# assafmu/wav2letter_pytorch

Hardware: AMD Instinct MI355X
Metric: audio-frames/sec/GPU (fwd+bwd+CTC), Wav2Letter 64-mel x 1000-frame bf16 (higher is better)
Workload: dtype bf16

## Files before the change

include/w2l_hip.h:

```cpp
#ifndef W2L_HIP_H
#define W2L_HIP_H
#include <stdint.h>
#ifdef __cplusplus
extern "C" {
#endif

const char* w2l_last_error(void);
int w2l_abi_version(void);


int w2l_pack_weights(const float* w, int64_t s_co, int64_t s_ci, int64_t s_kw, int Cout, int Cin, int Kw,
                     int CoutP, int CinP, void* w_fwd_hi, void* w_fwd_lo, void* w_dgr_hi, void* w_dgr_lo,
                     void* stream);

int w2l_sgd_pack(float* p, float* g, float* m, int first_step, float lr, float momentum, float weight_decay,
                 int nesterov, int zero_grad, int Cout, int Cin, int Kw, void* w_fwd_hi, void* w_fwd_lo, void* w_dgr_hi,
                 void* w_dgr_lo, void* w_fwd_q, void* w_dgr_q, float q_scale, void* stream);

int w2l_nct_to_ntc(const float* x, int N, int C, int T, int CP, int pad_l, int pad_r, int pad_mode,
                   const int32_t* lens, void* out_hi, void* out_lo, void* stream);

int w2l_pad_cast(const float* g, int N, int T, int C, int CP, int halo, void* out_hi, void* out_lo, float* colsum,
                 void* stream);

int w2l_conv_stat_tiles(int N, int Tout);
int w2l_conv1d_igemm(const void* xp, int64_t x_bstride, int64_t x_rows_total, const void* w, void* y, int y_f32,
                     int accumulate, const float* bias, float* stats_partial, int N, int Cin, int Cout, int Tout,
                     int Kw, int stride, int dil, void* stream);

int w2l_conv1d_igemm_tune(const void* xp, int64_t x_bstride, int64_t x_rows_total, const void* w, void* y, int y_f32,
                          const float* bias, float* stats_partial, int N, int Cin, int Cout, int Tout, int Kw, int stride,
                          int dil, int reps, void* stream);

int w2l_conv1d_igemm_ws(const void* xp, int64_t x_bstride, int64_t x_rows_total, const void* w, void* y, int y_f32,
                        int accumulate, const float* bias, float* stats_partial, int N, int Cin, int Cout, int Tout, int Kw,
                        int stride, int dil, void* splitk_ws, int64_t splitk_ws_bytes, void* stream);
int w2l_conv1d_igemm_tune_ws(const void* xp, int64_t x_bstride, int64_t x_rows_total, const void* w, void* y, int y_f32,
                             const float* bias, float* stats_partial, int N, int Cin, int Cout, int Tout, int Kw, int stride,
                             int dil, int reps, void* splitk_ws, int64_t splitk_ws_bytes, void* stream);
int64_t w2l_conv_splitk_workspace_bytes(int N, int Cout, int Tout);
int w2l_conv_streamk_ranges(int idx, int N, int Cin, int Cout, int Tout, int Kw, int stride, int dil, int64_t ws_bytes);
int w2l_conv_streamk_pieces(int tiles, int steps, int G, int* out, int cap);

int w2l_conv1d_igemm_fp8(const void* xq, int64_t x_bstride, int64_t x_rows_total, const void* wq, void* y, int y_f32,
                         float descale, const float* descale_dev, const float* bias, float* stats_partial, int N, int Cin,
                         int Cout, int Tout, int Kw, int dil, void* stream);
int w2l_conv1d_igemm_fp8_tune(const void* xq, int64_t x_bstride, int64_t x_rows_total, const void* wq, void* y, int y_f32,
                              const float* bias, float* stats_partial, int N, int Cin, int Cout, int Tout, int Kw, int dil,
                              int reps, void* stream);

void w2l_conv_force_tile_config(int idx);
void w2l_conv_force_fp8_config(int idx);
int w2l_conv_plan(int N, int Cin, int Cout, int Tout, int Kw, int stride, int dil, int stats_flag, int64_t ws_bytes,
                  int forced_idx, int* out);
int w2l_conv_plan_fp8(int N, int Cin, int Cout, int Tout, int Kw, int dil, int stats_flag, int forced_idx, int* out);

int w2l_wgrad_needs_zero(int N, int Cin, int Cout, int Tout, int Kw);
int w2l_conv1d_wgrad(const void* dy, int64_t dy_bstride, const void* xp, int64_t x_bstride, int64_t x_rows_total,
                     float* dw, int N, int Cin, int Cout, int Tout, int Kw, int stride, int dil, int accumulate,
                     void* stream);

int w2l_conv1d_wgrad_ws(const void* dy, int64_t dy_bstride, const void* xp, int64_t x_bstride, int64_t x_rows_total, float* dw,
                        int N, int Cin, int Cout, int Tout, int Kw, int stride, int dil, int accumulate, void* ws,
                        int64_t ws_bytes, void* stream);
int w2l_conv1d_wgrad_tune_ws(const void* dy, int64_t dy_bstride, const void* xp, int64_t x_bstride, int64_t x_rows_total,
                             float* dw_scratch, int N, int Cin, int Cout, int Tout, int Kw, int stride, int dil, int reps,
                             void* ws, int64_t ws_bytes, void* stream);
int w2l_wgrad_needs_zero_ws(int N, int Cin, int Cout, int Tout, int Kw, int64_t ws_bytes);
int64_t w2l_wgrad_workspace_bytes(int Cin, int Cout, int Kw);

int64_t w2l_wgrad_dealt_workspace_bytes(int Cin, int Cout, int Kw);
int w2l_conv1d_wgrad_tune_x(const void* dy, int64_t dy_bstride, const void* xp, int64_t x_bstride, int64_t x_rows_total,
                            float* dw_scratch, int N, int Cin, int Cout, int Tout, int Kw, int stride, int dil, int reps,
                            void* ws, int64_t ws_bytes, int flags, void* stream);
int w2l_wgrad_needs_zero_x(int N, int Cin, int Cout, int Tout, int Kw, int stride, int dil, int64_t ws_bytes);
int w2l_wgrad_dealt_segments(int tiles, int steps, int ranges, int* out, int max_blocks);
int w2l_wgrad_plan(int N, int Cin, int Cout, int Tout, int Kw);

typedef struct {
    const void* dy;
    int64_t dy_bstride;
    const void* xp;
    int64_t x_bstride;
    int64_t x_rows_total;
    float* dw;
    int Cin, Cout, Kw, pad_;
} w2l_wgrad_item_t;
#define W2L_WGRAD_GROUP_MAX 8
int w2l_conv1d_wgrad_group(const w2l_wgrad_item_t* items, int nitems, int N, int Tout, int dil, int form, void* stream);
int w2l_wgrad_group_tiles(int Cin, int Cout, int Kw, int form);

void w2l_wgrad_force_plan(int splits, int order);
void w2l_wgrad_deterministic(int on);

int w2l_conv1d_wgrad_tune(const void* dy, int64_t dy_bstride, const void* xp, int64_t x_bstride, int64_t x_rows_total,
                          float* dw_scratch, int N, int Cin, int Cout, int Tout, int Kw, int stride, int dil, int reps,
                          void* stream);

int w2l_wgrad_fp8_needs_zero(int N, int Cin, int Cout, int Tout, int Kw);
int w2l_conv1d_wgrad_fp8(const void* dyq, int64_t dy_bstride, const void* xq, int64_t x_bstride, int64_t x_rows_total,
                         float* dw, int N, int Cin, int Cout, int Tout, int Kw, int dil, float descale,
                         const float* descale_dev, int accumulate, void* stream);
int w2l_conv1d_wgrad_fp8_tune(const void* dyq, int64_t dy_bstride, const void* xq, int64_t x_bstride, int64_t x_rows_total,
                              float* dw_scratch, int N, int Cin, int Cout, int Tout, int Kw, int dil, int reps, void* stream);

int w2l_tune_save(const char* path);
int w2l_tune_load(const char* path);

int w2l_dwconv_fwd(const void* x_hi, const void* x_lo, int x_rows, const float* w, void* y_hi, void* y_lo, int N, int Tout,
                   int C, int K, int stride, int dil, const int32_t* lens, void* stream);
int w2l_dwconv_dgrad(const void* dy, int dy_f32, int dy_rows, const float* w, void* dxp, int dxp_f32, int N, int Tp, int Tout,
                     int C, int K, int dil, const int32_t* lens, void* stream);
int w2l_dwconv_wgrad(const void* dy, int dy_f32, int dy_rows, const void* x_hi, const void* x_lo, int x_rows, float* dw, int N,
                     int Tout, int C, int K, int stride, int dil, const int32_t* lens, void* stream);


int w2l_bn_finalize(const float* partial, int ntiles, int C, int64_t count, const float* gamma, const float* beta,
                    float eps, float momentum, float* running_mean, float* running_var, float* mean, float* invstd,
                    float* scale, float* shift, void* stream);

typedef struct {
    int32_t N, T, C;
    const void* y;
    int32_t y_f32;
    const float* scale;
    const float* shift;
    const float* mean;
    const float* invstd;
    const void* y2;
    const float* scale2;
    const float* shift2;
    const float* mean2;
    const float* invstd2;
    int32_t act;
    float drop_p;
    uint64_t seed, offset;
    uint8_t* mask;
    const int32_t* lens;
    const uint64_t* offset_dev;
    uint64_t* q_clipped;
} w2l_bnact_t;

int w2l_bn_act_fwd(const w2l_bnact_t* d, void* out_hi, void* out_lo, int out_rows, int pad_l, int pad_r,
                   int pad_mode, void* stream);
int w2l_bn_act_fwd_q(const w2l_bnact_t* d, void* out_hi, void* out_lo, void* out_q, float q_scale, int out_rows,
                     int pad_l, int pad_r, int pad_mode, void* stream);
typedef struct {
    const float* partial;
    int32_t rows;
    int64_t count;
    const float* gamma;
    const float* beta;
    float eps, momentum;
    float* running_mean;
    float* running_var;
    float* mean;
    float* invstd;
    float* scale;
    float* shift;
} w2l_bnfin_t;
int w2l_bn_act_fwd_fin(const w2l_bnact_t* d, const w2l_bnfin_t* f1, const w2l_bnfin_t* f2, void* out_hi, void* out_q,
                       float q_scale, int out_rows, int pad_l, int pad_r, int pad_mode, void* stream);
void w2l_conv_stats_mode(int slots);

int w2l_quantize_e4m3(const void* src, int src_f32, int64_t n, float scale, void* dst, void* stream);

typedef struct {
    const void* dxp;
    int32_t f32;
    int32_t pad_l, pad_r, pad_mode;
    int32_t rows;
} w2l_gradsrc_t;

int w2l_bn_bwd_blocks(int N, int T, int C);
int w2l_bn_act_bwd_reduce(const w2l_bnact_t* d, const w2l_gradsrc_t* g1, const w2l_gradsrc_t* g2, float* partial,
                          void* stream);
int w2l_bn_bwd_finalize(const float* partial, int nblocks, int C, int ncomp, float* sums, void* stream);
int w2l_bn_act_bwd_apply(const w2l_bnact_t* d, const w2l_gradsrc_t* g1, const w2l_gradsrc_t* g2, const float* sums,
                         void* dy_hi, void* dy_lo, int halo, void* dy2_hi, void* dy2_lo, int halo2, void* stream);
int w2l_bn_act_bwd_apply_fin(const w2l_bnact_t* d, const w2l_gradsrc_t* g1, const w2l_gradsrc_t* g2, const float* partial,
                             int nblocks, float* sums, void* dy_hi, void* dy_lo, int halo, void* dy2_hi, void* dy2_lo,
                             int halo2, float* amax, void* stream);
int w2l_bn_bwd_fast_ok(const w2l_bnact_t* d, const w2l_gradsrc_t* g1, const w2l_gradsrc_t* g2);
int w2l_bn_act_bwd_reduce_slots(const w2l_bnact_t* d, const w2l_gradsrc_t* g1, float* partial, int slots, void* stream);
int w2l_bn_act_bwd_apply_slots(const w2l_bnact_t* d, const w2l_gradsrc_t* g1, const float* partial, int nrows, float* sums,
                               void* dy_hi, int halo, float* amax, void* stream);
#define W2L_AMAX_SLOTS 64
int w2l_bn_act_bwd_apply_amax(const w2l_bnact_t* d, const w2l_gradsrc_t* g1, const w2l_gradsrc_t* g2, const float* sums,
                              void* dy_hi, void* dy_lo, int halo, void* dy2_hi, void* dy2_lo, int halo2, float* amax,
                              void* stream);
int w2l_quantize_e4m3_dyn(const void* src_bf16, int64_t n, const float* amax, void* dst, float* inv_scale, void* stream);

int w2l_conv1d_dgrad_bnreduce_ws(const void* dy, int64_t dy_rows_total, const void* w_dgr, void* dxp, float* partial,
                                 const w2l_bnact_t* d, int pad_l, int pad_r, int pad_mode, int per, int Cconv_out,
                                 int flat_rows, int Kw, int dil, void* splitk_ws, int64_t splitk_ws_bytes, void* stream);
int w2l_conv1d_dgrad_bnreduce_tune_ws(const void* dy, int64_t dy_rows_total, const void* w_dgr, void* dxp, float* partial,
                                      const w2l_bnact_t* d, int pad_l, int pad_r, int pad_mode, int per, int Cconv_out,
                                      int flat_rows, int Kw, int dil, int reps, void* splitk_ws, int64_t splitk_ws_bytes,
                                      void* stream);

typedef struct {
    const float* scale;
    const float* shift;
    const void* res;
    const void* res_lo;
    int32_t act;
    const int32_t* lens;
    void* out_hi;
    void* out_lo;
    int32_t out_rows, pad_l, pad_r, pad_mode;
} w2l_bnact_epi_t;
int w2l_conv1d_igemm_bnact(const void* xp, int64_t x_bstride, int64_t x_rows_total, const void* w, const float* acc_in,
                           const float* bias, const w2l_bnact_epi_t* e, int N, int Cin, int Cout, int Tout, int Kw, int stride,
                           int dil, void* stream);
int w2l_conv1d_igemm_bnact_ws(const void* xp, int64_t x_bstride, int64_t x_rows_total, const void* w, const float* acc_in,
                              const float* bias, const w2l_bnact_epi_t* e, int N, int Cin, int Cout, int Tout, int Kw,
                              int stride, int dil, void* splitk_ws, int64_t splitk_ws_bytes, void* stream);
int w2l_conv1d_igemm_bnact_tune_ws(const void* xp, int64_t x_bstride, int64_t x_rows_total, const void* w, const float* bias,
                                   const w2l_bnact_epi_t* e, int N, int Cin, int Cout, int Tout, int Kw, int stride, int dil,
                                   int reps, void* splitk_ws, int64_t splitk_ws_bytes, void* stream);

int w2l_conv1d_igemm_bnact_fp8(const void* xq, int64_t x_bstride, int64_t x_rows_total, const void* wq, float descale,
                               const float* bias, const w2l_bnact_epi_t* e, void* out_q, float q_scale, int64_t* q_clipped,
                               int N, int Cin, int Cout, int Tout, int Kw, int dil, void* stream);
int w2l_conv1d_igemm_bnact_fp8_tune(const void* xq, int64_t x_bstride, int64_t x_rows_total, const void* wq, const float* bias,
                                    const w2l_bnact_epi_t* e, void* out_q, float q_scale, int N, int Cin, int Cout, int Tout,
                                    int Kw, int dil, int reps, void* stream);

int w2l_log_softmax_fwd(const float* logits, int N, int T, int C, int CP, int mode, float* out, void* stream);
int w2l_log_softmax_bwd(const float* gout, const float* out, int N, int T, int C, int mode, float* glogits,
                        void* stream);
int64_t w2l_ctc_workspace_bytes(int N, int T, int Smax);
int w2l_ctc_loss(const float* log_probs, const int32_t* targets, const int32_t* input_lengths,
                 const int32_t* target_lengths, int N, int T, int C, int Smax, int blank, int zero_infinity,
                 float* nll, float* loss, float* grad, void* workspace, void* stream);

int64_t w2l_ctc_align_workspace_bytes(int N, int T, int Smax);
int w2l_ctc_align(const float* x, const int32_t* input_lengths, const int32_t* targets, int64_t target_stride,
                  const int32_t* target_lengths, int64_t length_stride, int N, int T, int A, int Smax, int blank,
                  int log_probs, void* workspace, int64_t workspace_bytes, float* score, int32_t* status, int32_t* path,
                  int32_t* starts, int32_t* ends, void* stream);

int w2l_argmax(const float* probs, int64_t rows, int C, int32_t* idx, void* stream);
int64_t w2l_ctc_beam_search_workspace_bytes(int N, int T, int k);
int w2l_ctc_beam_search(const float* probs, const int32_t* sizes, int N, int T, int A, const int32_t* label_info_host,
                        int blank, int end_index, int k, double beta, double prune, int log_probs, void* workspace,
                        int64_t workspace_bytes, void* out, void* stream);
typedef struct {
    const float* prob;
    const float* bo;
    const uint64_t* ngram_keys;
    const int32_t* ngram_vals;
    int64_t ngram_cap;
    const uint64_t* trie_keys;
    const int32_t* trie_vals;
    int64_t trie_cap;
    const int32_t* trie_word;
    int32_t n_entries;
    int32_t n_words;
    int32_t n_trie_nodes;
} w2l_ngram_lm_t;
int w2l_ngram_lm_build(const uint64_t* keys, const int32_t* vals, int64_t n, uint64_t* table_keys, int32_t* table_vals,
                       int64_t cap, int32_t* dups, void* stream);
int64_t w2l_ctc_beam_search_lm_workspace_bytes(int N, int T, int k, int order);
int w2l_ctc_beam_search_lm(const float* probs, const int32_t* sizes, int N, int T, int A, const int32_t* label_info_host,
                           int blank, int end_index, int space_index, int k, double alpha, double beta, double prune,
                           int log_probs, const w2l_ngram_lm_t* lm, int order, void* workspace, int64_t workspace_bytes,
                           void* out, void* stream);
int w2l_levenshtein_host(const int32_t* a_host, int na, const int32_t* b_host, int nb);
int w2l_greedy_score_host(const int32_t* idx_host, int N, int T, const int32_t* sizes_host, int blank, const int32_t* lut,
                          int n_labels, const int32_t* ref_cp, const int64_t* ref_off, int64_t* totals, int32_t* hyp_cp,
                          int64_t* hyp_off);

int w2l_novograd_pack(float* p, const float* g, float* exp_avg, float* exp_avg_sq, float* max_exp_avg_sq, float* scratch,
                      int scratch_floats, float lr, float beta1, float beta2, float eps, float weight_decay, int grad_averaging,
                      int Cout, int Cin, int Kw, void* w_fwd_hi, void* w_fwd_lo, void* w_dgr_hi, void* w_dgr_lo, void* stream);

int w2l_logmel(const float* audio, const int32_t* n_samples, const float* noise, float dither, float preemph, int N,
               int64_t audio_stride, const float* window, int win_length, int n_fft, int hop, const float* fbT,
               const int32_t* fb_range, int n_mels, int take_log, float log_guard, float* logmel, int Tmax, void* stream);
int w2l_feature_normalize(const float* logmel, const int32_t* n_samples, int hop, int N, int Tmax, int n_mels, float eps,
                          float* mean_ws, float* std_ws, float* out_nct, void* stream);
int w2l_zero_rects(float* x, int N, int C, int T, const int32_t* rects, int R, void* stream);

#define W2L_RESAMPLE_TILE 512
#define W2L_RESAMPLE_MAX_K 512
#define W2L_RESAMPLE_MAX_SPAN 8192
int w2l_resample(const float* x, int64_t in_stride, float* out, int64_t out_stride, int N, const int32_t* rows_host,
                 const int32_t* rows_dev, const int32_t* banks_host, const int32_t* banks_dev, int n_banks, const float* taps,
                 int64_t n_taps, void* stream);

int w2l_stream_probe(void* stream_a, void* stream_b, void* stamps_dev, int rounds, int spin_us);

// ... 53 lines not shown
```

wav2letter_pytorch_amd/_lib.py:

```python
from __future__ import annotations

import ctypes as C
import os

os.environ.setdefault('GPU_MAX_HW_QUEUES', '8')

import torch

_HERE = os.path.dirname(os.path.abspath(__file__))
LIB_PATH = os.environ.get('W2L_LIB') or os.path.join(_HERE, 'libw2l_hip.so')

c_p = C.c_void_p
c_i = C.c_int
c_i64 = C.c_int64
c_u64 = C.c_uint64
c_f = C.c_float


class BnActDesc(C.Structure):
    _fields_ = [
        ('N', C.c_int32), ('T', C.c_int32), ('C', C.c_int32),
        ('y', c_p), ('y_f32', C.c_int32),
        ('scale', c_p), ('shift', c_p), ('mean', c_p), ('invstd', c_p),
        ('y2', c_p), ('scale2', c_p), ('shift2', c_p), ('mean2', c_p), ('invstd2', c_p),
        ('act', C.c_int32), ('drop_p', c_f), ('seed', c_u64), ('offset', c_u64),
        ('mask', c_p), ('lens', c_p), ('offset_dev', c_p), ('q_clipped', c_p),
    ]


class WgradItem(C.Structure):
    _fields_ = [('dy', c_p), ('dy_bstride', C.c_int64), ('xp', c_p), ('x_bstride', C.c_int64), ('x_rows_total', C.c_int64),
                ('dw', c_p), ('Cin', C.c_int32), ('Cout', C.c_int32), ('Kw', C.c_int32), ('pad_', C.c_int32)]


class BnFin(C.Structure):
    _fields_ = [('partial', c_p), ('rows', C.c_int32), ('count', C.c_int64), ('gamma', c_p), ('beta', c_p), ('eps', c_f),
                ('momentum', c_f), ('running_mean', c_p), ('running_var', c_p), ('mean', c_p), ('invstd', c_p), ('scale', c_p),
                ('shift', c_p)]


class LmTables(C.Structure):
    _fields_ = [('prob', c_p), ('bo', c_p), ('ngram_keys', c_p), ('ngram_vals', c_p), ('ngram_cap', C.c_int64),
                ('trie_keys', c_p), ('trie_vals', c_p), ('trie_cap', C.c_int64), ('trie_word', c_p), ('n_entries', C.c_int32),
                ('n_words', C.c_int32), ('n_trie_nodes', C.c_int32)]


class BnActEpi(C.Structure):
    _fields_ = [('scale', c_p), ('shift', c_p), ('res', c_p), ('res_lo', c_p), ('act', C.c_int32), ('lens', c_p),
                ('out_hi', c_p), ('out_lo', c_p), ('out_rows', C.c_int32), ('pad_l', C.c_int32), ('pad_r', C.c_int32),
                ('pad_mode', C.c_int32)]


class GradSrc(C.Structure):
    _fields_ = [('dxp', c_p), ('f32', C.c_int32), ('pad_l', C.c_int32), ('pad_r', C.c_int32),
                ('pad_mode', C.c_int32), ('rows', C.c_int32)]


_SIGNATURES = {
    'w2l_last_error': (C.c_char_p, []),
    'w2l_abi_version': (c_i, []),
    'w2l_tune_save': (c_i, [C.c_char_p]),
    'w2l_tune_load': (c_i, [C.c_char_p]),
    'w2l_pack_weights': (c_i, [c_p, c_i64, c_i64, c_i64, c_i, c_i, c_i, c_i, c_i, c_p, c_p, c_p, c_p, c_p]),
    'w2l_sgd_pack': (c_i, [c_p, c_p, c_p, c_i, c_f, c_f, c_f, c_i, c_i, c_i, c_i, c_i, c_p, c_p, c_p, c_p, c_p, c_p, c_f, c_p]),
    'w2l_novograd_pack': (c_i, [c_p, c_p, c_p, c_p, c_p, c_p, c_i, c_f, c_f, c_f, c_f, c_f, c_i, c_i, c_i, c_i, c_p, c_p, c_p, c_p,
                                c_p]),
    'w2l_nct_to_ntc': (c_i, [c_p, c_i, c_i, c_i, c_i, c_i, c_i, c_i, c_p, c_p, c_p, c_p]),
    'w2l_pad_cast': (c_i, [c_p, c_i, c_i, c_i, c_i, c_i, c_p, c_p, c_p, c_p]),
    'w2l_conv_stat_tiles': (c_i, [c_i, c_i]),
    'w2l_conv1d_igemm': (c_i, [c_p, c_i64, c_i64, c_p, c_p, c_i, c_i, c_p, c_p, c_i, c_i, c_i, c_i, c_i, c_i, c_i, c_p]),
    'w2l_conv1d_igemm_tune': (c_i, [c_p, c_i64, c_i64, c_p, c_p, c_i, c_p, c_p, c_i, c_i, c_i, c_i, c_i, c_i, c_i, c_i, c_p]),
    'w2l_conv1d_igemm_ws': (c_i, [c_p, c_i64, c_i64, c_p, c_p, c_i, c_i, c_p, c_p, c_i, c_i, c_i, c_i, c_i, c_i, c_i, c_p, c_i64, c_p]),
    'w2l_conv1d_igemm_tune_ws': (c_i, [c_p, c_i64, c_i64, c_p, c_p, c_i, c_p, c_p, c_i, c_i, c_i, c_i, c_i, c_i, c_i, c_i, c_p,
                                       c_i64, c_p]),
    'w2l_conv1d_igemm_bnact': (c_i, [c_p, c_i64, c_i64, c_p, c_p, c_p, C.POINTER(BnActEpi), c_i, c_i, c_i, c_i, c_i, c_i, c_i, c_p]),
    'w2l_conv1d_igemm_bnact_ws': (c_i, [c_p, c_i64, c_i64, c_p, c_p, c_p, C.POINTER(BnActEpi), c_i, c_i, c_i, c_i, c_i, c_i, c_i,
                                        c_p, c_i64, c_p]),
    'w2l_conv1d_igemm_bnact_tune_ws': (c_i, [c_p, c_i64, c_i64, c_p, c_p, C.POINTER(BnActEpi), c_i, c_i, c_i, c_i, c_i, c_i, c_i,
                                             c_i, c_p, c_i64, c_p]),
    'w2l_conv_splitk_workspace_bytes': (c_i64, [c_i, c_i, c_i]),
    'w2l_conv_streamk_ranges': (c_i, [c_i] * 8 + [c_i64]),
    'w2l_conv_streamk_pieces': (c_i, [c_i, c_i, c_i, c_p, c_i]),
    'w2l_conv_force_tile_config': (None, [c_i]),
    'w2l_conv_force_fp8_config': (None, [c_i]),
    'w2l_conv_plan': (c_i, [c_i] * 8 + [c_i64, c_i, c_p]),
    'w2l_conv_plan_fp8': (c_i, [c_i] * 8 + [c_p]),
    'w2l_wgrad_force_plan': (None, [c_i, c_i]),
    'w2l_wgrad_deterministic': (None, [c_i]),
    'w2l_wgrad_needs_zero': (c_i, [c_i, c_i, c_i, c_i, c_i]),
    'w2l_conv1d_wgrad': (c_i, [c_p, c_i64, c_p, c_i64, c_i64, c_p, c_i, c_i, c_i, c_i, c_i, c_i, c_i, c_i, c_p]),
    'w2l_conv1d_wgrad_ws': (c_i, [c_p, c_i64, c_p, c_i64, c_i64, c_p, c_i, c_i, c_i, c_i, c_i, c_i, c_i, c_i, c_p, c_i64, c_p]),
    'w2l_conv1d_wgrad_tune_ws': (c_i, [c_p, c_i64, c_p, c_i64, c_i64, c_p, c_i, c_i, c_i, c_i, c_i, c_i, c_i, c_i, c_p, c_i64, c_p]),
    'w2l_wgrad_needs_zero_ws': (c_i, [c_i, c_i, c_i, c_i, c_i, c_i64]),
    'w2l_wgrad_workspace_bytes': (c_i64, [c_i, c_i, c_i]),
    'w2l_wgrad_dealt_workspace_bytes': (c_i64, [c_i, c_i, c_i]),
    'w2l_conv1d_wgrad_tune_x': (c_i, [c_p, c_i64, c_p, c_i64, c_i64, c_p, c_i, c_i, c_i, c_i, c_i, c_i, c_i, c_i, c_p, c_i64, c_i, c_p]),
    'w2l_wgrad_needs_zero_x': (c_i, [c_i, c_i, c_i, c_i, c_i, c_i, c_i, c_i64]),
    'w2l_wgrad_dealt_segments': (c_i, [c_i, c_i, c_i, c_p, c_i]),
    'w2l_wgrad_plan': (c_i, [c_i, c_i, c_i, c_i, c_i]),
    'w2l_conv1d_wgrad_group': (c_i, [c_p, c_i, c_i, c_i, c_i, c_i, c_p]),
    'w2l_wgrad_group_tiles': (c_i, [c_i, c_i, c_i, c_i]),
    'w2l_conv1d_wgrad_tune': (c_i, [c_p, c_i64, c_p, c_i64, c_i64, c_p, c_i, c_i, c_i, c_i, c_i, c_i, c_i, c_i, c_p]),
    'w2l_dwconv_fwd': (c_i, [c_p, c_p, c_i, c_p, c_p, c_p, c_i, c_i, c_i, c_i, c_i, c_i, c_p, c_p]),
    'w2l_dwconv_dgrad': (c_i, [c_p, c_i, c_i, c_p, c_p, c_i, c_i, c_i, c_i, c_i, c_i, c_i, c_p, c_p]),
    'w2l_dwconv_wgrad': (c_i, [c_p, c_i, c_i, c_p, c_p, c_i, c_p, c_i, c_i, c_i, c_i, c_i, c_i, c_p, c_p]),
    'w2l_bn_finalize': (c_i, [c_p, c_i, c_i, c_i64, c_p, c_p, c_f, c_f, c_p, c_p, c_p, c_p, c_p, c_p, c_p]),
    'w2l_bn_act_fwd': (c_i, [C.POINTER(BnActDesc), c_p, c_p, c_i, c_i, c_i, c_i, c_p]),
    'w2l_bn_act_fwd_q': (c_i, [C.POINTER(BnActDesc), c_p, c_p, c_p, c_f, c_i, c_i, c_i, c_i, c_p]),
    'w2l_bn_bwd_fast_ok': (c_i, [C.POINTER(BnActDesc), C.POINTER(GradSrc), C.POINTER(GradSrc)]),
    'w2l_bn_act_bwd_reduce_slots': (c_i, [C.POINTER(BnActDesc), C.POINTER(GradSrc), c_p, c_i, c_p]),
    'w2l_bn_act_bwd_apply_slots': (c_i, [C.POINTER(BnActDesc), C.POINTER(GradSrc), c_p, c_i, c_p, c_p, c_i, c_p, c_p]),
    'w2l_bn_act_fwd_fin': (c_i, [C.POINTER(BnActDesc), C.POINTER(BnFin), C.POINTER(BnFin), c_p, c_p, c_f, c_i, c_i, c_i, c_i, c_p]),
    'w2l_conv_stats_mode': (None, [c_i]),
    'w2l_quantize_e4m3': (c_i, [c_p, c_i, c_i64, c_f, c_p, c_p]),
    'w2l_quantize_e4m3_dyn': (c_i, [c_p, c_i64, c_p, c_p, c_p, c_p]),
    'w2l_bn_act_bwd_apply_amax': (c_i, [C.POINTER(BnActDesc), C.POINTER(GradSrc), C.POINTER(GradSrc), c_p, c_p, c_p, c_i,
                                        c_p, c_p, c_i, c_p, c_p]),
    'w2l_conv1d_igemm_fp8': (c_i, [c_p, c_i64, c_i64, c_p, c_p, c_i, c_f, c_p, c_p, c_p, c_i, c_i, c_i, c_i, c_i, c_i, c_p]),
    'w2l_conv1d_igemm_bnact_fp8': (c_i, [c_p, c_i64, c_i64, c_p, c_f, c_p, C.POINTER(BnActEpi), c_p, c_f, c_p, c_i, c_i, c_i, c_i,
                                         c_i, c_i, c_p]),
    'w2l_conv1d_igemm_bnact_fp8_tune': (c_i, [c_p, c_i64, c_i64, c_p, c_p, C.POINTER(BnActEpi), c_p, c_f, c_i, c_i, c_i, c_i, c_i,
                                              c_i, c_i, c_p]),
    'w2l_conv1d_igemm_fp8_tune': (c_i, [c_p, c_i64, c_i64, c_p, c_p, c_i, c_p, c_p, c_i, c_i, c_i, c_i, c_i, c_i, c_i, c_p]),
    'w2l_bn_bwd_blocks': (c_i, [c_i, c_i, c_i]),
    'w2l_bn_act_bwd_reduce': (c_i, [C.POINTER(BnActDesc), C.POINTER(GradSrc), C.POINTER(GradSrc), c_p, c_p]),
    'w2l_bn_bwd_finalize': (c_i, [c_p, c_i, c_i, c_i, c_p, c_p]),
    'w2l_bn_act_bwd_apply': (c_i, [C.POINTER(BnActDesc), C.POINTER(GradSrc), C.POINTER(GradSrc), c_p, c_p, c_p, c_i,
                                   c_p, c_p, c_i, c_p]),
    'w2l_conv1d_dgrad_bnreduce_ws': (c_i, [c_p, c_i64, c_p, c_p, c_p, C.POINTER(BnActDesc), c_i, c_i, c_i, c_i, c_i, c_i, c_i, c_i,
                                           c_p, c_i64, c_p]),
    'w2l_conv1d_dgrad_bnreduce_tune_ws': (c_i, [c_p, c_i64, c_p, c_p, c_p, C.POINTER(BnActDesc), c_i, c_i, c_i, c_i, c_i, c_i, c_i,
                                                c_i, c_i, c_p, c_i64, c_p]),
    'w2l_bn_act_bwd_apply_fin': (c_i, [C.POINTER(BnActDesc), C.POINTER(GradSrc), C.POINTER(GradSrc), c_p, c_i, c_p, c_p, c_p, c_i,
                                       c_p, c_p, c_i, c_p, c_p]),
    'w2l_log_softmax_fwd': (c_i, [c_p, c_i, c_i, c_i, c_i, c_i, c_p, c_p]),
    'w2l_log_softmax_bwd': (c_i, [c_p, c_p, c_i, c_i, c_i, c_i, c_p, c_p]),
    'w2l_ctc_workspace_bytes': (c_i64, [c_i, c_i, c_i]),
    'w2l_ctc_loss': (c_i, [c_p, c_p, c_p, c_p, c_i, c_i, c_i, c_i, c_i, c_i, c_p, c_p, c_p, c_p, c_p]),
    'w2l_argmax': (c_i, [c_p, c_i64, c_i, c_p, c_p]),
    'w2l_ctc_align_workspace_bytes': (c_i64, [c_i, c_i, c_i]),
    'w2l_ctc_align': (c_i, [c_p, c_p, c_p, c_i64, c_p, c_i64, c_i, c_i, c_i, c_i, c_i, c_i, c_p, c_i64, c_p, c_p, c_p, c_p, c_p,
                            c_p]),
    'w2l_ctc_beam_search_workspace_bytes': (c_i64, [c_i, c_i, c_i]),
    'w2l_ctc_beam_search': (c_i, [c_p, c_p, c_i, c_i, c_i, c_p, c_i, c_i, c_i, C.c_double, C.c_double, c_i, c_p, c_i64, c_p,
                                  c_p]),
    'w2l_ngram_lm_build': (c_i, [c_p, c_p, c_i64, c_p, c_p, c_i64, c_p, c_p]),
    'w2l_ctc_beam_search_lm_workspace_bytes': (c_i64, [c_i, c_i, c_i, c_i]),
    'w2l_ctc_beam_search_lm': (c_i, [c_p, c_p, c_i, c_i, c_i, c_p, c_i, c_i, c_i, c_i, C.c_double, C.c_double, C.c_double, c_i,
                                     C.POINTER(LmTables), c_i, c_p, c_i64, c_p, c_p]),
    'w2l_logmel': (c_i, [c_p, c_p, c_p, c_f, c_f, c_i, c_i64, c_p, c_i, c_i, c_i, c_p, c_p, c_i, c_i, c_f, c_p, c_i, c_p]),
    'w2l_feature_normalize': (c_i, [c_p, c_p, c_i, c_i, c_i, c_i, c_f, c_p, c_p, c_p, c_p]),
    'w2l_zero_rects': (c_i, [c_p, c_i, c_i, c_i, c_p, c_i, c_p]),
    'w2l_resample': (c_i, [c_p, c_i64, c_p, c_i64, c_i, c_p, c_p, c_p, c_p, c_i, c_p, c_i64, c_p]),
    'w2l_levenshtein_host': (c_i, [c_p, c_i, c_p, c_i]),
    'w2l_greedy_score_host': (c_i, [c_p, c_i, c_i, c_p, c_i, c_p, c_i, c_p, c_p, c_p, c_p, c_p]),
    'w2l_wgrad_fp8_needs_zero': (c_i, [c_i, c_i, c_i, c_i, c_i]),
    'w2l_conv1d_wgrad_fp8': (c_i, [c_p, c_i64, c_p, c_i64, c_i64, c_p, c_i, c_i, c_i, c_i, c_i, c_i, c_f, c_p, c_i, c_p]),
    'w2l_conv1d_wgrad_fp8_tune': (c_i, [c_p, c_i64, c_p, c_i64, c_i64, c_p, c_i, c_i, c_i, c_i, c_i, c_i, c_i, c_p]),
    'w2l_stream_probe': (c_i, [c_p, c_p, c_p, c_i, c_i]),
    'w2l_rccl_available': (c_i, []),
    'w2l_rccl_library': (C.c_char_p, []),
    'w2l_rccl_unique_id': (c_i, [c_p]),
    'w2l_rccl_init': (c_i, [c_p, c_i, c_i, c_p]),
    'w2l_rccl_world': (c_i, [c_p, c_p]),
    'w2l_rccl_all_reduce': (c_i, [c_p, c_p, c_i64, c_i, c_i, c_p]),
    'w2l_rccl_broadcast': (c_i, [c_p, c_p, c_i64, c_i, c_p]),
    'w2l_rccl_destroy': (c_i, [c_p]),
    'w2l_replay_op': (c_i, [C.c_char_p]),
    'w2l_replay_arity': (c_i, [c_i]),
    'w2l_replay': (c_i, [c_p, c_i, c_p]),
    'w2l_event_create': (c_i, [c_p]),
    'w2l_event_destroy': (c_i, [c_p]),
    'w2l_event_record': (c_i, [c_p, c_p]),
    'w2l_stream_wait_event': (c_i, [c_p, c_p]),
    'w2l_event_query': (c_i, [c_p]),
    'w2l_event_synchronize': (c_i, [c_p]),
    'w2l_stream_wait_stream': (c_i, [c_p, c_p]),
    'w2l_fill_zero': (c_i, [c_p, c_i64, c_p]),
    'w2l_pad_vec_f32': (c_i, [c_p, c_i, c_p, c_i, c_f, c_p]),
# ... 378 lines not shown
```

wav2letter_pytorch_amd/csrc/bn_act.hip:

```cpp
#include "common.h"
#include "../../include/w2l_hip.h"

namespace {

#ifndef W2L_PHILOX_ROUNDS
#define W2L_PHILOX_ROUNDS 10
#endif
__device__ __forceinline__ void philox4x32_10(uint32_t c0, uint32_t c1, uint32_t c2, uint32_t c3, uint32_t k0,
                                              uint32_t k1, uint32_t out[4]) {
#pragma unroll
    for (int i = 0; i < W2L_PHILOX_ROUNDS; ++i) {
        const uint64_t p0 = (uint64_t)0xD2511F53u * c0, p1 = (uint64_t)0xCD9E8D57u * c2;
        const uint32_t hi0 = (uint32_t)(p0 >> 32), lo0 = (uint32_t)p0;
        const uint32_t hi1 = (uint32_t)(p1 >> 32), lo1 = (uint32_t)p1;
        const uint32_t n0 = hi1 ^ c1 ^ k0, n1 = lo1, n2 = hi0 ^ c3 ^ k1, n3 = lo0;
        c0 = n0; c1 = n1; c2 = n2; c3 = n3;
        k0 += 0x9E3779B9u; k1 += 0xBB67AE85u;
    }
    out[0] = c0; out[1] = c1; out[2] = c2; out[3] = c3;
}

__device__ __forceinline__ uint32_t dropout_bits(uint64_t seed, uint64_t offset, uint64_t gidx, uint32_t thresh) {
    uint32_t r[4];
    philox4x32_10((uint32_t)gidx, (uint32_t)(gidx >> 32), (uint32_t)offset, (uint32_t)(offset >> 32), (uint32_t)seed,
                  (uint32_t)(seed >> 32), r);
    uint32_t bits = 0;
#pragma unroll
    for (int j = 0; j < 4; ++j) {
        bits |= ((r[j] & 0xFFFFu) >= thresh ? 1u : 0u) << (2 * j);
        bits |= ((r[j] >> 16) >= thresh ? 1u : 0u) << (2 * j + 1);
    }
    return bits;
}

template <bool F32>
__device__ __forceinline__ void load8(const void* base, int64_t off, float v[8]) {
    if (F32) {
        const f32x4* p = reinterpret_cast<const f32x4*>(reinterpret_cast<const float*>(base) + off);
        const f32x4 a = p[0], b = p[1];
#pragma unroll
        for (int j = 0; j < 4; ++j) { v[j] = a[j]; v[4 + j] = b[j]; }
    } else {
        const u16x8 a = *reinterpret_cast<const u16x8*>(reinterpret_cast<const bf16_raw*>(base) + off);
#pragma unroll
        for (int j = 0; j < 8; ++j) v[j] = bf16_bits_to_f32(a[j]);
    }
}
__device__ __forceinline__ void loadp8(const float* p, int c, float v[8]) {
    const f32x4 a = *reinterpret_cast<const f32x4*>(p + c), b = *reinterpret_cast<const f32x4*>(p + c + 4);
#pragma unroll
    for (int j = 0; j < 4; ++j) { v[j] = a[j]; v[4 + j] = b[j]; }
}
__device__ __forceinline__ void store8_split(bf16_raw* hi, bf16_raw* lo, int64_t off, const float v[8]) {
    u16x8 h, l;
#pragma unroll
    for (int j = 0; j < 8; ++j) {
        bf16_raw a, b;
        f32_split_bf16(v[j], a, b);
        h[j] = a; l[j] = b;
    }
    *reinterpret_cast<u16x8*>(hi + off) = h;
    if (lo) *reinterpret_cast<u16x8*>(lo + off) = l;
}

__device__ __forceinline__ int pad_src_row(int r, int T, int pad_l, int pad_r, int pad_mode) {
    int t = r - pad_l;
    if (t >= 0 && t < T) return t;
    if (pad_mode != 1 || t < -pad_l || t >= T + pad_r) return -1;
    t = t < 0 ? -t : 2 * (T - 1) - t;
    return (t >= 0 && t < T) ? t : -1;
}

struct Chan {
    float sc[8], sh[8], m[8], is[8];
};
__device__ __forceinline__ void load_chan(Chan& ch, const float* scale, const float* shift, const float* mean,
                                          const float* invstd, int c) {
#pragma unroll
    for (int j = 0; j < 8; ++j) { ch.sc[j] = 1.f; ch.sh[j] = 0.f; ch.m[j] = 0.f; ch.is[j] = 0.f; }
    if (scale) { loadp8(scale, c, ch.sc); loadp8(shift, c, ch.sh); }
    if (mean) { loadp8(mean, c, ch.m); loadp8(invstd, c, ch.is); }
}

template <bool F32, bool HAS2>
__device__ __forceinline__ uint32_t preact8(const w2l_bnact_t& d, const Chan& c1, const Chan& c2, int64_t row ,
                                            int cg, int G, float z[8], float y1[8], float y2v[8], uint32_t thresh,
                                            float inv_keep, bool gen_mask, bool write_mask) {
    const int64_t off = row * d.C + cg * 8;
    load8<F32>(d.y, off, y1);
#pragma unroll
    for (int j = 0; j < 8; ++j) z[j] = y1[j] * c1.sc[j] + c1.sh[j];
    if (HAS2) {
        load8<F32>(d.y2, off, y2v);
#pragma unroll
        for (int j = 0; j < 8; ++j) z[j] += y2v[j] * c2.sc[j] + c2.sh[j];
    }
    uint32_t bits = 0xFFu;
    if (d.drop_p > 0.f) {
        const int64_t gidx = row * G + cg;
        if (gen_mask) {
            bits = dropout_bits(d.seed, d.offset + (d.offset_dev ? *d.offset_dev : 0ull), (uint64_t)gidx, thresh);
            if (write_mask) d.mask[gidx] = (uint8_t)bits;
        } else {
            bits = d.mask[gidx];
        }
#pragma unroll
        for (int j = 0; j < 8; ++j) z[j] = (bits >> j) & 1u ? z[j] * inv_keep : 0.f;
    }
    return bits;
}

__device__ __forceinline__ float activate(float z, int act) {
    if (act == 1) return fminf(fmaxf(z, 0.f), 20.f);
    if (act == 2) return fmaxf(z, 0.f);
    return z;
}
template <int ACT>
__device__ __forceinline__ float activate_t(float z) {
    if (ACT == 1) return fminf(fmaxf(z, 0.f), 20.f);
    if (ACT == 2) return fmaxf(z, 0.f);
    return z;
}
__device__ __forceinline__ bool act_pass(float z, int act) {
    if (act == 1) return z >= 0.f && z <= 20.f;
    if (act == 2) return z > 0.f;
    return true;
}

constexpr int AMAX_SLOTS = W2L_AMAX_SLOTS;
__device__ __forceinline__ void amax_publish(float* amax, int slot, float mx) {
    unsigned* p = reinterpret_cast<unsigned*>(amax) + slot;
    const unsigned v = __float_as_uint(mx);
    if (v > __hip_atomic_load(p, __ATOMIC_RELAXED, __HIP_MEMORY_SCOPE_AGENT)) atomicMax(p, v);
}
constexpr int BWD_SLAB = 64;

__device__ __forceinline__ uint2 quant8_e4m3(const float v[8], float scale) {
    float q[8];
#pragma unroll
    for (int j = 0; j < 8; ++j) q[j] = fminf(fmaxf(v[j] * scale, -448.f), 448.f);
    int lo = __builtin_amdgcn_cvt_pk_fp8_f32(q[0], q[1], 0, false);
    lo = __builtin_amdgcn_cvt_pk_fp8_f32(q[2], q[3], lo, true);
    int hi = __builtin_amdgcn_cvt_pk_fp8_f32(q[4], q[5], 0, false);
    hi = __builtin_amdgcn_cvt_pk_fp8_f32(q[6], q[7], hi, true);
    return make_uint2((unsigned)lo, (unsigned)hi);
}

template <bool F32, bool HAS2, int ACT>
__global__ __launch_bounds__(256) void bn_act_fwd_kernel(w2l_bnact_t d, bf16_raw* out_hi, bf16_raw* out_lo, int R,
                                                          int pad_l, int pad_r, int pad_mode, uint32_t thresh,
                                                          float inv_keep, uint8_t* out_q, float q_scale, float inv_g) {
    const int G = d.C >> 3;
    const int n = blockIdx.y;
    unsigned clipped = 0;
    const float q_limit = 448.f / q_scale;
    const int idx = blockIdx.x * 256 + threadIdx.x;
    if (idx < R * G) {
        int r = (int)((float)idx * inv_g);
        r -= (r * G > idx) ? 1 : 0;
        r += ((r + 1) * G <= idx) ? 1 : 0;
        const int cg = idx - r * G;
        const unsigned orow = (unsigned)n * R + r;
        const int t = pad_src_row(r, d.T, pad_l, pad_r, pad_mode);
        float a[8];
#pragma unroll
        for (int j = 0; j < 8; ++j) a[j] = 0.f;
        if (t >= 0 && (!d.lens || t < d.lens[n])) {
            float z[8], y1[8], y2v[8];
            Chan c1, c2;
            load_chan(c1, d.scale, d.shift, nullptr, nullptr, cg * 8);
            if (HAS2) load_chan(c2, d.scale2, d.shift2, nullptr, nullptr, cg * 8);
            preact8<F32, HAS2>(d, c1, c2, (int64_t)n * d.T + t, cg, G, z, y1, y2v, thresh, inv_keep, true,
                         r - pad_l == t);
#pragma unroll
            for (int j = 0; j < 8; ++j) a[j] = activate_t<ACT>(z[j]);
        }
        store8_split(out_hi, out_lo, (int64_t)orow * d.C + cg * 8, a);
        if (out_q) {
            *reinterpret_cast<uint2*>(out_q + (int64_t)orow * d.C + cg * 8) = quant8_e4m3(a, q_scale);
            if (d.q_clipped && r - pad_l == t) {
#pragma unroll
                for (int j = 0; j < 8; ++j) clipped += fabsf(a[j]) > q_limit ? 1u : 0u;
            }
        }
    }
    if (out_q && d.q_clipped && __any(clipped != 0)) {
#pragma unroll
        for (int m = 1; m < 64; m <<= 1) clipped += __shfl_xor(clipped, m, 64);
        if ((threadIdx.x & 63) == 0) atomicAdd(reinterpret_cast<unsigned long long*>(d.q_clipped), (unsigned long long)clipped);
    }
}

struct FinBranch {
    const float* partial;
    int rows;
    double count;
    const float* gamma;
    const float* beta;
    float eps, momentum;
    float* running_mean;
    float* running_var;
    float* mean;
    float* invstd;
    float* scale;
    float* shift;
};

#ifndef W2L_FWD_FIN_U
#define W2L_FWD_FIN_U 1
#endif
constexpr int FWD_FIN_U = W2L_FWD_FIN_U;
#ifndef W2L_FWD_FIN_BLOCKS
#define W2L_FWD_FIN_BLOCKS 2560
#endif
__host__ __device__ inline int fwd_rows_per_block(int64_t rows, int C) {
    const int batch = 4 * FWD_FIN_U * 8;
    int64_t nb = (rows * (C / BWD_SLAB) + (int64_t)batch * W2L_FWD_FIN_BLOCKS - 1) / ((int64_t)batch * W2L_FWD_FIN_BLOCKS);
    nb = nb < 1 ? 1 : (nb > 16 ? 16 : nb);
    return (int)nb * batch;
}

template <bool HAS2, int ACT>
__global__ __launch_bounds__(256) void bn_act_fwd_fin_kernel(w2l_bnact_t d, FinBranch f1, FinBranch f2, bf16_raw* out_hi, int R,
                                                              int pad_l, int pad_r, int pad_mode, uint32_t thresh, float inv_keep,
                                                              uint8_t* out_q, float q_scale, int rpb) {
    __shared__ double red[2][2][BWD_SLAB];
    __shared__ float s_sc[2][BWD_SLAB], s_sh[2][BWD_SLAB];
    const int tid = threadIdx.x, lane = tid & 63, wave = tid >> 6;
    const int G = d.C >> 3;
    const int nslabs = d.C / BWD_SLAB;
    const int slab = blockIdx.x % nslabs, chunk = blockIdx.x / nslabs;
    const int cgl = lane & 7, rr = lane >> 3;
    const int cg = slab * (BWD_SLAB / 8) + cgl, c = cg * 8;
    const int T = d.T;
    const int64_t rows = (int64_t)d.N * R;
    constexpr int U = FWD_FIN_U;
    const int nbatch = rpb / (4 * U * 8);
    int64_t q0 = (int64_t)chunk * rpb + (int64_t)wave * (U * 8) + rr;
    u16x8 ya[U], yb[U];
    int nn[U], tt[U], rw[U];
    bool ok[U];
    auto load_batch = [&]() {
#pragma unroll
        for (int u = 0; u < U; ++u) {
            const int64_t q = q0 + 8 * u;
            ok[u] = false;
            nn[u] = 0; tt[u] = 0; rw[u] = 0;
            if (q < rows) {
                const int n = (int)(q / R), r = (int)(q - (int64_t)n * R);
                const int t = pad_src_row(r, T, pad_l, pad_r, pad_mode);
                nn[u] = n; tt[u] = t; rw[u] = r;
                ok[u] = t >= 0 && (!d.lens || t < d.lens[n]);
                if (ok[u]) {
                    const int64_t src = ((int64_t)n * T + t) * d.C + c;
                    ya[u] = *reinterpret_cast<const u16x8*>(reinterpret_cast<const bf16_raw*>(d.y) + src);
                    if (HAS2) yb[u] = *reinterpret_cast<const u16x8*>(reinterpret_cast<const bf16_raw*>(d.y2) + src);
                }
            }
        }
    };
    load_batch();
    {
        const int cc = tid & 63, ch = slab * BWD_SLAB + cc;
        const int br = tid >> 7, k = (tid >> 6) & 1;
        const FinBranch& f = br ? f2 : f1;
        if ((br == 0 || HAS2) && f.partial) {
            double a = 0.0;
            int j = 0;
            for (; j + 8 <= f.rows; j += 8) {
                float v[8];
#pragma unroll
                for (int u = 0; u < 8; ++u) v[u] = f.partial[((int64_t)(j + u) * 2 + k) * d.C + ch];
#pragma unroll
                for (int u = 0; u < 8; ++u) a += v[u];
            }
            for (; j < f.rows; ++j) a += f.partial[((int64_t)j * 2 + k) * d.C + ch];
            red[br][k][cc] = a;
        }
        __syncthreads();
        if (tid < 128 && (tid < 64 || HAS2)) {
            const int b = tid >> 6;
            const FinBranch& g = b ? f2 : f1;
            float sc = 1.f, sh = 0.f;
            if (g.partial) {
                const double mu = red[b][0][cc] / g.count;
                double var = red[b][1][cc] / g.count - mu * mu;
                if (var < 0.0) var = 0.0;
                const float m = (float)mu, istd = (float)(1.0 / sqrt(var + (double)g.eps));
                const float ga = g.gamma ? g.gamma[ch] : 1.f, be = g.beta ? g.beta[ch] : 0.f;
                sc = ga * istd;
                sh = be - m * ga * istd;
                if (chunk == 0) {
                    if (g.running_mean) {
                        const double unbiased = g.count > 1.0 ? var * g.count / (g.count - 1.0) : var;
                        g.running_mean[ch] = (1.f - g.momentum) * g.running_mean[ch] + g.momentum * m;
                        g.running_var[ch] = (1.f - g.momentum) * g.running_var[ch] + g.momentum * (float)unbiased;
                    }
                    if (g.mean) { g.mean[ch] = m; g.invstd[ch] = istd; }
                    g.scale[ch] = sc;
                    g.shift[ch] = sh;
                }
            } else {
                const float* scp = b ? d.scale2 : d.scale;
                const float* shp = b ? d.shift2 : d.shift;
                if (scp) { sc = scp[ch]; sh = shp[ch]; }
            }
            s_sc[b][cc] = sc;
            s_sh[b][cc] = sh;
        }
        __syncthreads();
    }
    float sc1[8], sh1[8], sc2[8], sh2[8];
#pragma unroll
    for (int j = 0; j < 8; ++j) {
        sc1[j] = s_sc[0][cgl * 8 + j]; sh1[j] = s_sh[0][cgl * 8 + j];
        sc2[j] = HAS2 ? s_sc[1][cgl * 8 + j] : 0.f; sh2[j] = HAS2 ? s_sh[1][cgl * 8 + j] : 0.f;
    }
    unsigned clipped = 0;
    const float q_limit = 448.f / q_scale;
    const bool drop = d.drop_p > 0.f;
    const uint64_t off = drop ? d.offset + (d.offset_dev ? *d.offset_dev : 0ull) : 0ull;
    for (int bt = 0; bt < nbatch; ++bt) {
    if (bt) load_batch();
#pragma unroll
    for (int u = 0; u < U; ++u) {
        const int64_t q = q0 + 8 * u;
        if (q >= rows) break;
        float a[8];
#pragma unroll
        for (int j = 0; j < 8; ++j) a[j] = 0.f;
        if (ok[u]) {
            float z[8];
#pragma unroll
            for (int j = 0; j < 8; ++j) {
                z[j] = bf16_bits_to_f32(ya[u][j]) * sc1[j] + sh1[j];
                if (HAS2) z[j] += bf16_bits_to_f32(yb[u][j]) * sc2[j] + sh2[j];
            }
            if (drop) {
                const int64_t gidx = ((int64_t)nn[u] * T + tt[u]) * G + cg;
                const uint32_t bits = dropout_bits(d.seed, off, (uint64_t)gidx, thresh);
                if (rw[u] - pad_l == tt[u]) d.mask[gidx] = (uint8_t)bits;
#pragma unroll
                for (int j = 0; j < 8; ++j) z[j] = (bits >> j) & 1u ? z[j] * inv_keep : 0.f;
            }
#pragma unroll
            for (int j = 0; j < 8; ++j) a[j] = activate_t<ACT>(z[j]);
        }
        store8_split(out_hi, nullptr, q * d.C + c, a);
        if (out_q) {
            *reinterpret_cast<uint2*>(out_q + q * d.C + c) = quant8_e4m3(a, q_scale);
            if (d.q_clipped && rw[u] - pad_l == tt[u]) {
#pragma unroll
                for (int j = 0; j < 8; ++j) clipped += fabsf(a[j]) > q_limit ? 1u : 0u;
            }
        }
    }
    q0 += 4 * U * 8;
    }
    if (out_q && d.q_clipped && __any(clipped != 0)) {
#pragma unroll
        for (int m = 1; m < 64; m <<= 1) clipped += __shfl_xor(clipped, m, 64);
        if (lane == 0) atomicAdd(reinterpret_cast<unsigned long long*>(d.q_clipped), (unsigned long long)clipped);
    }
}

__global__ __launch_bounds__(256) void quantize_e4m3_kernel(const void* src, int src_f32, int64_t ngroups, float scale,
                                                             uint8_t* dst) {
    for (int64_t i = (int64_t)blockIdx.x * 256 + threadIdx.x; i < ngroups; i += (int64_t)gridDim.x * 256) {
        float v[8];
        if (src_f32) load8<true>(src, i * 8, v);
        else load8<false>(src, i * 8, v);
        *reinterpret_cast<uint2*>(dst + i * 8) = quant8_e4m3(v, scale);
    }
}

template <bool GF32>
__device__ __forceinline__ void add_grad8(const w2l_gradsrc_t& s, int n, int t, int T, int C, int cg, float g[8]) {
    const int64_t base = (int64_t)n * s.rows;
    float v[8];
    load8<GF32>(s.dxp, (base + t + s.pad_l) * C + cg * 8, v);
#pragma unroll
    for (int j = 0; j < 8; ++j) g[j] += v[j];
    if (s.pad_mode == 1) {
        if (t >= 1 && t <= s.pad_l) {
            load8<GF32>(s.dxp, (base + s.pad_l - t) * C + cg * 8, v);
#pragma unroll
            for (int j = 0; j < 8; ++j) g[j] += v[j];
        }
        if (t <= T - 2 && t >= T - 1 - s.pad_r) {
            load8<GF32>(s.dxp, (base + s.pad_l + 2 * (T - 1) - t) * C + cg * 8, v);
#pragma unroll
            for (int j = 0; j < 8; ++j) g[j] += v[j];
        }
    }
}

struct BwdRow {
    float g[8];
    float xh1[8];
    float xh2[8];
};

template <bool F32, bool GF32, bool HAS2>
__device__ __forceinline__ void bwd_row(const w2l_bnact_t& d, const Chan& c1, const Chan& c2, const w2l_gradsrc_t& g1,
                                        const w2l_gradsrc_t& g2, int has_g2, int n, int t, int cg, int G, float inv_keep,
                                        BwdRow& o) {
    float z[8], y1[8], y2v[8];
#pragma unroll
    for (int j = 0; j < 8; ++j) { o.g[j] = 0.f; o.xh1[j] = 0.f; o.xh2[j] = 0.f; y2v[j] = 0.f; }
    const uint32_t bits = preact8<F32, HAS2>(d, c1, c2, (int64_t)n * d.T + t, cg, G, z, y1, y2v, 0, inv_keep, false, false);
    const bool masked = d.lens && t >= d.lens[n];
    float g[8];
#pragma unroll
    for (int j = 0; j < 8; ++j) g[j] = 0.f;
    if (!masked) {
        add_grad8<GF32>(g1, n, t, d.T, d.C, cg, g);
        if (has_g2) add_grad8<GF32>(g2, n, t, d.T, d.C, cg, g);
    }
    const float gk = d.drop_p > 0.f ? inv_keep : 1.f;
#pragma unroll
    for (int j = 0; j < 8; ++j) {
        const bool keep = (bits >> j) & 1u;
        o.g[j] = (!masked && keep && act_pass(z[j], d.act)) ? g[j] * gk : 0.f;
        o.xh1[j] = (y1[j] - c1.m[j]) * c1.is[j];
        if (HAS2) o.xh2[j] = (y2v[j] - c2.m[j]) * c2.is[j];
    }
}

__host__ __device__ inline int bwd_rows_per_wave(int64_t rows, int C) {
    int64_t rw = (rows * (C / BWD_SLAB) + 4095) / 4096;
    rw = (rw + 7) / 8 * 8;
    return (int)(rw < 16 ? 16 : (rw > 64 ? 64 : rw));
}

template <bool F32, bool GF32, bool HAS2>
__global__ __launch_bounds__(256) void bn_act_bwd_reduce_kernel(w2l_bnact_t d, w2l_gradsrc_t g1, w2l_gradsrc_t g2,
                                                                 int has_g2, float* partial, float inv_keep, int rw,
                                                                 int nchunks) {
    const int G = d.C >> 3;
    const int nslabs = d.C / BWD_SLAB;
    const int lane = threadIdx.x & 63;
    const int task = blockIdx.x * 4 + (threadIdx.x >> 6);
    if (task >= nslabs * nchunks) return;
    const int chunk = task / nslabs, slab = task - chunk * nslabs;
    const int cg = slab * (BWD_SLAB / 8) + (lane & 7);
    const int rr = lane >> 3;
    constexpr int ncomp = HAS2 ? 4 : 2;
    const int64_t rows = (int64_t)d.N * d.T;
    const int64_t row0 = (int64_t)chunk * rw;
    int64_t rend = row0 + rw;
    if (rend > rows) rend = rows;
    float s0[8], s1[8], s2[8];
#pragma unroll
    for (int j = 0; j < 8; ++j) { s0[j] = 0.f; s1[j] = 0.f; s2[j] = 0.f; }
    Chan c1, c2;
    load_chan(c1, d.scale, d.shift, d.mean, d.invstd, cg * 8);
    if (HAS2) load_chan(c2, d.scale2, d.shift2, d.mean2, d.invstd2, cg * 8);
    int n = (int)((row0 + rr) / d.T), t = (int)((row0 + rr) - (int64_t)n * d.T);
#pragma unroll 2
    for (int64_t row = row0 + rr; row < rend; row += 8, t += 8) {
        while (t >= d.T) { t -= d.T; ++n; }
        BwdRow o;
        bwd_row<F32, GF32, HAS2>(d, c1, c2, g1, g2, has_g2, n, t, cg, G, inv_keep, o);
#pragma unroll
        for (int j = 0; j < 8; ++j) {
            s0[j] += o.g[j];
            s1[j] += o.g[j] * o.xh1[j];
            if (HAS2) s2[j] += o.g[j] * o.xh2[j];
        }
    }
#pragma unroll
    for (int m = 8; m < 64; m <<= 1)
#pragma unroll
        for (int j = 0; j < 8; ++j) {
            s0[j] += __shfl_xor(s0[j], m, 64);
            s1[j] += __shfl_xor(s1[j], m, 64);
            if (HAS2) s2[j] += __shfl_xor(s2[j], m, 64);
        }
    if (rr == 0) {
        float* dst = partial + (int64_t)chunk * ncomp * d.C + cg * 8;
        auto put = [&](float* q, const float* v) {
            *reinterpret_cast<f32x4*>(q) = f32x4{v[0], v[1], v[2], v[3]};
            *reinterpret_cast<f32x4*>(q + 4) = f32x4{v[4], v[5], v[6], v[7]};
        };
        put(dst, s0);
        put(dst + d.C, s1);
        if (ncomp == 4) { put(dst + 2 * d.C, s0); put(dst + 3 * d.C, s2); }
    }
}

__global__ __launch_bounds__(256) void bn_bwd_finalize_kernel(const float* partial, int nblocks, int ncols, float* sums) {
    __shared__ float red[8][33];
    const int cx = threadIdx.x & 31, ly = threadIdx.x >> 5;
    const int col = blockIdx.x * 32 + cx;
    float s = 0.f;
    if (col < ncols) {
        int b = ly;
        float a[8];
        for (; b + 56 < nblocks; b += 64) {
#pragma unroll
// ... 100 lines not shown
        }
    }
}

__host__ __device__ inline int apply_rows_per_block(int64_t rows, int C) {
    int64_t r = rows * (C / BWD_SLAB) / 1536;
    r = (r + 31) / 32 * 32;
    return (int)(r < 64 ? 64 : (r > 1024 ? 1024 : r));
}

template <bool F32, bool GF32, bool HAS2>
__global__ __launch_bounds__(256) void bn_act_bwd_apply_fin_kernel(w2l_bnact_t d, w2l_gradsrc_t g1, w2l_gradsrc_t g2,
                                                                    int has_g2, const float* partial, int nb, float* sums_out,
                                                                    bf16_raw* dy_hi, bf16_raw* dy_lo, int h1, bf16_raw* dy2_hi,
                                                                    bf16_raw* dy2_lo, int h2, float inv_keep, float* amax,
                                                                    int rpb) {
    constexpr int ncomp = HAS2 ? 4 : 2;
    __shared__ float red[4][ncomp][BWD_SLAB];
    __shared__ float ssum[ncomp][BWD_SLAB];
    const int tid = threadIdx.x, lane = tid & 63, wave = tid >> 6;
    const int G = d.C >> 3;
    const int nslabs = d.C / BWD_SLAB;
    const int slab = blockIdx.x % nslabs, chunk = blockIdx.x / nslabs;
    const int T = d.T, N = d.N;
    {
        const int c = slab * BWD_SLAB + (tid & 63);
        float a[ncomp];
#pragma unroll
        for (int k = 0; k < ncomp; ++k) a[k] = 0.f;
        int j = wave;
        for (; j + 12 < nb; j += 16) {
            float v[4][ncomp];
#pragma unroll
            for (int u = 0; u < 4; ++u)
#pragma unroll
                for (int k = 0; k < ncomp; ++k) v[u][k] = partial[((int64_t)(j + 4 * u) * ncomp + k) * d.C + c];
#pragma unroll
            for (int u = 0; u < 4; ++u)
#pragma unroll
                for (int k = 0; k < ncomp; ++k) a[k] += v[u][k];
        }
        for (; j < nb; j += 4)
#pragma unroll
            for (int k = 0; k < ncomp; ++k) a[k] += partial[((int64_t)j * ncomp + k) * d.C + c];
#pragma unroll
        for (int k = 0; k < ncomp; ++k) red[wave][k][tid & 63] = a[k];
        __syncthreads();
        if (tid < ncomp * BWD_SLAB) {
            const int k = tid >> 6, cc = tid & 63;
            const float t4 = (red[0][k][cc] + red[1][k][cc]) + (red[2][k][cc] + red[3][k][cc]);
            ssum[k][cc] = t4;
            if (chunk == 0) sums_out[(int64_t)k * d.C + slab * BWD_SLAB + cc] = t4;
        }
        __syncthreads();
    }
    const int cgl = lane & 7, rr = lane >> 3;
    const int cg = slab * (BWD_SLAB / 8) + cgl, c = cg * 8;
    Chan c1, c2;
    load_chan(c1, d.scale, d.shift, d.mean, d.invstd, c);
    if (HAS2) load_chan(c2, d.scale2, d.shift2, d.mean2, d.invstd2, c);
    float sg[8], sgx[8], sg2[8], sgx2[8];
#pragma unroll
    for (int j = 0; j < 8; ++j) {
        sg[j] = ssum[0][cgl * 8 + j];
        sgx[j] = ssum[1][cgl * 8 + j];
        sg2[j] = HAS2 ? ssum[2][cgl * 8 + j] : 0.f;
        sgx2[j] = HAS2 ? ssum[3][cgl * 8 + j] : 0.f;
    }
    const float invM = 1.f / ((float)N * (float)T);
    const int64_t rows = (int64_t)N * T;
    const int rpw = rpb >> 2;
    const int64_t row0 = (int64_t)chunk * rpb + (int64_t)wave * rpw;
    int64_t rend = row0 + rpw;
    if (rend > rows) rend = rows;
    float mx1 = 0.f, mx2 = 0.f;
    if (row0 + rr < rend) {
        int n = (int)((row0 + rr) / T), t = (int)((row0 + rr) - (int64_t)n * T);
#pragma unroll 2
        for (int64_t row = row0 + rr; row < rend; row += 8, t += 8) {
            while (t >= T) { t -= T; ++n; }
            BwdRow o;
            bwd_row<F32, GF32, HAS2>(d, c1, c2, g1, g2, has_g2, n, t, cg, G, inv_keep, o);
            float o1[8], o2[8];
            if (d.mean) {
#pragma unroll
                for (int j = 0; j < 8; ++j) o1[j] = c1.sc[j] * (o.g[j] - sg[j] * invM - o.xh1[j] * sgx[j] * invM);
            } else {
#pragma unroll
                for (int j = 0; j < 8; ++j) o1[j] = o.g[j] * c1.sc[j];
            }
            store8_split(dy_hi, dy_lo, ((int64_t)h1 + (int64_t)n * (T + h1) + t) * d.C + c, o1);
            if (amax) {
#pragma unroll
                for (int j = 0; j < 8; ++j) mx1 = fmaxf(mx1, fabsf(o1[j]));
            }
            if (HAS2 && dy2_hi) {
                if (d.mean2) {
#pragma unroll
                    for (int j = 0; j < 8; ++j) o2[j] = c2.sc[j] * (o.g[j] - sg2[j] * invM - o.xh2[j] * sgx2[j] * invM);
                } else {
#pragma unroll
                    for (int j = 0; j < 8; ++j) o2[j] = o.g[j] * c2.sc[j];
                }
                store8_split(dy2_hi, dy2_lo, ((int64_t)h2 + (int64_t)n * (T + h2) + t) * d.C + c, o2);
                if (amax) {
#pragma unroll
                    for (int j = 0; j < 8; ++j) mx2 = fmaxf(mx2, fabsf(o2[j]));
                }
            }
        }
    }
    {
        const int nchunks = gridDim.x / nslabs;
        float z[8];
#pragma unroll
        for (int j = 0; j < 8; ++j) z[j] = 0.f;
        for (int pass = 0; pass < 2; ++pass) {
            bf16_raw* hi = pass ? dy2_hi : dy_hi;
            bf16_raw* lo = pass ? dy2_lo : dy_lo;
            const int h = pass ? h2 : h1;
            if (hi == nullptr || h == 0) continue;
            const int total = h * (N + 1);
            const int per = (total + nchunks - 1) / nchunks;
            int e = (chunk + 1) * per;
            if (e > total) e = total;
            for (int hr = chunk * per + wave * 8 + rr; hr < e; hr += 32) {
                const int gap = hr / h, r = hr - gap * h;
                store8_split(hi, lo, ((int64_t)gap * (T + h) + r) * d.C + c, z);
            }
        }
    }
    if (amax) {
#pragma unroll
        for (int m = 1; m < 64; m <<= 1) {
            mx1 = fmaxf(mx1, __shfl_xor(mx1, m, 64));
            mx2 = fmaxf(mx2, __shfl_xor(mx2, m, 64));
        }
        if (lane == 0) {
            const int slot = blockIdx.x & (AMAX_SLOTS - 1);
            amax_publish(amax, slot, mx1);
            if (HAS2 && dy2_hi) amax_publish(amax, AMAX_SLOTS + slot, mx2);
        }
    }
}


struct FastRow {
    u16x8 y, g, ga, gb;
    unsigned bits;
    bool live, fa, fb, masked;
    int n, t;
};

__device__ __forceinline__ void fast_row_load(const w2l_bnact_t& d, const w2l_gradsrc_t& s, int64_t row, int64_t rows, int c,
                                              int cg, int G, FastRow& o) {
    o.live = row < rows;
    o.fa = o.fb = o.masked = false;
    o.bits = 0xFFu;
    o.n = 0; o.t = 0;
    if (!o.live) return;
    const int T = d.T;
    const int n = (int)(row / T), t = (int)(row - (int64_t)n * T);
    o.n = n; o.t = t;
    o.y = *reinterpret_cast<const u16x8*>(reinterpret_cast<const bf16_raw*>(d.y) + row * d.C + c);
    if (d.drop_p > 0.f) o.bits = d.mask[row * G + cg];
    o.masked = d.lens && t >= d.lens[n];
    const bf16_raw* gp = reinterpret_cast<const bf16_raw*>(s.dxp);
    const int64_t base = (int64_t)n * s.rows;
    o.g = *reinterpret_cast<const u16x8*>(gp + (base + t + s.pad_l) * d.C + c);
    if (s.pad_mode == 1) {
        o.fa = t >= 1 && t <= s.pad_l;
        o.fb = t <= T - 2 && t >= T - 1 - s.pad_r;
        if (o.fa) o.ga = *reinterpret_cast<const u16x8*>(gp + (base + s.pad_l - t) * d.C + c);
        if (o.fb) o.gb = *reinterpret_cast<const u16x8*>(gp + (base + s.pad_l + 2 * (T - 1) - t) * d.C + c);
    }
}

template <int ACT, bool DROP>
__device__ __forceinline__ void fast_row_eval(const FastRow& r, const Chan& ch, float inv_keep, float g[8], float xh[8]) {
    float gv[8];
#pragma unroll
    for (int j = 0; j < 8; ++j) gv[j] = bf16_bits_to_f32(r.g[j]);
    if (r.fa) {
#pragma unroll
        for (int j = 0; j < 8; ++j) gv[j] += bf16_bits_to_f32(r.ga[j]);
    }
    if (r.fb) {
#pragma unroll
        for (int j = 0; j < 8; ++j) gv[j] += bf16_bits_to_f32(r.gb[j]);
    }
    const float gk = DROP ? inv_keep : 1.f;
    const bool row_ok = !r.masked;
#pragma unroll
    for (int j = 0; j < 8; ++j) {
        const float y = bf16_bits_to_f32(r.y[j]);
        float z = y * ch.sc[j] + ch.sh[j];
        bool pass = row_ok;
        if (DROP) {
            pass = pass && ((r.bits >> j) & 1u);
            z *= inv_keep;
        }
        if (ACT == 1) pass = pass && z >= 0.f && z <= 20.f;
        else if (ACT == 2) pass = pass && z > 0.f;
        g[j] = pass ? gv[j] * gk : 0.f;
        xh[j] = (y - ch.m[j]) * ch.is[j];
    }
}

template <int U, int ACT, bool DROP>
__global__ __launch_bounds__(256) void bn_bwd_reduce_fast_kernel(w2l_bnact_t d, w2l_gradsrc_t g1, float* partial, float inv_keep,
                                                                  int slots) {
    __shared__ float red[4][2][BWD_SLAB];
    const int tid = threadIdx.x, lane = tid & 63, wave = tid >> 6;
    const int G = d.C >> 3, nslabs = d.C / BWD_SLAB;
    const int slab = blockIdx.x % nslabs, chunk = blockIdx.x / nslabs;
    const int cgl = lane & 7, rr = lane >> 3;
    const int cg = slab * (BWD_SLAB / 8) + cgl, c = cg * 8;
    const int64_t rows = (int64_t)d.N * d.T;
    const int64_t q0 = ((int64_t)chunk * 4 + wave) * (U * 8) + rr;
    FastRow r[U];
#pragma unroll
    for (int u = 0; u < U; ++u) fast_row_load(d, g1, q0 + 8 * u, rows, c, cg, G, r[u]);
    Chan ch;
    load_chan(ch, d.scale, d.shift, d.mean, d.invstd, c);
    float s0[8], s1[8];
#pragma unroll
    for (int j = 0; j < 8; ++j) { s0[j] = 0.f; s1[j] = 0.f; }
#pragma unroll
    for (int u = 0; u < U; ++u) {
        if (!r[u].live) continue;
        float g[8], xh[8];
        fast_row_eval<ACT, DROP>(r[u], ch, inv_keep, g, xh);
#pragma unroll
        for (int j = 0; j < 8; ++j) { s0[j] += g[j]; s1[j] += g[j] * xh[j]; }
    }
#pragma unroll
    for (int m = 8; m < 64; m <<= 1)
#pragma unroll
        for (int j = 0; j < 8; ++j) {
            s0[j] += __shfl_xor(s0[j], m, 64);
            s1[j] += __shfl_xor(s1[j], m, 64);
        }
    if (rr == 0) {
#pragma unroll
        for (int j = 0; j < 8; ++j) { red[wave][0][cgl * 8 + j] = s0[j]; red[wave][1][cgl * 8 + j] = s1[j]; }
    }
    __syncthreads();
    if (tid < 2 * BWD_SLAB) {
        const int k = tid >> 6, cc = tid & 63;
        const float t4 = (red[0][k][cc] + red[1][k][cc]) + (red[2][k][cc] + red[3][k][cc]);
        atomicAdd(partial + ((int64_t)(chunk % slots) * 2 + k) * d.C + slab * BWD_SLAB + cc, t4);
    }
}

template <int U, int ACT, bool DROP>
__global__ __launch_bounds__(256) void bn_bwd_apply_fast_kernel(w2l_bnact_t d, w2l_gradsrc_t g1, const float* partial, int nb,
                                                                 float* sums_out, bf16_raw* dy_hi, int h1, float inv_keep,
                                                                 float* amax) {
    __shared__ float ssum[2][BWD_SLAB];
    __shared__ float smax[4];
    const int tid = threadIdx.x, lane = tid & 63, wave = tid >> 6;
    const int G = d.C >> 3, nslabs = d.C / BWD_SLAB;
    const int slab = blockIdx.x % nslabs, chunk = blockIdx.x / nslabs;
    const int cgl = lane & 7, rr = lane >> 3;
    const int cg = slab * (BWD_SLAB / 8) + cgl, c = cg * 8;
    const int T = d.T, N = d.N;
    const int64_t rows = (int64_t)N * T;
    const int64_t q0 = ((int64_t)chunk * 4 + wave) * (U * 8) + rr;
    FastRow r[U];
#pragma unroll
    for (int u = 0; u < U; ++u) fast_row_load(d, g1, q0 + 8 * u, rows, c, cg, G, r[u]);
    if (tid < 2 * BWD_SLAB) {
        const int k = tid >> 6, cc = tid & 63;
        float a = 0.f;
        int j = 0;
        for (; j + 8 <= nb; j += 8) {
            float v[8];
#pragma unroll
            for (int u = 0; u < 8; ++u) v[u] = partial[((int64_t)(j + u) * 2 + k) * d.C + slab * BWD_SLAB + cc];
#pragma unroll
            for (int u = 0; u < 8; ++u) a += v[u];
        }
        for (; j < nb; ++j) a += partial[((int64_t)j * 2 + k) * d.C + slab * BWD_SLAB + cc];
        ssum[k][cc] = a;
        if (chunk == 0) sums_out[(int64_t)k * d.C + slab * BWD_SLAB + cc] = a;
    }
    __syncthreads();
    Chan ch;
    load_chan(ch, d.scale, d.shift, d.mean, d.invstd, c);
    float sg[8], sgx[8];
#pragma unroll
    for (int j = 0; j < 8; ++j) { sg[j] = ssum[0][cgl * 8 + j]; sgx[j] = ssum[1][cgl * 8 + j]; }
    const float invM = 1.f / ((float)N * (float)T);
    float mx = 0.f;
#pragma unroll
    for (int u = 0; u < U; ++u) {
        if (!r[u].live) continue;
        float g[8], xh[8], o[8];
        fast_row_eval<ACT, DROP>(r[u], ch, inv_keep, g, xh);
        if (d.mean) {
#pragma unroll
            for (int j = 0; j < 8; ++j) o[j] = ch.sc[j] * (g[j] - sg[j] * invM - xh[j] * sgx[j] * invM);
        } else {
#pragma unroll
            for (int j = 0; j < 8; ++j) o[j] = g[j] * ch.sc[j];
        }
        store8_split(dy_hi, nullptr, ((int64_t)h1 + (int64_t)r[u].n * (T + h1) + r[u].t) * d.C + c, o);
        if (amax) {
#pragma unroll
            for (int j = 0; j < 8; ++j) mx = fmaxf(mx, fabsf(o[j]));
        }
    }
    if (h1 > 0) {
        const int nchunks = gridDim.x / nslabs;
        float z[8];
#pragma unroll
        for (int j = 0; j < 8; ++j) z[j] = 0.f;
        const int total = h1 * (N + 1);
        const int per = (total + nchunks - 1) / nchunks;
        int e = (chunk + 1) * per;
        if (e > total) e = total;
        for (int hr = chunk * per + wave * 8 + rr; hr < e; hr += 32) {
            const int gap = hr / h1, rw = hr - gap * h1;
            store8_split(dy_hi, nullptr, ((int64_t)gap * (T + h1) + rw) * d.C + c, z);
        }
    }
    if (amax) {
#pragma unroll
        for (int m = 1; m < 64; m <<= 1) mx = fmaxf(mx, __shfl_xor(mx, m, 64));
        if (lane == 0) smax[wave] = mx;
        __syncthreads();
        if (tid == 0) amax_publish(amax, blockIdx.x & (AMAX_SLOTS - 1), fmaxf(fmaxf(smax[0], smax[1]), fmaxf(smax[2], smax[3])));
    }
}

struct RowCur {
    int64_t row;
    int n, t;
    const bf16_raw* py;
    const bf16_raw* pg;
    const uint8_t* pm;
};
__device__ __forceinline__ void rowcur_init(RowCur& q, const w2l_bnact_t& d, const w2l_gradsrc_t& s, int64_t row, int c, int cg, int G) {
    q.row = row;
    q.n = (int)(row / d.T);
    q.t = (int)(row - (int64_t)q.n * d.T);
    q.py = reinterpret_cast<const bf16_raw*>(d.y) + row * d.C + c;
    q.pg = reinterpret_cast<const bf16_raw*>(s.dxp) + ((int64_t)q.n * s.rows + q.t + s.pad_l) * d.C + c;
    q.pm = d.mask ? d.mask + row * G + cg : nullptr;
}
__device__ __forceinline__ void rowcur_step(RowCur& q, const w2l_bnact_t& d, const w2l_gradsrc_t& s, int G) {
    q.row += 8;
    q.t += 8;
    q.py += 8 * (int64_t)d.C;
    q.pg += 8 * (int64_t)d.C;
    if (q.pm) q.pm += 8 * G;
    if (q.t >= d.T) {
        q.t -= d.T;
        ++q.n;
        q.pg += (int64_t)(s.rows - d.T) * d.C;
    }
}
__device__ __forceinline__ void fast_row_load_cur(const w2l_bnact_t& d, const w2l_gradsrc_t& s, const RowCur& q, bool live, FastRow& o) {
    o.live = live;
    o.fa = o.fb = o.masked = false;
    o.bits = 0xFFu;
    o.n = q.n; o.t = q.t;
    if (!live) return;
    const int T = d.T, t = q.t;
    o.y = *reinterpret_cast<const u16x8*>(q.py);
    if (d.drop_p > 0.f) o.bits = *q.pm;
    o.masked = d.lens && t >= d.lens[q.n];
    o.g = *reinterpret_cast<const u16x8*>(q.pg);
    if (s.pad_mode == 1) {
        o.fa = t >= 1 && t <= s.pad_l;
        o.fb = t <= T - 2 && t >= T - 1 - s.pad_r;
        if (o.fa) o.ga = *reinterpret_cast<const u16x8*>(q.pg - 2 * (int64_t)t * d.C);
        if (o.fb) o.gb = *reinterpret_cast<const u16x8*>(q.pg + 2 * (int64_t)(T - 1 - t) * d.C);
    }
}

template <int ACT, bool DROP>
__global__ __launch_bounds__(256) void bn_bwd_reduce_loop_kernel(w2l_bnact_t d, w2l_gradsrc_t g1, float* partial, float inv_keep,
                                                                  int slots, int iters) {
    __shared__ float red[4][2][BWD_SLAB];
    const int tid = threadIdx.x, lane = tid & 63, wave = tid >> 6;
    const int G = d.C >> 3, nslabs = d.C / BWD_SLAB;
    const int slab = blockIdx.x % nslabs, chunk = blockIdx.x / nslabs;
    const int cgl = lane & 7, rr = lane >> 3;
    const int cg = slab * (BWD_SLAB / 8) + cgl, c = cg * 8;
    const int64_t rows = (int64_t)d.N * d.T;
    RowCur q;
    rowcur_init(q, d, g1, ((int64_t)chunk * 4 + wave) * ((int64_t)iters * 8) + rr, c, cg, G);
    FastRow cur, nxt;
    fast_row_load_cur(d, g1, q, q.row < rows, cur);
    Chan ch;
    load_chan(ch, d.scale, d.shift, d.mean, d.invstd, c);
    float s0[8], s1[8];
#pragma unroll
    for (int j = 0; j < 8; ++j) { s0[j] = 0.f; s1[j] = 0.f; }
    for (int it = 0; it < iters; ++it) {
        rowcur_step(q, d, g1, G);
        fast_row_load_cur(d, g1, q, it + 1 < iters && q.row < rows, nxt);
        if (cur.live) {
            float g[8], xh[8];
            fast_row_eval<ACT, DROP>(cur, ch, inv_keep, g, xh);
#pragma unroll
            for (int j = 0; j < 8; ++j) { s0[j] += g[j]; s1[j] += g[j] * xh[j]; }
        }
        cur = nxt;
    }
#pragma unroll
    for (int m = 8; m < 64; m <<= 1)
#pragma unroll
        for (int j = 0; j < 8; ++j) {
            s0[j] += __shfl_xor(s0[j], m, 64);
            s1[j] += __shfl_xor(s1[j], m, 64);
        }
    if (rr == 0) {
#pragma unroll
        for (int j = 0; j < 8; ++j) { red[wave][0][cgl * 8 + j] = s0[j]; red[wave][1][cgl * 8 + j] = s1[j]; }
    }
    __syncthreads();
    if (tid < 2 * BWD_SLAB) {
        const int k = tid >> 6, cc = tid & 63;
        const float t4 = (red[0][k][cc] + red[1][k][cc]) + (red[2][k][cc] + red[3][k][cc]);
        atomicAdd(partial + ((int64_t)(chunk % slots) * 2 + k) * d.C + slab * BWD_SLAB + cc, t4);
    }
}

template <int ACT, bool DROP>
__global__ __launch_bounds__(256) void bn_bwd_apply_loop_kernel(w2l_bnact_t d, w2l_gradsrc_t g1, const float* partial, int nb,
                                                                 float* sums_out, bf16_raw* dy_hi, int h1, float inv_keep,
                                                                 float* amax, int iters) {
    __shared__ float ssum[2][BWD_SLAB];
    __shared__ float smax[4];
    const int tid = threadIdx.x, lane = tid & 63, wave = tid >> 6;
    const int G = d.C >> 3, nslabs = d.C / BWD_SLAB;
    const int slab = blockIdx.x % nslabs, chunk = blockIdx.x / nslabs;
    const int cgl = lane & 7, rr = lane >> 3;
    const int cg = slab * (BWD_SLAB / 8) + cgl, c = cg * 8;
    const int T = d.T, N = d.N;
    const int64_t rows = (int64_t)N * T;
    RowCur q;
    rowcur_init(q, d, g1, ((int64_t)chunk * 4 + wave) * ((int64_t)iters * 8) + rr, c, cg, G);
    bf16_raw* pdy = dy_hi + ((int64_t)h1 + (int64_t)q.n * (T + h1) + q.t) * d.C + c;
    FastRow cur, nxt;
    fast_row_load_cur(d, g1, q, q.row < rows, cur);
    if (tid < 2 * BWD_SLAB) {
        const int k = tid >> 6, cc = tid & 63;
        float a = 0.f;
        int j = 0;
        for (; j + 8 <= nb; j += 8) {
            float v[8];
#pragma unroll
            for (int u = 0; u < 8; ++u) v[u] = partial[((int64_t)(j + u) * 2 + k) * d.C + slab * BWD_SLAB + cc];
#pragma unroll
            for (int u = 0; u < 8; ++u) a += v[u];
        }
        for (; j < nb; ++j) a += partial[((int64_t)j * 2 + k) * d.C + slab * BWD_SLAB + cc];
        ssum[k][cc] = a;
        if (chunk == 0) sums_out[(int64_t)k * d.C + slab * BWD_SLAB + cc] = a;
    }
    __syncthreads();
    Chan ch;
    load_chan(ch, d.scale, d.shift, d.mean, d.invstd, c);
    const float invM = 1.f / ((float)N * (float)T);
    float sg[8], sgx[8];
#pragma unroll
    for (int j = 0; j < 8; ++j) { sg[j] = ssum[0][cgl * 8 + j] * invM; sgx[j] = ssum[1][cgl * 8 + j] * invM; }
    float mx = 0.f;
    for (int it = 0; it < iters; ++it) {
        bf16_raw* const pdy_cur = pdy;
        pdy += (int64_t)(q.t + 8 >= T ? 8 + h1 : 8) * d.C;
        rowcur_step(q, d, g1, G);
        fast_row_load_cur(d, g1, q, it + 1 < iters && q.row < rows, nxt);
        if (cur.live) {
            float g[8], xh[8], o[8];
            fast_row_eval<ACT, DROP>(cur, ch, inv_keep, g, xh);
            if (d.mean) {
#pragma unroll
                for (int j = 0; j < 8; ++j) o[j] = ch.sc[j] * (g[j] - sg[j] - xh[j] * sgx[j]);
            } else {
#pragma unroll
                for (int j = 0; j < 8; ++j) o[j] = g[j] * ch.sc[j];
            }
            store8_split(pdy_cur, nullptr, 0, o);
            if (amax) {
#pragma unroll
                for (int j = 0; j < 8; ++j) mx = fmaxf(mx, fabsf(o[j]));
            }
        }
        cur = nxt;
    }
    if (h1 > 0) {
        const int nchunks = gridDim.x / nslabs;
        float z[8];
#pragma unroll
        for (int j = 0; j < 8; ++j) z[j] = 0.f;
        const int total = h1 * (N + 1);
        const int per = (total + nchunks - 1) / nchunks;
        int e = (chunk + 1) * per;
        if (e > total) e = total;
        for (int hr = chunk * per + wave * 8 + rr; hr < e; hr += 32) {
            const int gap = hr / h1, rw = hr - gap * h1;
            store8_split(dy_hi, nullptr, ((int64_t)gap * (T + h1) + rw) * d.C + c, z);
        }
    }
    if (amax) {
#pragma unroll
        for (int m = 1; m < 64; m <<= 1) mx = fmaxf(mx, __shfl_xor(mx, m, 64));
        if (lane == 0) smax[wave] = mx;
        __syncthreads();
        if (tid == 0) amax_publish(amax, blockIdx.x & (AMAX_SLOTS - 1), fmaxf(fmaxf(smax[0], smax[1]), fmaxf(smax[2], smax[3])));
    }
}

__global__ __launch_bounds__(256) void quantize_e4m3_dyn_kernel(const bf16_raw* src, int64_t ngroups, const float* amax,
                                                                 uint8_t* dst, float* inv_scale) {
    float a = amax[threadIdx.x & (AMAX_SLOTS - 1)];
#pragma unroll
    for (int m = 1; m < 64; m <<= 1) a = fmaxf(a, __shfl_xor(a, m, 64));
    const float scale = a > 0.f ? exp2f(floorf(log2f(224.f / a))) : 1.f;
    if (blockIdx.x == 0 && threadIdx.x == 0) inv_scale[0] = 1.f / scale;
    for (int64_t i = (int64_t)blockIdx.x * 256 + threadIdx.x; i < ngroups; i += (int64_t)gridDim.x * 256) {
        float v[8];
        load8<false>(src, i * 8, v);
        *reinterpret_cast<uint2*>(dst + i * 8) = quant8_e4m3(v, scale);
    }
}

__global__ __launch_bounds__(256) void bn_finalize_kernel(const float* partial, int ntiles, int C, double count,
                                                          const float* gamma, const float* beta, float eps, float momentum,
                                                          float* running_mean, float* running_var, float* mean,
                                                          float* invstd, float* scale, float* shift) {
    __shared__ double red1[8][33], red2[8][33];
    const int cx = threadIdx.x & 31, ly = threadIdx.x >> 5;
    const int c = blockIdx.x * 32 + cx;
    double s1 = 0.0, s2 = 0.0;
    if (partial && c < C) {
        int t = ly;
        for (; t + 56 < ntiles; t += 64) {
            float a[8], b[8];
#pragma unroll
            for (int u = 0; u < 8; ++u) {
                a[u] = partial[(int64_t)(t + 8 * u) * 2 * C + c];
                b[u] = partial[(int64_t)(t + 8 * u) * 2 * C + C + c];
            }
#pragma unroll
            for (int u = 0; u < 8; ++u) { s1 += a[u]; s2 += b[u]; }
        }
        for (; t < ntiles; t += 8) {
            s1 += partial[(int64_t)t * 2 * C + c];
            s2 += partial[(int64_t)t * 2 * C + C + c];
        }
    }
    red1[ly][cx] = s1;
    red2[ly][cx] = s2;
    __syncthreads();
    if (ly != 0 || c >= C) return;
    float m, istd;
    if (partial) {
        s1 = 0.0; s2 = 0.0;
#pragma unroll
        for (int k = 0; k < 8; ++k) { s1 += red1[k][cx]; s2 += red2[k][cx]; }
        const double mu = s1 / count;
        double var = s2 / count - mu * mu;
        if (var < 0.0) var = 0.0;
        m = (float)mu;
        istd = (float)(1.0 / sqrt(var + (double)eps));
        if (running_mean) {
            const double unbiased = count > 1.0 ? var * count / (count - 1.0) : var;
            running_mean[c] = (1.f - momentum) * running_mean[c] + momentum * m;
            running_var[c] = (1.f - momentum) * running_var[c] + momentum * (float)unbiased;
        }
    } else {
        m = running_mean[c];
        istd = 1.f / sqrtf(running_var[c] + eps);
    }
    const float g = gamma ? gamma[c] : 1.f, b = beta ? beta[c] : 0.f;
    if (mean) { mean[c] = m; invstd[c] = istd; }
    scale[c] = g * istd;
    shift[c] = b - m * g * istd;
}

int elementwise_blocks(int64_t items) {
    int64_t b = (items + 255) / 256;
    return (int)(b < 1 ? 1 : (b > 4096 ? 4096 : b));
}

int check_desc(const w2l_bnact_t* d, const char* who) {
    W2L_CHECK_ARG(d && d->y, "%s: null descriptor / y", who);
    W2L_CHECK_ARG(d->N > 0 && d->T > 0 && d->C > 0 && d->C % 8 == 0 && d->C <= 2048, "%s: bad N/T/C (%d,%d,%d)", who,
                  d->N, d->T, d->C);
    W2L_CHECK_ARG(d->drop_p >= 0.f && d->drop_p < 1.f, "%s: dropout p must be in [0,1)", who);
    W2L_CHECK_ARG(d->drop_p == 0.f || d->mask, "%s: dropout needs a mask buffer", who);
    W2L_CHECK_ARG((d->scale == nullptr) == (d->shift == nullptr), "%s: scale/shift must come together", who);
    return 0;
}

}

extern "C" int w2l_bn_finalize(const float* partial, int ntiles, int C, int64_t count, const float* gamma,
                               const float* beta, float eps, float momentum, float* running_mean, float* running_var,
                               float* mean, float* invstd, float* scale, float* shift, void* stream) {
    W2L_CHECK_ARG(scale && shift && C > 0, "bn_finalize: null output");
    W2L_CHECK_ARG(partial || (running_mean && running_var), "bn_finalize: eval mode needs running stats");
    W2L_CHECK_ARG(!partial || (ntiles > 0 && count > 0), "bn_finalize: bad tile count");
    hipLaunchKernelGGL(bn_finalize_kernel, dim3((C + 31) / 32), dim3(256), 0, (hipStream_t)stream, partial, ntiles, C,
                       (double)count, gamma, beta, eps, momentum, running_mean, running_var, mean, invstd, scale, shift);
    W2L_CHECK_LAUNCH();
    return 0;
}

extern "C" int w2l_bn_act_fwd(const w2l_bnact_t* d, void* out_hi, void* out_lo, int out_rows, int pad_l, int pad_r,
                              int pad_mode, void* stream) {
    return w2l_bn_act_fwd_q(d, out_hi, out_lo, nullptr, 1.f, out_rows, pad_l, pad_r, pad_mode, stream);
}

extern "C" int w2l_quantize_e4m3(const void* src, int src_f32, int64_t n, float scale, void* dst, void* stream) {
    W2L_CHECK_ARG(src && dst && n > 0 && n % 8 == 0 && scale > 0.f, "quantize_e4m3: bad arguments (n must be a multiple of 8)");
    hipLaunchKernelGGL(quantize_e4m3_kernel, dim3(elementwise_blocks(n / 8)), dim3(256), 0, (hipStream_t)stream, src, src_f32,
                       n / 8, scale, (uint8_t*)dst);
    W2L_CHECK_LAUNCH();
    return 0;
}

extern "C" int w2l_bn_act_fwd_q(const w2l_bnact_t* d, void* out_hi, void* out_lo, void* out_q, float q_scale, int out_rows,
                                int pad_l, int pad_r, int pad_mode, void* stream) {
    if (int e = check_desc(d, "bn_act_fwd")) return e;
    W2L_CHECK_ARG(!out_q || q_scale > 0.f, "bn_act_fwd: the e4m3 copy needs a positive scale");
    W2L_CHECK_ARG(out_hi && out_rows >= pad_l + d->T + pad_r && pad_l >= 0 && pad_r >= 0, "bn_act_fwd: bad output geometry");
    W2L_CHECK_ARG(pad_mode != 1 || (pad_l < d->T && pad_r < d->T), "bn_act_fwd: reflect pad (%d,%d) needs pad < T=%d",
                  pad_l, pad_r, d->T);
    const uint32_t thresh = (uint32_t)(d->drop_p * 65536.f);
    const float inv_keep = 1.f / (1.f - d->drop_p);
    W2L_CHECK_ARG((int64_t)d->N * out_rows * (d->C / 8) < (1LL << 31), "bn_act_fwd: tensor too large for 32-bit indexing");
    const int64_t per_utt = (int64_t)out_rows * (d->C / 8);
    W2L_CHECK_ARG(per_utt < (1 << 24) && d->N <= 65535, "bn_act_fwd: more than 2^24 channel groups per utterance or N > 65535");
    const dim3 grid((unsigned)((per_utt + 255) / 256), (unsigned)d->N);
    const float inv_g = 1.f / (float)(d->C / 8);
#define W2L_FWD_A(F, H, A)                                                                                   \
    hipLaunchKernelGGL((bn_act_fwd_kernel<F, H, A>), grid, dim3(256), 0, (hipStream_t)stream, *d,               \
                       (bf16_raw*)out_hi, (bf16_raw*)out_lo, out_rows, pad_l, pad_r, pad_mode, thresh, inv_keep,    \
                       (uint8_t*)out_q, q_scale, inv_g)
#define W2L_FWD(F, H) do { if (d->act == 1) W2L_FWD_A(F, H, 1); else if (d->act == 2) W2L_FWD_A(F, H, 2); else W2L_FWD_A(F, H, 0); } while (0)
    if (d->y_f32) { if (d->y2) W2L_FWD(true, true); else W2L_FWD(true, false); }
    else { if (d->y2) W2L_FWD(false, true); else W2L_FWD(false, false); }
#undef W2L_FWD
#undef W2L_FWD_A
    W2L_CHECK_LAUNCH();
    return 0;
}

extern "C" int w2l_bn_act_fwd_fin(const w2l_bnact_t* d, const w2l_bnfin_t* f1, const w2l_bnfin_t* f2, void* out_hi, void* out_q,
                                  float q_scale, int out_rows, int pad_l, int pad_r, int pad_mode, void* stream) {
    if (int e = check_desc(d, "bn_act_fwd_fin")) return e;
    W2L_CHECK_ARG(!d->y_f32, "bn_act_fwd_fin: bf16 y only (the fp32 mode takes w2l_bn_finalize + w2l_bn_act_fwd)");
    W2L_CHECK_ARG(d->C % BWD_SLAB == 0, "bn_act_fwd_fin: C=%d must be a multiple of %d", d->C, BWD_SLAB);
    W2L_CHECK_ARG(f1 && (f2 != nullptr) == (d->y2 != nullptr), "bn_act_fwd_fin: one finalize record per branch");
    W2L_CHECK_ARG(!out_q || q_scale > 0.f, "bn_act_fwd_fin: the e4m3 copy needs a positive scale");
    W2L_CHECK_ARG(out_hi && out_rows >= pad_l + d->T + pad_r && pad_l >= 0 && pad_r >= 0, "bn_act_fwd_fin: bad output geometry");
    W2L_CHECK_ARG(pad_mode != 1 || (pad_l < d->T && pad_r < d->T), "bn_act_fwd_fin: reflect pad (%d,%d) needs pad < T=%d", pad_l,
                  pad_r, d->T);
    FinBranch b[2];
    const w2l_bnfin_t* fs[2] = {f1, f2};
    for (int i = 0; i < 2; ++i) {
        FinBranch& o = b[i];
        const w2l_bnfin_t* f = fs[i];
        o = FinBranch{nullptr, 0, 1.0, nullptr, nullptr, 0.f, 0.f, nullptr, nullptr, nullptr, nullptr, nullptr, nullptr};
        if (!f) continue;
        W2L_CHECK_ARG(!f->partial || (f->rows > 0 && f->count > 0 && f->scale && f->shift), "bn_act_fwd_fin: bad finalize record");
        o = FinBranch{f->partial, f->rows, (double)f->count, f->gamma, f->beta, f->eps, f->momentum, f->running_mean, f->running_var,
                      f->mean, f->invstd, f->scale, f->shift};
    }
    const uint32_t thresh = (uint32_t)(d->drop_p * 65536.f);
    const float inv_keep = 1.f / (1.f - d->drop_p);
    const int64_t rows = (int64_t)d->N * out_rows;
    W2L_CHECK_ARG(rows * (d->C / 8) < (1LL << 31), "bn_act_fwd_fin: tensor too large for 32-bit indexing");
    const int rpb = fwd_rows_per_block(rows, d->C);
    const int nchunks = (int)((rows + rpb - 1) / rpb);
    const dim3 grid((unsigned)(nchunks * (d->C / BWD_SLAB)));
#define W2L_FIN_A(H, A)                                                                                                      \
    hipLaunchKernelGGL((bn_act_fwd_fin_kernel<H, A>), grid, dim3(256), 0, (hipStream_t)stream, *d, b[0], b[1], (bf16_raw*)out_hi, \
                       out_rows, pad_l, pad_r, pad_mode, thresh, inv_keep, (uint8_t*)out_q, q_scale, rpb)
#define W2L_FIN(H) do { if (d->act == 1) W2L_FIN_A(H, 1); else if (d->act == 2) W2L_FIN_A(H, 2); else W2L_FIN_A(H, 0); } while (0)
    if (d->y2) W2L_FIN(true); else W2L_FIN(false);
#undef W2L_FIN
#undef W2L_FIN_A
    W2L_CHECK_LAUNCH();
    return 0;
}

extern "C" int w2l_bn_bwd_blocks(int N, int T, int C) {
    if (N <= 0 || T <= 0 || C < BWD_SLAB) return 0;
    const int64_t rows = (int64_t)N * T;
    const int rw = bwd_rows_per_wave(rows, C);
    return (int)((rows + rw - 1) / rw);
}

#define W2L_DISPATCH_BWD2(KERNEL, H2, ...)                                                                 \
    do {                                                                                                   \
        if (d->y_f32 && g1->f32) hipLaunchKernelGGL((KERNEL<true, true, H2>), __VA_ARGS__);                \
        else if (d->y_f32) hipLaunchKernelGGL((KERNEL<true, false, H2>), __VA_ARGS__);                     \
        else if (g1->f32) hipLaunchKernelGGL((KERNEL<false, true, H2>), __VA_ARGS__);                      \
        else hipLaunchKernelGGL((KERNEL<false, false, H2>), __VA_ARGS__);                                  \
    } while (0)
#define W2L_DISPATCH_BWD(KERNEL, ...)                                                                      \
    do {                                                                                                   \
        if (d->y2) W2L_DISPATCH_BWD2(KERNEL, true, __VA_ARGS__);                                           \
        else W2L_DISPATCH_BWD2(KERNEL, false, __VA_ARGS__);                                                \
    } while (0)

extern "C" int w2l_bn_act_bwd_reduce(const w2l_bnact_t* d, const w2l_gradsrc_t* g1, const w2l_gradsrc_t* g2,
                                     float* partial, void* stream) {
    if (int e = check_desc(d, "bn_act_bwd_reduce")) return e;
    W2L_CHECK_ARG(g1 && g1->dxp && partial, "bn_act_bwd_reduce: null pointer");
    W2L_CHECK_ARG(!g2 || g2->f32 == g1->f32, "bn_act_bwd_reduce: gradient sources must share a dtype");
    W2L_CHECK_ARG(g1->rows >= g1->pad_l + d->T + g1->pad_r && (!g2 || g2->rows >= g2->pad_l + d->T + g2->pad_r),
                  "bn_act_bwd_reduce: gradient source has too few rows per utterance");
    W2L_CHECK_ARG(d->C % BWD_SLAB == 0, "bn_act_bwd_reduce: C=%d must be a multiple of %d", d->C, BWD_SLAB);
    const int64_t rows = (int64_t)d->N * d->T;
    const int rw = bwd_rows_per_wave(rows, d->C);
    const int nchunks = w2l_bn_bwd_blocks(d->N, d->T, d->C);
    const int tasks = nchunks * (d->C / BWD_SLAB);
    const float inv_keep = 1.f / (1.f - d->drop_p);
    w2l_gradsrc_t g2v = g2 ? *g2 : *g1;
    W2L_DISPATCH_BWD(bn_act_bwd_reduce_kernel, dim3((tasks + 3) / 4), dim3(256), 0, (hipStream_t)stream, *d, *g1, g2v,
                     g2 ? 1 : 0, partial, inv_keep, rw, nchunks);
    W2L_CHECK_LAUNCH();
    return 0;
}

static bool bwd_fast_ok(const w2l_bnact_t* d, const w2l_gradsrc_t* g1, const w2l_gradsrc_t* g2) {
    return !d->y_f32 && !d->y2 && g1 && !g1->f32 && g2 == nullptr && d->C % BWD_SLAB == 0 && d->scale != nullptr;
}

static int bn_loop_iters(int64_t rows, int T, int C) {
    static const int forced = getenv("W2L_BN_LOOP_ITERS") ? atoi(getenv("W2L_BN_LOOP_ITERS")) : -1;
    int it = forced >= 0 ? forced : ((rows >= 12000 && rows * C >= 8000000) ? 4 : 0);
    if (T < 8) it = 0;
    while (it > 1 && rows < 4LL * it * 8 * 4) it >>= 1;
    return it;
}

extern "C" int w2l_bn_bwd_fast_ok(const w2l_bnact_t* d, const w2l_gradsrc_t* g1, const w2l_gradsrc_t* g2) {
    return d && bwd_fast_ok(d, g1, g2) ? 1 : 0;
}

extern "C" int w2l_bn_act_bwd_reduce_slots(const w2l_bnact_t* d, const w2l_gradsrc_t* g1, float* partial, int slots, void* stream) {
    if (int e = check_desc(d, "bn_act_bwd_reduce_slots")) return e;
    W2L_CHECK_ARG(g1 && g1->dxp && partial && slots >= 1 && slots <= 64, "bn_act_bwd_reduce_slots: null pointer / slots not in 1..64");
    W2L_CHECK_ARG(bwd_fast_ok(d, g1, nullptr), "bn_act_bwd_reduce_slots: bf16 y and gradient, one branch, one source, C %% 64 == 0 only");
    W2L_CHECK_ARG(g1->rows >= g1->pad_l + d->T + g1->pad_r, "bn_act_bwd_reduce_slots: gradient source has too few rows per utterance");
    const int64_t rows = (int64_t)d->N * d->T;
    const float inv_keep = 1.f / (1.f - d->drop_p);
    const bool drop = d->drop_p > 0.f;
    const int iters = bn_loop_iters(rows, d->T, d->C);
    if (iters > 0) {
        const int nch = (int)((rows + 4LL * iters * 8 - 1) / (4LL * iters * 8));
        const dim3 lgrid((unsigned)(nch * (d->C / BWD_SLAB)));
#define W2L_REDL(A, D) hipLaunchKernelGGL((bn_bwd_reduce_loop_kernel<A, D>), lgrid, dim3(256), 0, (hipStream_t)stream, *d, *g1, partial, inv_keep, slots, iters)
        switch (d->act) {
            case 1: if (drop) W2L_REDL(1, true); else W2L_REDL(1, false); break;
            case 2: if (drop) W2L_REDL(2, true); else W2L_REDL(2, false); break;
            default: if (drop) W2L_REDL(0, true); else W2L_REDL(0, false); break;
        }
#undef W2L_REDL
        W2L_CHECK_LAUNCH();
        return 0;
    }
    constexpr int U = 2;
    const int nchunks = (int)((rows + 4 * U * 8 - 1) / (4 * U * 8));
    const dim3 grid((unsigned)(nchunks * (d->C / BWD_SLAB)));
#define W2L_RED(A, D) hipLaunchKernelGGL((bn_bwd_reduce_fast_kernel<U, A, D>), grid, dim3(256), 0, (hipStream_t)stream, *d, *g1, partial, inv_keep, slots)
    switch (d->act) {
        case 1: if (drop) W2L_RED(1, true); else W2L_RED(1, false); break;
        case 2: if (drop) W2L_RED(2, true); else W2L_RED(2, false); break;
        default: if (drop) W2L_RED(0, true); else W2L_RED(0, false); break;
    }
#undef W2L_RED
    W2L_CHECK_LAUNCH();
    return 0;
}

extern "C" int w2l_bn_act_bwd_apply_slots(const w2l_bnact_t* d, const w2l_gradsrc_t* g1, const float* partial, int nrows, float* sums,
                                          void* dy_hi, int halo, float* amax, void* stream) {
    if (int e = check_desc(d, "bn_act_bwd_apply_slots")) return e;
    W2L_CHECK_ARG(g1 && g1->dxp && dy_hi && partial && sums && nrows > 0 && halo >= 0, "bn_act_bwd_apply_slots: null pointer / no partial rows");
    W2L_CHECK_ARG(bwd_fast_ok(d, g1, nullptr), "bn_act_bwd_apply_slots: bf16 y and gradient, one branch, one source, C %% 64 == 0 only");
    W2L_CHECK_ARG(g1->rows >= g1->pad_l + d->T + g1->pad_r, "bn_act_bwd_apply_slots: gradient source has too few rows per utterance");
    const int64_t rows = (int64_t)d->N * d->T;
    W2L_CHECK_ARG((rows + (int64_t)halo * (d->N + 1)) * (d->C / 8) < (1LL << 31), "bn_act_bwd_apply_slots: tensor too large for 32-bit indexing");
    const float inv_keep = 1.f / (1.f - d->drop_p);
    const int iters = bn_loop_iters(rows, d->T, d->C);
    if (iters > 0) {
        const int nch = (int)((rows + 4LL * iters * 8 - 1) / (4LL * iters * 8));
        const dim3 lgrid((unsigned)(nch * (d->C / BWD_SLAB)));
        const bool dropl = d->drop_p > 0.f;
#define W2L_APPL(A, D) hipLaunchKernelGGL((bn_bwd_apply_loop_kernel<A, D>), lgrid, dim3(256), 0, (hipStream_t)stream, *d, *g1, partial, nrows, sums, (bf16_raw*)dy_hi, halo, inv_keep, amax, iters)
        switch (d->act) {
            case 1: if (dropl) W2L_APPL(1, true); else W2L_APPL(1, false); break;
            case 2: if (dropl) W2L_APPL(2, true); else W2L_APPL(2, false); break;
            default: if (dropl) W2L_APPL(0, true); else W2L_APPL(0, false); break;
        }
#undef W2L_APPL
        W2L_CHECK_LAUNCH();
        return 0;
    }
    const int U = amax ? 4 : (d->C <= 384 ? 2 : 1);
    const int nchunks = (int)((rows + 4 * U * 8 - 1) / (4 * U * 8));
    const dim3 grid((unsigned)(nchunks * (d->C / BWD_SLAB)));
#define W2L_APP(UU, A, D) hipLaunchKernelGGL((bn_bwd_apply_fast_kernel<UU, A, D>), grid, dim3(256), 0, (hipStream_t)stream, *d, *g1, partial, nrows, sums, (bf16_raw*)dy_hi, halo, inv_keep, amax)
#define W2L_APP_U(A, D) do { if (U == 4) W2L_APP(4, A, D); else if (U == 2) W2L_APP(2, A, D); else W2L_APP(1, A, D); } while (0)
    const bool drop = d->drop_p > 0.f;
    switch (d->act) {
        case 1: if (drop) W2L_APP_U(1, true); else W2L_APP_U(1, false); break;
        case 2: if (drop) W2L_APP_U(2, true); else W2L_APP_U(2, false); break;
        default: if (drop) W2L_APP_U(0, true); else W2L_APP_U(0, false); break;
    }
#undef W2L_APP_U
#undef W2L_APP
    W2L_CHECK_LAUNCH();
    return 0;
}

extern "C" int w2l_bn_bwd_finalize(const float* partial, int nblocks, int C, int ncomp, float* sums, void* stream) {
    W2L_CHECK_ARG(partial && sums && nblocks > 0 && C > 0 && (ncomp == 2 || ncomp == 4), "bn_bwd_finalize: bad arguments");
    hipLaunchKernelGGL(bn_bwd_finalize_kernel, dim3((ncomp * C + 31) / 32), dim3(256), 0, (hipStream_t)stream, partial,
                       nblocks, ncomp * C, sums);
    W2L_CHECK_LAUNCH();
    return 0;
}

extern "C" int w2l_bn_act_bwd_apply(const w2l_bnact_t* d, const w2l_gradsrc_t* g1, const w2l_gradsrc_t* g2,
                                    const float* sums, void* dy_hi, void* dy_lo, int halo, void* dy2_hi, void* dy2_lo,
                                    int halo2, void* stream) {
    return w2l_bn_act_bwd_apply_amax(d, g1, g2, sums, dy_hi, dy_lo, halo, dy2_hi, dy2_lo, halo2, nullptr, stream);
}

extern "C" int w2l_bn_act_bwd_apply_fin(const w2l_bnact_t* d, const w2l_gradsrc_t* g1, const w2l_gradsrc_t* g2,
                                        const float* partial, int nblocks, float* sums, void* dy_hi, void* dy_lo, int halo,
                                        void* dy2_hi, void* dy2_lo, int halo2, float* amax, void* stream) {
    if (int e = check_desc(d, "bn_act_bwd_apply_fin")) return e;
    W2L_CHECK_ARG(g1 && g1->dxp && dy_hi && partial && sums && nblocks > 0, "bn_act_bwd_apply_fin: null pointer / no partial rows");
    W2L_CHECK_ARG(d->C % BWD_SLAB == 0, "bn_act_bwd_apply_fin: C=%d must be a multiple of %d", d->C, BWD_SLAB);
    W2L_CHECK_ARG(!g2 || g2->f32 == g1->f32, "bn_act_bwd_apply_fin: gradient sources must share a dtype");
    W2L_CHECK_ARG(halo >= 0 && halo2 >= 0, "bn_act_bwd_apply_fin: negative halo");
    W2L_CHECK_ARG(g1->rows >= g1->pad_l + d->T + g1->pad_r && (!g2 || g2->rows >= g2->pad_l + d->T + g2->pad_r),
                  "bn_act_bwd_apply_fin: gradient source has too few rows per utterance");
    const int64_t rows = (int64_t)d->N * d->T;
    W2L_CHECK_ARG((rows + (int64_t)(halo + halo2) * (d->N + 1)) * (d->C / 8) < (1LL << 31),
                  "bn_act_bwd_apply_fin: tensor too large for 32-bit indexing");
    const int rpb = apply_rows_per_block(rows, d->C);
    const int nchunks = (int)((rows + rpb - 1) / rpb);
    const int blocks = nchunks * (d->C / BWD_SLAB);
    const float inv_keep = 1.f / (1.f - d->drop_p);
    w2l_gradsrc_t g2v = g2 ? *g2 : *g1;
    W2L_DISPATCH_BWD(bn_act_bwd_apply_fin_kernel, dim3(blocks), dim3(256), 0, (hipStream_t)stream, *d, *g1, g2v, g2 ? 1 : 0,
                     partial, nblocks, sums, (bf16_raw*)dy_hi, (bf16_raw*)dy_lo, halo, (bf16_raw*)dy2_hi, (bf16_raw*)dy2_lo,
                     halo2, inv_keep, amax, rpb);
    W2L_CHECK_LAUNCH();
    return 0;
}

extern "C" int w2l_quantize_e4m3_dyn(const void* src_bf16, int64_t n, const float* amax, void* dst, float* inv_scale,
                                     void* stream) {
    W2L_CHECK_ARG(src_bf16 && dst && amax && inv_scale && n > 0 && n % 8 == 0, "quantize_e4m3_dyn: bad arguments");
    hipLaunchKernelGGL(quantize_e4m3_dyn_kernel, dim3(elementwise_blocks(n / 8)), dim3(256), 0, (hipStream_t)stream,
                       (const bf16_raw*)src_bf16, n / 8, amax, (uint8_t*)dst, inv_scale);
    W2L_CHECK_LAUNCH();
    return 0;
}

extern "C" int w2l_bn_act_bwd_apply_amax(const w2l_bnact_t* d, const w2l_gradsrc_t* g1, const w2l_gradsrc_t* g2,
                                         const float* sums, void* dy_hi, void* dy_lo, int halo, void* dy2_hi, void* dy2_lo,
                                         int halo2, float* amax, void* stream) {
    if (int e = check_desc(d, "bn_act_bwd_apply")) return e;
    W2L_CHECK_ARG(g1 && g1->dxp && dy_hi, "bn_act_bwd_apply: null pointer");
    W2L_CHECK_ARG(!d->mean || sums, "bn_act_bwd_apply: BatchNorm backward needs the reduced sums");
    W2L_CHECK_ARG(!g2 || g2->f32 == g1->f32, "bn_act_bwd_apply: gradient sources must share a dtype");
    W2L_CHECK_ARG(halo >= 0 && halo2 >= 0, "bn_act_bwd_apply: negative halo");
    W2L_CHECK_ARG(g1->rows >= g1->pad_l + d->T + g1->pad_r && (!g2 || g2->rows >= g2->pad_l + d->T + g2->pad_r),
                  "bn_act_bwd_apply: gradient source has too few rows per utterance");
    const int G = d->C / 8;
    const int64_t items = (int64_t)d->N * d->T * G + (int64_t)halo * (d->N + 1) * G +
                          (dy2_hi ? (int64_t)halo2 * (d->N + 1) * G : 0);
    W2L_CHECK_ARG(items < (1LL << 31), "bn_act_bwd_apply: tensor too large for 32-bit indexing");
    const int blocks = elementwise_blocks(items);
    const float inv_keep = 1.f / (1.f - d->drop_p);
    w2l_gradsrc_t g2v = g2 ? *g2 : *g1;
    W2L_DISPATCH_BWD(bn_act_bwd_apply_kernel, dim3(blocks), dim3(256), 0, (hipStream_t)stream, *d, *g1, g2v, g2 ? 1 : 0,
                     sums, (bf16_raw*)dy_hi, (bf16_raw*)dy_lo, halo, (bf16_raw*)dy2_hi, (bf16_raw*)dy2_lo, halo2,
                     inv_keep, amax);
    W2L_CHECK_LAUNCH();
    return 0;
}
```

wav2letter_pytorch_amd/engine.py:

```python
from __future__ import annotations

import atexit
import ctypes as C
import math
import os
from dataclasses import dataclass, field
from typing import Callable, List, NamedTuple, Optional, Sequence, Tuple

import torch

from . import _lib
from . import wgrad_groups as WG
from ._lib import BnActDesc, BnActEpi, GradSrc, check, lib, ptr, stream_ptr

ACT_NONE, ACT_CLAMP20, ACT_RELU = 0, 1, 2
PAD_ZERO, PAD_REFLECT = 0, 1


def _none():
    return None


class _Volatile(dict):

    def __reduce__(self):
        return (_none, ())

    def __deepcopy__(self, memo):
        return None


class _nullctx:
    def __enter__(self):
        return None

    def __exit__(self, *a):
        return False


def roundup(x: int, m: int) -> int:
    return (x + m - 1) // m * m


def zeros(shape, dtype, device) -> torch.Tensor:
    t = torch.empty(shape, dtype=dtype, device=device)
    if t.is_cuda:
        check(lib.w2l_fill_zero(ptr(t), t.numel() * t.element_size(), stream_ptr()), 'w2l_fill_zero')
    else:
        t.zero_()
    return t


def zero_(t: torch.Tensor) -> torch.Tensor:
    if t.is_cuda and t.is_contiguous():
        check(lib.w2l_fill_zero(ptr(t), t.numel() * t.element_size(), stream_ptr()), 'w2l_fill_zero')
    else:
        t.zero_()
    return t


def _py(fn, *args):
    rec = _lib.recording()
    if rec is None:
        return fn(*args)
    rec.python(fn, *args, stream=torch.cuda.current_stream())


def padded_channels(c: int) -> int:
    return roundup(c, 64)


@dataclass
class ConvSpec:
    weight: torch.Tensor
    bias: Optional[torch.Tensor]
    kernel: int
    stride: int
    dilation: int
    pad_l: int
    pad_r: int
    pad_mode: int
    bn_weight: Optional[torch.Tensor] = None
    bn_bias: Optional[torch.Tensor] = None
    running_mean: Optional[torch.Tensor] = None
    running_var: Optional[torch.Tensor] = None
    num_batches_tracked: Optional[torch.Tensor] = None
    eps: float = 1e-3
    momentum: float = 0.1
    name: str = ''

    @property
    def has_bn(self) -> bool:
        return self.bn_weight is not None

    def out_len(self, T: int) -> int:
        return (T + self.pad_l + self.pad_r - (self.kernel - 1) * self.dilation - 1) // self.stride + 1

    @property
    def cout(self) -> int:
        return self.weight.shape[0]

    @property
    def cin(self) -> int:
        return self.weight.shape[1]

    def params(self) -> List[torch.Tensor]:
        out = [self.weight]
        if self.bias is not None:
            out.append(self.bias)
        if self.has_bn:
            out += [self.bn_weight, self.bn_bias]
        return out


@dataclass
class UnitSpec:
    main: ConvSpec
    src: int
    act: int = ACT_NONE
    drop_p: float = 0.0
    dw: Optional[ConvSpec] = None
    res: Optional[ConvSpec] = None
    res_src: Optional[int] = None
    update_lens: bool = False
    mask_out: bool = False


@dataclass
class Act:
    hi: torch.Tensor
    lo: Optional[torch.Tensor]
    N: int
    T: int
    C: int
    CP: int
    pad_l: int
    pad_r: int
    pad_mode: int
    lens: Optional[torch.Tensor] = None
    q: Optional[torch.Tensor] = None
    q_scale: float = 1.0

    @property
    def rows(self) -> int:
        return self.pad_l + self.T + self.pad_r


@dataclass
class _PackedW:
    version: int
    fwd_hi: torch.Tensor
    fwd_lo: Optional[torch.Tensor]
    dgr_hi: torch.Tensor
    dgr_lo: Optional[torch.Tensor]
    cinp: int
    coutp: int
    src_ptr: int = 0
    ready: Optional['_lib.Event'] = None


@dataclass
class _UnitCtx:
    unit: UnitSpec
    y: torch.Tensor = None
    y2: Optional[torch.Tensor] = None
    Tout: int = 0
    scale: Optional[torch.Tensor] = None
    shift: Optional[torch.Tensor] = None
    mean: Optional[torch.Tensor] = None
    invstd: Optional[torch.Tensor] = None
    scale2: Optional[torch.Tensor] = None
    shift2: Optional[torch.Tensor] = None
    mean2: Optional[torch.Tensor] = None
    invstd2: Optional[torch.Tensor] = None
    mask: Optional[torch.Tensor] = None
    seed: int = 0
    offset: int = 0
    out_index: int = 0
    lens_out: Optional[torch.Tensor] = None
    mid: Optional['Act'] = None
    keep: list = field(default_factory=list)


class _GradSource(NamedTuple):
    buf: torch.Tensor
    pad_l: int
    pad_r: int
    pad_mode: int
    per: int
    partial: Optional[torch.Tensor] = None


def _row_ptr(t: torch.Tensor, rows: int, width: int, esize: int) -> C.c_void_p:
    return C.c_void_p(t.data_ptr() + rows * width * esize)


@dataclass(eq=False, slots=True)
class _WgradJob:
    conv: ConvSpec
    pk: _PackedW
    dy_hi: torch.Tensor
    dy_lo: Optional[torch.Tensor]
    halo: int
    Tout: int
    src: Act
    f8: Optional[tuple] = None
    token: Optional[int] = None
    order: int = 0
    at: Optional[int] = None

    @property
    def N(self) -> int:
        return self.src.N

    @property
    def row_off(self) -> int:
        return self.src.pad_l - self.conv.pad_l

    @property
    def x_bstride(self) -> int:
        return self.src.rows * self.src.CP

    @property
    def x_rows_total(self) -> int:
        return self.src.N * self.src.rows - self.row_off

    @property
    def dy_bstride(self) -> int:
        return (self.Tout + self.halo) * self.pk.coutp

    @property
    def dw_shape(self) -> Tuple[int, int, int]:
        return (self.conv.kernel, self.pk.coutp, self.pk.cinp)

    @property
    def flops(self) -> float:
        return 2.0 * self.src.N * self.Tout * self.conv.cout * self.conv.cin * self.conv.kernel

    def dy_ptr(self, t: torch.Tensor, esize: int) -> C.c_void_p:
        return _row_ptr(t, self.halo, self.pk.coutp, esize)

    def x_ptr(self, t: torch.Tensor, esize: int) -> C.c_void_p:
        return _row_ptr(t, self.row_off, self.src.CP, esize)

    def held(self) -> tuple:
        ts = (self.dy_hi, self.dy_lo, self.src.hi, self.src.lo) + ((self.src.q,) + self.f8 if self.f8 else ())
        return tuple(t for t in ts if t is not None)


_dropout_calls = 0
AUTOTUNE = os.environ.get('W2L_AUTOTUNE', '1') != '0'
_tuned_shapes = set()
TUNE_REPS = int(os.environ.get('W2L_TUNE_REPS', '2'))
TUNE_CACHE = os.environ.get('W2L_TUNE_CACHE') or None
_tune_state = {'dirty': False}


def _tune_once(key, why=None) -> bool:
    if key in _tuned_shapes:
        return False
    _tuned_shapes.add(key)
    _tune_state['dirty'] = True
    if why is not None:
        _lib.poison(why)
    return True
_wgroup_plans = {}
_wgroup_forms = {}


def load_tune_cache(path: str) -> int:
    n = lib.w2l_tune_load(path.encode())
    if n < 0:
        check(1, 'w2l_tune_load')
    with open(path) as f:
        for line in f:
            t = line.split()
            if len(t) == 6 and t[0] == 'wgroup':
                try:
                    layers = tuple(tuple(int(v) for v in l.split(',')) for l in t[5].split(';'))
                    _wgroup_forms[(layers, int(t[1]), int(t[2]), int(t[3]))] = int(t[4])
                    n += 1
                except ValueError:
                    pass
    return n


def save_tune_cache(path: str):
    tmp = '%s.tmp.%d' % (path, os.getpid())
    check(lib.w2l_tune_save(tmp.encode()), 'w2l_tune_save')
    with open(tmp, 'a') as f:
        for (layers, n, tout, dil), form in sorted(_wgroup_forms.items()):
            f.write('wgroup %d %d %d %d %s\n' % (n, tout, dil, form, ';'.join(','.join(str(v) for v in l) for l in layers)))
    os.replace(tmp, path)


def _flush_tune_cache():
    if _tune_state['dirty'] and TUNE_CACHE:
        save_tune_cache(TUNE_CACHE)
    _tune_state['dirty'] = False


if TUNE_CACHE and os.path.exists(TUNE_CACHE):
    load_tune_cache(TUNE_CACHE)
atexit.register(_flush_tune_cache)

AFTER_FORWARD: list = []

KERNEL_TIMER: Optional[list] = None


class _timed:
    def __init__(self, name, flops):
        self.name, self.flops = name, flops

    def __enter__(self):
        if KERNEL_TIMER is not None:
            self.s = torch.cuda.Event(enable_timing=True)
            self.e = torch.cuda.Event(enable_timing=True)
            self.s.record()

    def __exit__(self, *a):
        if KERNEL_TIMER is not None:
            self.e.record()
            KERNEL_TIMER.append((self.name, self.flops, self.s, self.e))


def _phys_strides(w: torch.Tensor):
    return w.stride(0), w.stride(1), w.stride(2)
# ... 19 lines not shown
                return hit
        cout, cin, kw = w.shape
        s_co, s_ci, s_kw = _phys_strides(w)
        check(lib.w2l_pack_weights(ptr(w), s_co, s_ci, s_kw, cout, cin, kw, hit.coutp, hit.cinp, ptr(hit.fwd_hi), ptr(hit.fwd_lo),
                                   ptr(hit.dgr_hi), ptr(hit.dgr_lo), stream_ptr()), 'w2l_pack_weights')
        hit.version, hit.ready = w._version, None
        return hit
    cout, cin, kw = w.shape
    coutp, cinp = padded_channels(cout), padded_channels(cin)
    dev = w.device
    if recording:
        _lib.poison('operand pack buffers created')
    fwd_hi = torch.empty(kw, coutp, cinp, dtype=torch.bfloat16, device=dev)
    dgr_hi = torch.empty(kw, cinp, coutp, dtype=torch.bfloat16, device=dev)
    fwd_lo = torch.empty_like(fwd_hi) if precise else None
    dgr_lo = torch.empty_like(dgr_hi) if precise else None
    s_co, s_ci, s_kw = _phys_strides(w)
    check(lib.w2l_pack_weights(ptr(w), s_co, s_ci, s_kw, cout, cin, kw, coutp, cinp, ptr(fwd_hi), ptr(fwd_lo),
                               ptr(dgr_hi), ptr(dgr_lo), stream_ptr()), 'w2l_pack_weights')
    pk = _PackedW(w._version, fwd_hi, fwd_lo, dgr_hi, dgr_lo, cinp, coutp, w.data_ptr())
    cache[precise] = pk
    return pk


def weight_event(w) -> '_lib.Event':
    ev = w.__dict__.get('_w2l_ready_ev')
    if ev is None:
        ev = w.__dict__['_w2l_ready_ev'] = _lib.Event()
        _wev_epoch[0] += 1
    return ev


_wev_epoch = [0]
_in_forward = [False]


FUSED_INFER = os.environ.get('W2L_FUSED_INFER', '1') != '0'
_infer_epoch = [0]


def infer_copies(units: Sequence['UnitSpec'], has_head: bool, fp8: bool, cp0: int) -> List[Tuple[bool, bool]]:
    out = []
    for ai in range(len(units) + 1):
        cp = cp0 if ai == 0 else padded_channels(units[ai - 1].main.cout)
        dense1 = [u.dw is None and u.main.stride == 1 for u in units if u.src == ai]
        dense1 += [u.res.stride == 1 for u in units if u.res is not None and u.res_src == ai]
        q = bool(fp8 and ai > 0 and cp % 128 == 0 and any(dense1))
        hi = (has_head and ai == len(units)) or any(not (q and d) for d in dense1)
        out.append((bool(hi or not q), q))
    return out


def bnact_rows(t: int, T: int, pad_l: int, pad_r: int, reflect: bool) -> List[int]:
    rows = [pad_l + t]
    if reflect:
        if 1 <= t <= pad_l:
            rows.append(pad_l - t)
        j = T - 1 - t
        if 1 <= j <= pad_r:
            rows.append(pad_l + T - 1 + j)
    return rows


def bnact_zero_rows(T: int, pad_l: int, pad_r: int) -> List[int]:
    return list(range(pad_l)) + [pad_l + T + j for j in range(pad_r)]


def fold_bn(gamma, beta, running_mean, running_var, eps: float):
    istd = 1.0 / torch.sqrt(running_var.float() + eps)
    scale = gamma.float() * istd
    return scale, beta.float() - running_mean.float() * gamma.float() * istd


def drop_infer_state():
    _infer_epoch[0] += 1


def invalidate_packed(params) -> int:
    if isinstance(params, torch.nn.Module):
        params = params.parameters()
    drop_infer_state()
    n = 0
    for p in params:
        cache = getattr(p, '_w2l_pack', None)
        if cache:
            for pk in cache.values():
                pk.version = -1
            n += 1
    return n


def _padded_vec(v: Optional[torch.Tensor], cp: int, fill: float) -> Optional[torch.Tensor]:
    if v is None:
        return None
    v = v.detach()
    if v.dtype != torch.float32:
        _lib.poison('a per-channel vector that is not fp32')
        v = v.float()
    if v.numel() == cp and v.is_contiguous():
        return v
    if v.is_cuda and v.is_contiguous():
        out = torch.empty(cp, dtype=torch.float32, device=v.device)
        check(lib.w2l_pad_vec_f32(ptr(v), v.numel(), ptr(out), cp, float(fill), stream_ptr()), 'w2l_pad_vec_f32')
        return out
    out = torch.full((cp,), fill, dtype=torch.float32, device=v.device)
    out[: v.numel()] = v
    return out


SPLITK_WS_CAP = 1 << 30
_splitk_ws = {}


def _splitk_workspace(dev, n, cout, tout):
    need = min(int(lib.w2l_conv_splitk_workspace_bytes(n, cout, tout)), SPLITK_WS_CAP)
    ws = _splitk_ws.get(dev.index)
    if ws is None or ws.numel() < need:
        if ws is not None:
            _retired_ws.append(ws)
        _lib.poison('split-K workspace grown')
        ws = torch.zeros(need, dtype=torch.uint8, device=dev)
        _splitk_ws[dev.index] = ws
    return ws


_side_streams = {}


def _side_stream(dev, main=None) -> 'torch.cuda.Stream':
    st = _side_streams.get(dev.index)
    if st is None:
        from .streams import concurrent_stream
        _lib.poison('side stream created')
        st = concurrent_stream(dev, 'wgrad', main=main)
        _side_streams[dev.index] = st
    return st


WGROUP_MAX = int(os.environ.get('W2L_WGRAD_GROUP_MAX', '3'))
_wgrad_ws = {}
_retired_ws = []
DETERMINISTIC_WGRAD = os.environ.get('W2L_DETERMINISTIC', '0') == '1'
lib.w2l_wgrad_deterministic(int(DETERMINISTIC_WGRAD))
DEALT_WGRAD = os.environ.get('W2L_DEALT_WGRAD', '1') == '1'
DEFER_SPREAD = os.environ.get('W2L_DEFER_SPREAD', 'start')
WGRAD_AFTER_DGRAD = os.environ.get('W2L_WGRAD_AFTER_DGRAD', '0') == '1'
FUSED_BN_REDUCE = os.environ.get('W2L_FUSED_BN_REDUCE', '0')
FUSED_BN_REDUCE_MAX_ROWS = 12288
FOLD_BN_FINALIZE = os.environ.get('W2L_FOLD_BN_FINALIZE', '0') == '1'
FOLD_BN_FWD = os.environ.get('W2L_FOLD_BN_FWD', 'auto')
FOLD_BN_FWD_MAX_ROWS = 12288
FAST_BN_BWD = os.environ.get('W2L_FAST_BN_BWD', '1') == '1'
STAT_SLOTS = int(os.environ.get('W2L_STAT_SLOTS', '8'))


def _wgrad_workspace(dev, cin, cout, kw):
    if DETERMINISTIC_WGRAD:
        need = min(int(lib.w2l_wgrad_workspace_bytes(cin, cout, kw)), SPLITK_WS_CAP)
    else:
        need = min(int(lib.w2l_wgrad_dealt_workspace_bytes(cin, cout, kw)), SPLITK_WS_CAP)
        if need == 0:
            return None
    ws = _wgrad_ws.get(dev.index)
    if ws is None or ws.numel() < need:
        if ws is not None:
            _retired_ws.append(ws)
        _lib.poison('weight-gradient workspace grown')
        ws = torch.zeros(need, dtype=torch.uint8, device=dev)
        _wgrad_ws[dev.index] = ws
    return ws


def _igemm(x: Act, row_off: int, w_hi, w_lo, y, bias, stats, Cin, Cout, Tout, Kw, stride, dil, precise, alg_flops=0.0):
    n = x.N
    bstride = x.rows * x.CP
    rows_total = n * x.rows - row_off
    esz = 2

    def xptr(t):
        return C.c_void_p(t.data_ptr() + row_off * x.CP * esz)

    st = stream_ptr()
    if not precise:
        ws = _splitk_workspace(x.hi.device, n, Cout, Tout)
        if AUTOTUNE:
            key = (n, Cin, Cout, Tout, Kw, stride, dil, stats is not None, x.hi.device.index)
            if _tune_once(key, 'measuring launches'):
                check(lib.w2l_conv1d_igemm_tune_ws(xptr(x.hi), bstride, rows_total, ptr(w_hi), ptr(y),
                                                   int(y.dtype == torch.float32), ptr(bias), ptr(stats), n, Cin, Cout, Tout,
                                                   Kw, stride, dil, TUNE_REPS, ptr(ws), ws.numel(), st), 'w2l_conv1d_igemm_tune_ws')
                if stats is not None and stats.shape[0] <= 64:
                    stats.zero_()
        with _timed('conv_igemm_kernel', alg_flops):
            check(lib.w2l_conv1d_igemm_ws(xptr(x.hi), bstride, rows_total, ptr(w_hi), ptr(y), int(y.dtype == torch.float32),
                                          0, ptr(bias), ptr(stats), n, Cin, Cout, Tout, Kw, stride, dil, ptr(ws), ws.numel(),
                                          st), 'w2l_conv1d_igemm_ws')
        return
    assert y.dtype == torch.float32
    check(lib.w2l_conv1d_igemm(xptr(x.hi), bstride, rows_total, ptr(w_hi), ptr(y), 1, 0, ptr(bias), None, n, Cin, Cout,
                               Tout, Kw, stride, dil, st), 'w2l_conv1d_igemm')
    check(lib.w2l_conv1d_igemm(xptr(x.hi), bstride, rows_total, ptr(w_lo), ptr(y), 1, 1, None, None, n, Cin, Cout, Tout,
                               Kw, stride, dil, st), 'w2l_conv1d_igemm')
    check(lib.w2l_conv1d_igemm(xptr(x.lo), bstride, rows_total, ptr(w_hi), ptr(y), 1, 1, None, ptr(stats), n, Cin, Cout,
                               Tout, Kw, stride, dil, st), 'w2l_conv1d_igemm')


FP8_ACT_SCALE = {ACT_CLAMP20: 16.0, ACT_RELU: 8.0, ACT_NONE: 8.0}
FP8_WEIGHT_RESCALE = 256
FP8_RESCALE_LAG = 8
AMAX_SLOTS = 64
FP8_DGRAD = os.environ.get('W2L_FP8_DGRAD', 'auto')
FP8_DGRAD_MIN_ROWS = 3072
FP8_WGRAD = os.environ.get('W2L_FP8_WGRAD', 'auto')
JOIN_EVENTS = None


_fp8_epoch = [0]


def _pow2_scale(amax: float) -> float:
    return 2.0 ** math.floor(math.log2(448.0 / max(float(amax), 1e-30)))


def _fp8_weights(conv: ConvSpec, pk: '_PackedW', dgrad: bool = False):
    w = conv.weight
    st = w.__dict__.get('_w2l_fp8')
    if st is None or st['q'].shape != pk.fwd_hi.shape or st['q'].device != pk.fwd_hi.device:
        _lib.poison('fp8 weight scale: first use')
        mn, mx = torch.aminmax(pk.fwd_hi)
        scale = _pow2_scale(max(-float(mn), float(mx)))
        dev = pk.fwd_hi.device
        st = _Volatile({'q': torch.empty(pk.fwd_hi.shape, dtype=torch.uint8, device=dev),
                        'qd': torch.empty(pk.dgr_hi.shape, dtype=torch.uint8, device=dev), 'scale': scale, 'age': 0,
                        'version': None, 'version_d': None, 'req': None})
        w.__dict__['_w2l_fp8'] = st
    elif not dgrad and not torch.cuda.is_current_stream_capturing():
        req = st.get('req')
        if req is not None and st['age'] >= FP8_RESCALE_LAG:
            ev, host = req
            ev.synchronize()
            _lib.poison('fp8 weight scale: adoption point')
            st['req'] = None
            scale = _pow2_scale(max(-float(host[0]), float(host[1])))
            if scale != st['scale']:
                st['scale'] = scale
                _fp8_epoch[0] += 1
                st['version'] = st['version_d'] = None
        elif req is None and st['age'] >= FP8_WEIGHT_RESCALE:
            _lib.poison('fp8 weight scale: amax request')
            host = torch.empty(2, dtype=torch.float32, pin_memory=True)
            host.copy_(torch.stack(torch.aminmax(pk.fwd_hi)).float(), non_blocking=True)
            ev = torch.cuda.Event()
            ev.record()
            st['req'] = (ev, host)
            st['age'] = 0
    key, vkey, src = ('qd', 'version_d', pk.dgr_hi) if dgrad else ('q', 'version', pk.fwd_hi)
    if st[vkey] != pk.version:
        check(lib.w2l_quantize_e4m3(ptr(src), 0, src.numel(), st['scale'], ptr(st[key]), stream_ptr()), 'w2l_quantize_e4m3')
        st[vkey] = pk.version
        if not dgrad:
            st['age'] += 1
    return st[key], st['scale']


class StackEngine:

    def __init__(self, units: Sequence[UnitSpec], head: Optional[ConvSpec], n_labels: int, precise: bool = False,
                 fp8: bool = False):
        if fp8 and precise:
            raise ValueError('fp8 operands and the fp32 parity mode exclude each other')
        self.fp8 = fp8
        """``head`` = the classifier conv followed by (log_)softmax; ``None`` runs an OPEN stack whose result is the last
        unit's activation as fp32 [N, C, T'] (stand-alone Conv1dBlock / MaskedConv1d / JasperBlock modules)."""
        self.units = list(units)
        self.head = head
        self.n_labels = n_labels
        self.precise = precise
        self.grad_ready: Optional[Callable] = None
        self.flat_ready: Optional[Callable] = None
        self.backward_done: Optional[Callable[[], None]] = None
        self.overlap_wgrad = True
        self._side = None
        self._main_stream = None
        self._side_used = False
        self._held: list = []
        self._dyq: dict = {}
        self._nbt_pending: list = []
        self._zero_pool = None
        self.dropout_counter: Optional[torch.Tensor] = None
        self._q_clipped: Optional[torch.Tensor] = None
        self.defer_wgrad = 0
        self.deferred = None
        self.grad_reduce_start: Optional[Callable] = None
        self._deferred: list = []
        self._wg_of: dict = {}
        self._wg_pending: dict = {}

    def parameters(self) -> List[torch.Tensor]:
        out = []
        for u in self.units:
            if u.dw is not None:
                out += u.dw.params()
            out += u.main.params()
            if u.res is not None:
                out += u.res.params()
        if self.head is not None:
            out += self.head.params()
        return out

    def _in_pad_for(self, act_index: int):
        pl = pr = 0
        mode = PAD_ZERO
        convs = []
        for u in self.units:
            if u.src == act_index:
                convs.append(u.dw if u.dw is not None else u.main)
            if u.res is not None and u.res_src == act_index:
                convs.append(u.res)
        if act_index == len(self.units) and self.head is not None:
            convs.append(self.head)
        for c in convs:
            if c.pad_l > pl or c.pad_r > pr:
                pl, pr = max(pl, c.pad_l), max(pr, c.pad_r)
            if c.pad_l or c.pad_r:
                mode = c.pad_mode
        return pl, pr, mode

    def forward(self, x: torch.Tensor, lens: Optional[torch.Tensor], training: bool, softmax_mode: int = 0,
                want_input_grad: bool = False):
        _in_forward[0] = True
        try:
            return self._forward(x, lens, training, softmax_mode, want_input_grad)
        finally:
            _in_forward[0] = False
            lib.w2l_conv_stats_mode(0)
            self._stat_pool = None

    def _forward(self, x, lens, training, softmax_mode, want_input_grad):
        _lib.require_device(x)
        global _dropout_calls
        if training:
            _infer_epoch[0] += 1
        if self._deferred:
            self.flush_deferred(pos=0)
        precise = self.precise
        N, C0, T0 = x.shape
        fold = training and not precise and x.is_cuda and not DETERMINISTIC_WGRAD and (
            FOLD_BN_FWD in ('1', True) or (FOLD_BN_FWD == 'auto' and self.units and
                                           N * T0 // max(1, self.units[0].main.stride) < FOLD_BN_FWD_MAX_ROWS))
        self._stat_pool = None
        self._after_apply = []
        if fold:
            need = 0
            for u in self.units:
                for c in (u.main, u.res):
                    if c is not None and c.has_bn:
                        need += STAT_SLOTS * 2 * padded_channels(c.cout)
            fold = need > 0
            if fold:
                self._stat_pool = [zeros(need, torch.float32, x.device), 0]
        lib.w2l_conv_stats_mode(STAT_SLOTS if fold else 0)
        x = x.contiguous().float()
        dev = x.device
        st = stream_ptr
        ctx = {'units': [], 'acts': [], 'training': training, 'x_shape': (N, C0, T0), 'want_dx': bool(want_input_grad)}
        lens_dev, mid_lens, out_lens, lens_final = self._plan_lens(lens, dev)
        pl, pr, mode = self._in_pad_for(0)
        cp0 = padded_channels(C0)
        a_hi = torch.empty(N, pl + T0 + pr, cp0, dtype=torch.bfloat16, device=dev)
        a_lo = torch.empty_like(a_hi) if precise else None
        if lens_dev is not None and not any((u.src == 0 and u.update_lens) for u in self.units):
            in_mask = None
        else:
            in_mask = lens_dev
        check(lib.w2l_nct_to_ntc(ptr(x), N, C0, T0, cp0, pl, pr, mode, ptr(in_mask), ptr(a_hi), ptr(a_lo), st()),
              'w2l_nct_to_ntc')
        acts: List[Act] = [Act(a_hi, a_lo, N, T0, C0, cp0, pl, pr, mode, in_mask)]
        if self.fp8 and self.head is None and self.units and cp0 % 128 == 0 and self._fp8_consumers(0):
            a0 = acts[0]
            a0.q = torch.empty(a_hi.shape, dtype=torch.uint8, device=dev)
            a0.q_scale = FP8_ACT_SCALE[self.units[0].act]
            check(lib.w2l_quantize_e4m3(ptr(a_hi), 0, a_hi.numel(), a0.q_scale, ptr(a0.q), st()), 'w2l_quantize_e4m3')

        for ui, u in enumerate(self.units):
            if ui and self._deferred:
                self.flush_deferred(pos=ui)
            uc = _UnitCtx(unit=u)
            src = acts[u.src]
            conv = u.main
            if u.dw is not None:
                dwc = u.dw
                src = self._dw_forward(dwc, src, mid_lens[ui])
                uc.mid = src
            y, stats, Tout = self._conv_forward(conv, src, need_stats=conv.has_bn and training)
            uc.y, uc.Tout = y, Tout
            coutp = y.shape[2]
            fins = [None, None]
            if conv.has_bn:
                if fold:
                    fins[0], (uc.scale, uc.shift, uc.mean, uc.invstd) = self._bn_fin_record(conv, stats, N * Tout, coutp)
                else:
                    uc.scale, uc.shift, uc.mean, uc.invstd = self._bn_finalize(conv, stats, N * Tout, coutp, training)
            if u.res is not None:
                rsrc = acts[u.res_src]
                y2, stats2, Tout2 = self._conv_forward(u.res, rsrc, need_stats=u.res.has_bn and training)
                if Tout2 != Tout or y2.shape != y.shape:
                    raise ValueError('residual branch shape mismatch')
                uc.y2 = y2
                if u.res.has_bn:
                    if fold:
                        fins[1], (uc.scale2, uc.shift2, uc.mean2, uc.invstd2) = self._bn_fin_record(u.res, stats2, N * Tout, coutp)
                    else:
                        uc.scale2, uc.shift2, uc.mean2, uc.invstd2 = self._bn_finalize(u.res, stats2, N * Tout, coutp, training)
            uc.lens_out = out_lens[ui]
            opl, opr, omode = self._in_pad_for(ui + 1)
            out_hi = torch.empty(N, opl + Tout + opr, coutp, dtype=torch.bfloat16, device=dev)
            out_lo = torch.empty_like(out_hi) if precise else None
            p = u.drop_p if training else 0.0
            if p > 0.0:
                uc.mask = torch.empty(N * Tout * (coutp // 8), dtype=torch.uint8, device=dev)
                uc.seed = torch.initial_seed() & 0xFFFFFFFFFFFFFFFF
                if self.dropout_counter is not None:
                    uc.offset = ui + 1
                else:
                    _dropout_calls += 1
                    uc.offset = _dropout_calls
            d = self._desc(uc, N, Tout, coutp, p, uc.lens_out)
            out_q, q_scale = None, 1.0
            if self.fp8 and coutp % 128 == 0 and self._fp8_consumers(ui + 1):
                out_q = torch.empty(N, opl + Tout + opr, coutp, dtype=torch.uint8, device=dev)
                q_scale = FP8_ACT_SCALE[u.act]
                if self._q_clipped is None or self._q_clipped.device != dev:
                    _lib.poison('fp8 saturation counter created')
                    self._q_clipped = torch.zeros(1, dtype=torch.int64, device=dev)
                d.q_clipped = self._q_clipped.data_ptr()
            if fins[0] is not None or fins[1] is not None:
                f1 = fins[0] if fins[0] is not None else _lib.BnFin()
                f2 = (fins[1] if fins[1] is not None else _lib.BnFin()) if u.res is not None else None
                check(lib.w2l_bn_act_fwd_fin(C.byref(d), C.byref(f1), C.byref(f2) if f2 is not None else None, ptr(out_hi),
                                             ptr(out_q), q_scale, opl + Tout + opr, opl, opr, omode, st()), 'w2l_bn_act_fwd_fin')
                for rm, rv, rm_p, rv_p in self._after_apply:
                    _lib.poison('running statistics of a padded channel count')
                    rm.copy_(rm_p[: rm.numel()])
                    rv.copy_(rv_p[: rv.numel()])
                self._after_apply = []
            else:
                check(lib.w2l_bn_act_fwd_q(C.byref(d), ptr(out_hi), ptr(out_lo), ptr(out_q), q_scale, opl + Tout + opr, opl, opr,
                                           omode, st()), 'w2l_bn_act_fwd_q')
            uc.out_index = ui + 1
            acts.append(Act(out_hi, out_lo, N, Tout, conv.cout, coutp, opl, opr, omode, uc.lens_out, out_q, q_scale))
            ctx['units'].append(uc)

        if self._nbt_pending:
            self._bump_counters(self._nbt_pending)
            self._nbt_pending = []
        if fold:
            lib.w2l_conv_stats_mode(0)
            self._stat_pool = None
        ctx['acts'] = acts
        ctx['softmax_mode'] = softmax_mode
        ctx['lens_out'] = lens_final
        last = acts[-1]
        if self.head is None:
            _lib.poison('open stack')
            a = last.hi[:, last.pad_l:last.pad_l + last.T, :last.C].float()
            if last.lo is not None:
                a = a + last.lo[:, last.pad_l:last.pad_l + last.T, :last.C].float()
            ctx['out'] = a.transpose(1, 2).contiguous()
            return ctx['out'], ctx
        logits, _, Th = self._conv_forward(self.head, last, need_stats=False, force_f32=True)
        out = torch.empty(N, Th, self.n_labels, dtype=torch.float32, device=dev)
        check(lib.w2l_log_softmax_fwd(ptr(logits), N, Th, self.n_labels, logits.shape[2], softmax_mode, ptr(out), st()),
              'w2l_log_softmax_fwd')
        ctx['out'] = out
        for hook in list(AFTER_FORWARD):
            _py(hook)
        return out, ctx

    def infer(self, x: torch.Tensor, lens: Optional[torch.Tensor], softmax_mode: int = 0):
        if self.head is None:
            raise ValueError('infer() needs a stack with a classifier')
        if not FUSED_INFER:
            with torch.no_grad():
                out, ctx = self.forward(x, lens, False, softmax_mode)
            return out, ctx['lens_out']
        _in_forward[0] = True
        try:
            with torch.no_grad():
                return self._infer(x, lens, softmax_mode)
        finally:
            _in_forward[0] = False

    def _infer_affine(self, conv: ConvSpec, cp: int):
        srcs = (conv.bias, conv.bn_weight, conv.bn_bias, conv.running_mean, conv.running_var)
        key = (_infer_epoch[0], cp) + tuple((t.data_ptr(), t._version) if t is not None else None for t in srcs)
        cache = self.__dict__.setdefault('_infer_fold', {})
        hit = cache.get(id(conv))
        if hit is not None and hit[0] == key:
            return hit[1]
        bias = _padded_vec(conv.bias, cp, 0.0)
        scale = shift = None
        if conv.has_bn:
            scale, shift, _, _ = self._bn_finalize(conv, None, 1, cp, False)
        self.infer_folds = getattr(self, 'infer_folds', 0) + 1
        cache[id(conv)] = (key, (bias, scale, shift))
        return bias, scale, shift

    def _infer_conv(self, conv: ConvSpec, src: Act, epi: BnActEpi, Tout: int, out_q=None, q_scale: float = 1.0):
        pk = pack_weights(conv, self.precise, need_dgrad=False)
        if pk.cinp != src.CP:
            raise ValueError(f'channel mismatch: conv expects {pk.cinp} padded channels, activation has {src.CP}')
        bias, scale, shift = self._infer_affine(conv, pk.coutp)
        epi.scale, epi.shift = ptr(scale), ptr(shift)
        n, cin, cout, kw, stride, dil = src.N, pk.cinp, pk.coutp, conv.kernel, conv.stride, conv.dilation
        row_off = src.pad_l - conv.pad_l
        bstride, rows_total = src.rows * src.CP, n * src.rows - row_off
        st = stream_ptr()
        if self.fp8 and src.q is not None and stride == 1 and cin % 128 == 0:
            wq, w_scale = _fp8_weights(conv, pk)
            xq = C.c_void_p(src.q.data_ptr() + row_off * src.CP)
            dev = src.q.device
            if out_q is not None and (self._q_clipped is None or self._q_clipped.device != dev):
                self._q_clipped = torch.zeros(1, dtype=torch.int64, device=dev)
            if AUTOTUNE:
                key = ('bnact_fp8', n, cin, cout, Tout, kw, dil, dev.index)
                if _tune_once(key):
                    check(lib.w2l_conv1d_igemm_bnact_fp8_tune(xq, bstride, rows_total, ptr(wq), ptr(bias), C.byref(epi), ptr(out_q),
                                                              q_scale, n, cin, cout, Tout, kw, dil, TUNE_REPS, st),
                          'w2l_conv1d_igemm_bnact_fp8_tune')
            with _timed('conv_igemm_fp8_kernel', 2.0 * n * Tout * conv.cout * conv.cin * kw):
                check(lib.w2l_conv1d_igemm_bnact_fp8(xq, bstride, rows_total, ptr(wq), 1.0 / (src.q_scale * w_scale), ptr(bias),
                                                     C.byref(epi), ptr(out_q), q_scale,
                                                     ptr(self._q_clipped) if out_q is not None else None, n, cin, cout, Tout, kw,
                                                     dil, st), 'w2l_conv1d_igemm_bnact_fp8')
            return
        if src.hi is None or not epi.out_hi:
            raise RuntimeError('infer(): a bf16-operand launch without its bf16 buffers (buffer plan out of step)')
        self._infer_conv_bf16(conv, src, epi, Tout, pk, bias, row_off, bstride, rows_total, st)
        if out_q is not None:
            check(lib.w2l_quantize_e4m3(C.c_void_p(epi.out_hi), 0, n * epi.out_rows * cout, q_scale, ptr(out_q), st),
                  'w2l_quantize_e4m3')

    def _infer_conv_bf16(self, conv, src, epi, Tout, pk, bias, row_off, bstride, rows_total, st):
        n, cin, cout, kw, stride, dil = src.N, pk.cinp, pk.coutp, conv.kernel, conv.stride, conv.dilation

        def xptr(t):
            return C.c_void_p(t.data_ptr() + row_off * src.CP * 2)

        flops = 2.0 * n * Tout * conv.cout * conv.cin * kw
        if self.precise:
            scratch = self.__dict__.setdefault('_infer_acc', {})
            acc = scratch.get((n, Tout, cout, src.hi.device))
            if acc is None:
                acc = scratch[(n, Tout, cout, src.hi.device)] = torch.empty(n, Tout, cout, dtype=torch.float32,
                                                                            device=src.hi.device)
                self.infer_buffers = getattr(self, 'infer_buffers', 0) + 1
            check(lib.w2l_conv1d_igemm(xptr(src.hi), bstride, rows_total, ptr(pk.fwd_hi), ptr(acc), 1, 0, ptr(bias), None, n, cin,
                                       cout, Tout, kw, stride, dil, st), 'w2l_conv1d_igemm')
            check(lib.w2l_conv1d_igemm(xptr(src.hi), bstride, rows_total, ptr(pk.fwd_lo), ptr(acc), 1, 1, None, None, n, cin,
                                       cout, Tout, kw, stride, dil, st), 'w2l_conv1d_igemm')
            check(lib.w2l_conv1d_igemm_bnact(xptr(src.lo), bstride, rows_total, ptr(pk.fwd_hi), ptr(acc), None, C.byref(epi), n,
                                             cin, cout, Tout, kw, stride, dil, st), 'w2l_conv1d_igemm_bnact')
            return
        ws = _splitk_workspace(src.hi.device, n, cout, Tout)
        if AUTOTUNE:
            key = ('bnact', n, cin, cout, Tout, kw, stride, dil, src.hi.device.index)
            if _tune_once(key):
                check(lib.w2l_conv1d_igemm_bnact_tune_ws(xptr(src.hi), bstride, rows_total, ptr(pk.fwd_hi), ptr(bias),
                                                         C.byref(epi), n, cin, cout, Tout, kw, stride, dil, TUNE_REPS, ptr(ws),
                                                         ws.numel(), st), 'w2l_conv1d_igemm_bnact_tune_ws')
        with _timed('conv_igemm_kernel', flops):
            check(lib.w2l_conv1d_igemm_bnact_ws(xptr(src.hi), bstride, rows_total, ptr(pk.fwd_hi), None, ptr(bias), C.byref(epi),
                                                n, cin, cout, Tout, kw, stride, dil, ptr(ws), ws.numel(), st),
                  'w2l_conv1d_igemm_bnact_ws')

    def _infer(self, x, lens, softmax_mode):
        _lib.require_device(x)
        if self._deferred:
            self.flush_deferred()
# ... 209 lines not shown

    def _igemm_fp8(self, conv: ConvSpec, pk: _PackedW, src: Act, y, bias, stats, Tout, flops):
        wq, w_scale = _fp8_weights(conv, pk)
        N, cin, cout = src.N, pk.cinp, pk.coutp
        row_off = src.pad_l - conv.pad_l
        xq = C.c_void_p(src.q.data_ptr() + row_off * src.CP)
        bstride, rows_total = src.rows * src.CP, N * src.rows - row_off
        y_f32 = int(y.dtype == torch.float32)
        st = stream_ptr()
        if AUTOTUNE:
            key = ('fp8', N, cin, cout, Tout, conv.kernel, conv.dilation, stats is not None, src.q.device.index)
            if _tune_once(key):
                check(lib.w2l_conv1d_igemm_fp8_tune(xq, bstride, rows_total, ptr(wq), ptr(y), y_f32, ptr(bias), ptr(stats), N,
                                                    cin, cout, Tout, conv.kernel, conv.dilation, TUNE_REPS, st),
                      'w2l_conv1d_igemm_fp8_tune')
                if stats is not None and getattr(self, '_stat_pool', None) is not None:
                    stats.zero_()
        with _timed('conv_igemm_fp8_kernel', flops):
            check(lib.w2l_conv1d_igemm_fp8(xq, bstride, rows_total, ptr(wq), ptr(y), y_f32, 1.0 / (src.q_scale * w_scale), None,
                                           ptr(bias), ptr(stats), N, cin, cout, Tout, conv.kernel, conv.dilation, st),
                  'w2l_conv1d_igemm_fp8')

    @staticmethod
    def _dw_weight(dwc: ConvSpec, cp: int) -> torch.Tensor:
        w = dwc.weight.detach()
        c, _, k = w.shape
        km = w.permute(2, 0, 1).reshape(k, c)
        if cp == c and km.is_contiguous():
            return km
        _lib.poison('depthwise weight of a padded channel count')
        out = torch.zeros(k, cp, dtype=torch.float32, device=w.device)
        out[:, :c] = km
        return out

    def _dw_forward(self, dwc: ConvSpec, src: Act, lens_mid, out=None) -> Act:
        if src.pad_l < dwc.pad_l or src.pad_r < dwc.pad_r:
            raise ValueError('activation buffer is not padded enough for its depthwise consumer')
        N, cp = src.N, src.CP
        Tmid = dwc.out_len(src.T)
        dev = src.hi.device
        if out is not None:
            mid_hi, mid_lo = out
        else:
            mid_hi = torch.empty(N, Tmid, cp, dtype=torch.bfloat16, device=dev)
            mid_lo = torch.empty_like(mid_hi) if self.precise else None
        row_off = src.pad_l - dwc.pad_l
        off = row_off * cp * 2
        w = self._dw_weight(dwc, cp)
        check(lib.w2l_dwconv_fwd(C.c_void_p(src.hi.data_ptr() + off),
                                 C.c_void_p(src.lo.data_ptr() + off) if src.lo is not None else None, src.rows, ptr(w),
                                 ptr(mid_hi), ptr(mid_lo), N, Tmid, cp, dwc.kernel, dwc.stride, dwc.dilation, ptr(lens_mid),
                                 stream_ptr()), 'w2l_dwconv_fwd')
        return Act(mid_hi, mid_lo, N, Tmid, dwc.cout, cp, 0, 0, PAD_ZERO, lens_mid)

    def _dw_backward(self, dwc: ConvSpec, dmid, src: Act, mid: Act, need_dx: bool, grads):
        g, per = dmid.buf, dmid.per
        N, cp = src.N, src.CP
        dev = g.device
        row_off = src.pad_l - dwc.pad_l
        k = dwc.kernel
        dwg = zeros((k, cp), torch.float32, dev)
        check(lib.w2l_dwconv_wgrad(ptr(g), int(g.dtype == torch.float32), per, _row_ptr(src.hi, row_off, cp, 2),
                                   _row_ptr(src.lo, row_off, cp, 2) if src.lo is not None else None, src.rows, ptr(dwg), N,
                                   mid.T, cp, k, dwc.stride, dwc.dilation, ptr(mid.lens), stream_ptr()), 'w2l_dwconv_wgrad')
        c = dwc.cout
        gw = dwg.view(k, cp, 1).permute(1, 2, 0)
        self._set(grads, dwc.weight, gw if cp == c else gw[:c], storage=dwg)
        if not need_dx:
            return None
        Tp = src.T + dwc.pad_l + dwc.pad_r
        tmid, lens_mid = mid.T, mid.lens
        if dwc.stride != 1:
            _lib.poison('strided depthwise data gradient')
            s_ = dwc.stride
            tup = (mid.T - 1) * s_ + 1
            up = torch.zeros(N, tup, cp, dtype=g.dtype, device=dev)
            up[:, 0:tup:s_] = g.view(N, per, cp)[:, :mid.T]
            g, per, tmid = up, tup, tup
            if lens_mid is not None:
                lens_mid = ((lens_mid - 1) * s_ + 1).clamp(min=0).to(torch.int32)
        dxp = torch.empty(N, Tp, cp, dtype=torch.float32 if self.precise else torch.bfloat16, device=dev)
        w = self._dw_weight(dwc, cp)
        check(lib.w2l_dwconv_dgrad(ptr(g), int(g.dtype == torch.float32), per, ptr(w), ptr(dxp),
                                   int(dxp.dtype == torch.float32), N, Tp, tmid, cp, k, dwc.dilation, ptr(lens_mid),
                                   stream_ptr()), 'w2l_dwconv_dgrad')
        return _GradSource(dxp, dwc.pad_l, dwc.pad_r, dwc.pad_mode, Tp)

    def _bn_finalize(self, conv: ConvSpec, stats, count, cp, training):
        dev = conv.weight.device
        scale, shift, mean, invstd = torch.empty(4, cp, dtype=torch.float32, device=dev).unbind(0)
        gamma = _padded_vec(conv.bn_weight, cp, 1.0)
        beta = _padded_vec(conv.bn_bias, cp, 0.0)
        rm, rv = conv.running_mean, conv.running_var
        padded_running = rm is not None and rm.numel() != cp
        if padded_running:
            rm_p, rv_p = _padded_vec(rm, cp, 0.0).clone(), _padded_vec(rv, cp, 1.0).clone()
        else:
            rm_p, rv_p = rm, rv
        if training:
            ntiles = stats.shape[0]
            check(lib.w2l_bn_finalize(ptr(stats), ntiles, cp, count, ptr(gamma), ptr(beta), conv.eps, conv.momentum,
                                      ptr(rm_p), ptr(rv_p), ptr(mean), ptr(invstd), ptr(scale), ptr(shift),
                                      stream_ptr()), 'w2l_bn_finalize')
            if padded_running:
                _lib.poison('running statistics of a padded channel count')
                rm.copy_(rm_p[: rm.numel()])
                rv.copy_(rv_p[: rv.numel()])
            if conv.num_batches_tracked is not None:
                self._nbt_pending.append(conv.num_batches_tracked)
        else:
            check(lib.w2l_bn_finalize(None, 0, cp, 1, ptr(gamma), ptr(beta), conv.eps, conv.momentum, ptr(rm_p),
                                      ptr(rv_p), ptr(mean), ptr(invstd), ptr(scale), ptr(shift), stream_ptr()),
                  'w2l_bn_finalize')
        return scale, shift, mean, invstd

    def _bn_fin_record(self, conv: ConvSpec, stats, count, cp):
        dev = conv.weight.device
        scale, shift, mean, invstd = torch.empty(4, cp, dtype=torch.float32, device=dev).unbind(0)
        gamma = _padded_vec(conv.bn_weight, cp, 1.0)
        beta = _padded_vec(conv.bn_bias, cp, 0.0)
        rm, rv = conv.running_mean, conv.running_var
        if rm is not None and rm.numel() != cp:
            rm_p, rv_p = _padded_vec(rm, cp, 0.0).clone(), _padded_vec(rv, cp, 1.0).clone()
            self._after_apply.append((rm, rv, rm_p, rv_p))
        else:
            rm_p, rv_p = rm, rv
        f = _lib.BnFin()
        f.partial, f.rows, f.count = stats.data_ptr(), stats.shape[0], count
        f.gamma, f.beta = gamma.data_ptr(), beta.data_ptr()
        f.eps, f.momentum = conv.eps, conv.momentum
        f.running_mean = rm_p.data_ptr() if rm_p is not None else None
        f.running_var = rv_p.data_ptr() if rv_p is not None else None
        f.mean, f.invstd, f.scale, f.shift = mean.data_ptr(), invstd.data_ptr(), scale.data_ptr(), shift.data_ptr()
        f._keep = (gamma, beta, rm_p, rv_p, stats)
        if conv.num_batches_tracked is not None:
            self._nbt_pending.append(conv.num_batches_tracked)
        return f, (scale, shift, mean, invstd)

    def _desc(self, uc: _UnitCtx, N, T, cp, p, lens, constant_stats: bool = False) -> BnActDesc:
        d = BnActDesc()
        d.N, d.T, d.C = N, T, cp
        d.y = uc.y.data_ptr()
        d.y_f32 = int(uc.y.dtype == torch.float32)
        for name in ('scale', 'shift', 'mean', 'invstd', 'scale2', 'shift2', 'mean2', 'invstd2'):
            t = getattr(uc, name)
            if constant_stats and name in ('mean', 'invstd', 'mean2', 'invstd2'):
                t = None
            setattr(d, name, t.data_ptr() if t is not None else None)
        d.y2 = uc.y2.data_ptr() if uc.y2 is not None else None
        d.act = uc.unit.act
        d.drop_p = float(p)
        d.seed, d.offset = uc.seed, uc.offset
        d.mask = uc.mask.data_ptr() if uc.mask is not None else None
        d.lens = lens.data_ptr() if lens is not None else None
        d.offset_dev = self.dropout_counter.data_ptr() if (self.dropout_counter is not None and p > 0.0) else None
        uc.keep.append(lens)
        return d

    def backward(self, ctx, g_out: torch.Tensor):
        try:
            return self._backward(ctx, g_out)
        finally:
            lib.w2l_conv_stats_mode(0)
            self._slot_pool = None

    def _backward(self, ctx, g_out: torch.Tensor):
        acts: List[Act] = ctx['acts']
        out = ctx['out']
        N = out.shape[0]
        dev = out.device
        grads = {}
        batch_stats = bool(ctx['training'])
        self._main_stream = torch.cuda.current_stream(dev) if dev.type == 'cuda' else None
        pool_elems = roundup(self.head.cout, 64) if self.head is not None else 0
        for uc in ctx['units']:
            if uc.unit.main.has_bn or (uc.unit.res is not None and uc.unit.res.has_bn):
                pool_elems += 4 * acts[uc.out_index].CP
        slot_need = 0
        if FAST_BN_BWD and not DETERMINISTIC_WGRAD and batch_stats and not self.precise and dev.type == 'cuda':
            slot_need = sum(STAT_SLOTS * 2 * acts[uc.out_index].CP for uc in ctx['units'] if uc.unit.main.has_bn and uc.unit.res is None)
        bias_need = 0
        if batch_stats:
            for u in self.units:
                for c in (u.main, u.res):
                    if c is not None and c.bias is not None and c.has_bn:
                        bias_need += roundup(c.cout, 64)
        zbuf = zeros(pool_elems + slot_need + bias_need, torch.float32, dev)
        small_pool = zbuf[:pool_elems]
        pool_off = 0
        self._slot_pool = [zbuf[pool_elems: pool_elems + slot_need], 0, {}] if slot_need else None
        self._zero_pool = [zbuf[pool_elems + slot_need:], 0] if bias_need else None
        lib.w2l_conv_stats_mode(STAT_SLOTS if self._slot_pool is not None else 0)
        lib.w2l_wgrad_deterministic(int(DETERMINISTIC_WGRAD))
        act_grads: List[List[_GradSource]] = [[] for _ in acts]
        if self.head is None:
            last = acts[-1]
            _lib.poison('open stack')
            gp = torch.zeros(N, last.T, last.CP, dtype=torch.float32, device=dev)
            gp[:, :, :last.C] = g_out.float().transpose(1, 2)
            act_grads[len(acts) - 1].append(_GradSource(gp, 0, 0, PAD_ZERO, last.T))
        else:
            self._plan_wgrad_groups(ctx)
            pool_off = self._head_backward(ctx, g_out, small_pool, grads, act_grads)
        self._units_backward(ctx, act_grads, small_pool, pool_off, grads, batch_stats)
        for recs in list(self._wg_pending.values()):
            for r in recs:
                self._wgrad_single(r, grads)
        self._wg_pending.clear()
        self._wg_of = {}
        ctx['input_grad'] = self.input_grad(ctx, act_grads[0]) if ctx.get('want_dx') and act_grads[0] else None
        if self.flat_ready is not None:
            _py(self.flat_ready, small_pool)
        elif self.grad_ready is not None:
            _py(self.grad_ready, None, small_pool, small_pool)
        if self._side_used:
            if JOIN_EVENTS is not None:
                em, es = torch.cuda.Event(enable_timing=True), torch.cuda.Event(enable_timing=True)
                em.record(self._main_stream)
                es.record(self._side)
                JOIN_EVENTS.append((em, es))
            _lib.stream_wait_stream(self._main_stream, self._side)
            self._side_used = False
        self._main_stream = None
        self._held.clear()
        self._dyq.clear()
        self._zero_pool = None
        self._slot_pool = None
        lib.w2l_conv_stats_mode(0)
        _flush_tune_cache()
        if self.backward_done is not None:
            _py(self.backward_done)
        return [grads.get(id(p)) for p in self.parameters()]

    def _head_backward(self, ctx, g_out, small_pool, grads, act_grads) -> int:
        precise = self.precise
        acts: List[Act] = ctx['acts']
        out = ctx['out']
        N, Th, L = out.shape
        dev = out.device
        st = stream_ptr
        pool_off = 0
        g_out = g_out.contiguous().float()
        glog = torch.empty_like(out)
        check(lib.w2l_log_softmax_bwd(ptr(g_out), ptr(out), N, Th, L, ctx['softmax_mode'], ptr(glog), st()),
              'w2l_log_softmax_bwd')
        head = self.head
        pk = pack_weights(head, precise)
        hh = roundup(Th, 64) - Th
        dy_hi = torch.empty(hh + N * (Th + hh), pk.coutp, dtype=torch.bfloat16, device=dev)
        dy_lo = torch.empty_like(dy_hi) if precise else None
        colsum = small_pool[pool_off: pool_off + pk.coutp]
        pool_off += roundup(head.cout, 64)
        check(lib.w2l_pad_cast(ptr(glog), N, Th, L, pk.coutp, hh, ptr(dy_hi), ptr(dy_lo), ptr(colsum), st()),
              'w2l_pad_cast')
        last = acts[-1]
        self._wgrad(head, pk, dy_hi, dy_lo, hh, Th, last, grads)
        if head.bias is not None:
            grads[id(head.bias)] = colsum[: head.cout]
        act_grads[len(acts) - 1].append(self._dgrad(head, pk, dy_hi, dy_lo, hh, Th, last, self._producer(ctx, len(acts) - 1)))
        return pool_off

    def _producer(self, ctx, act_index: int):
        mode = FUSED_BN_REDUCE
        if mode in (False, '0') or self.precise or act_index < 1:
            return None
        uc = ctx['units'][act_index - 1]
        u = uc.unit
        if u.res is not None or not u.main.has_bn or uc.y is None or uc.y.dtype != torch.bfloat16:
            return None
        if mode == 'auto' and uc.y.shape[0] * uc.y.shape[1] >= FUSED_BN_REDUCE_MAX_ROWS:
            return None
        return (uc, ctx['training'])

    def _units_backward(self, ctx, act_grads, small_pool, pool_off, grads, batch_stats: bool):
        precise = self.precise
        acts: List[Act] = ctx['acts']
        N = ctx['out'].shape[0]
        dev = ctx['out'].device
        st = stream_ptr
        amax_pool = (zeros((len(acts) + 1, 2, AMAX_SLOTS), torch.float32, dev)
                     if self.fp8 else None)
        slot_pool = self._slot_pool
        for uc in reversed(ctx['units']):
            u = uc.unit
            oi = uc.out_index
            srcs = act_grads[oi]
            if not srcs:
                raise RuntimeError('activation without a gradient source')
            if len(srcs) > 2:
                raise NotImplementedError('more than two consumers of one activation')
            a_out = acts[oi]
            Tout, coutp = uc.Tout, a_out.CP
            p = u.drop_p if (ctx['training'] and uc.mask is not None) else 0.0
            d = self._desc(uc, N, Tout, coutp, p, uc.lens_out)
            g1 = self._gsrc(srcs[0])
            g2 = self._gsrc(srcs[1]) if len(srcs) > 1 else None
            sums = None
            fold = fast = False
            if u.main.has_bn or (u.res is not None and u.res.has_bn):
                ncomp = 4 if u.res is not None else 2
                fused = [s_.partial for s_ in srcs if s_.partial is not None]
                fast = False
                if len(fused) == len(srcs) and ncomp == 2:
                    fused = list({id(t): t for t in fused}.values())
                    partial = fused[0] if len(fused) == 1 else torch.cat(fused, 0)
                    nb = partial.shape[0]
# ... 573 lines not shown
```

wav2letter_pytorch_amd/replay.py:

```python
from __future__ import annotations

import os
import weakref
from typing import Optional

import numpy as np
import torch

from . import _lib
from ._lib import check, lib, ptr

ENABLED = os.environ.get('W2L_REPLAY', '1') != '0'
WARM_STEPS = int(os.environ.get('W2L_REPLAY_WARM', '2'))
MAX_GROUPS = int(os.environ.get('W2L_REPLAY_MAX_SHAPES', '8'))
MAX_FAILURES = 3
FP8_EAGER_EVERY = 256
FP8_EAGER_STEPS = 10
VERBOSE = os.environ.get('W2L_REPLAY_VERBOSE', '0') == '1'
LENS_RING = 4
TRANSIENT = ('fp8 weight scale', 'kernel plans were measured', 'measuring launches', 'workspace grown', 'created', 'table built',
             'momentum buffer')

_last_backward = [None]
STATS = {'recorded': 0, 'replayed_F': 0, 'replayed_B': 0, 'replayed_O': 0, 'replayed_X': 0, 'poisoned': []}


def _say(msg):
    if VERBOSE:
        print('[w2l replay] ' + msg, flush=True)


_POOLS: list = []


class _Lease:
    __slots__ = ('__weakref__',)


def new_pool(lease):
    pool = torch.cuda.MemPool()
    _POOLS.append((pool, weakref.ref(lease)))
    return pool


def purge_pools():
    if _POOLS and any(ref() is None for _, ref in _POOLS):
        dead = [e for e in _POOLS if e[1]() is None]
        _POOLS[:] = [e for e in _POOLS if e[1]() is not None]
        del dead


class RecordSet:

    def __init__(self, group, index):
        self.group = weakref.ref(group)
        self.index = index
        self.reset()

    def reset(self):
        self.lease = _Lease()
        self.lease_O = _Lease()
        self.lease_X = _Lease()
        self.pool = self.pool_O = self.pool_X = None
        self.F = self.B = self.O = self.X = None
        self.O_sig = self.X_sig = None
        self.x_static = self.x_ref = None
        self.g_static = None
        self.out = None
        self.ectx = None
        self.lens_out = None
        self.lens_static = None
        self.grads = None
        self.deferred = []
        self.O_ptrs = None
        self.O_spare = None

    def ensure_pool(self):
        if self.pool is None:
            self.pool = new_pool(self.lease)
        return self.pool


class Group:
    def __init__(self, key):
        self.key = key
        self.sets = [RecordSet(self, 0), RecordSet(self, 1)]
        self.next = 0
        self.seen = 0
        self.failures = 0
        self.disabled = None
        self.fp8_epoch = None
        self.replays = 0
        self.eager_left = 0
        self.last_use = 0


def opt_signature(opt):
    clip = opt._clip_signature() if hasattr(opt, '_clip_signature') else None
    return tuple((g['lr'], g['momentum'], g['weight_decay'], g['nesterov'], g['dampening'], g.get('maximize', False))
                 for g in opt.param_groups) + (opt.__dict__.get('_w2l_state_epoch', 0), clip)


class StepReplayer:

    def __init__(self, engine):
        self.engine = weakref.ref(engine)
        self.groups = {}
        self.pending: Optional[RecordSet] = None
        self.counter = None
        self.counter_host = 0
        self.clock = 0
        self.after_replayed_O = False
        self.opt_stream = None
        self.first_seen = {}
        self._fused_ws = None

    def _mode_flags(self):
        from . import engine as E
        return (E.DETERMINISTIC_WGRAD, E.DEALT_WGRAD, E.DEFER_SPREAD, E.WGRAD_AFTER_DGRAD, E.FUSED_BN_REDUCE, E.FOLD_BN_FINALIZE,
                E.FOLD_BN_FWD, E.FAST_BN_BWD, E.STAT_SLOTS, E.FP8_DGRAD, E.FP8_WGRAD, E.WGROUP_MAX, E.AUTOTUNE,
                os.environ.get('W2L_WGRAD_GROUPS', 'auto'))

    def plan_forward(self, x, lens, training, softmax_mode, keep_ctx):
        from . import engine as E
        eng = self.engine()
        if (not ENABLED or eng is None or not training or keep_ctx or not x.is_cuda or x.requires_grad or not torch.is_grad_enabled()
                or eng.head is None or eng.precise or eng.grad_ready is not None or eng.flat_ready is not None
                or eng.backward_done is not None or eng.grad_reduce_start is not None or eng.dropout_counter is not None
                or E.KERNEL_TIMER is not None or E.JOIN_EVENTS is not None or _lib._trace['saved'] or _lib.recording() is not None
                or x.dtype != torch.float32 or not x.is_contiguous() or (lens is not None and lens.is_cuda)
                or E.DEFER_SPREAD != 'start' or torch.cuda.is_current_stream_capturing()):
            return None
        purge_pools()
        defer = eng.defer_wgrad if eng.deferred is not None else 0
        key = (tuple(x.shape), softmax_mode, lens is None, x.device.index, _lib.raw_stream(), self._mode_flags(),
               defer if isinstance(defer, int) else tuple(sorted(defer)), id(eng.deferred), bool(eng.overlap_wgrad),
               torch.initial_seed(), E._wev_epoch[0])
        self.clock += 1
        g = self.groups.get(key)
        if g is None:
            n = self.first_seen.get(key, 0) + 1
            if len(self.first_seen) > 4096:
                self.first_seen.clear()
            self.first_seen[key] = n
            if n <= WARM_STEPS:
                return None
            if len(self.groups) >= MAX_GROUPS:
                victim = min(self.groups.values(), key=lambda v: v.last_use)
                if (self.pending is not None and self.pending.group() is victim) or self.clock - victim.last_use < 4 * MAX_GROUPS:
                    return None
                del self.groups[victim.key]
            free, total = torch.cuda.mem_get_info(x.device)
            if free < 0.2 * total:
                return None
            g = self.groups[key] = Group(key)
            g.seen = WARM_STEPS
            g.fp8_epoch = E._fp8_epoch[0]
        g.last_use = self.clock
        if g.disabled is not None:
            return None
        if g.fp8_epoch != E._fp8_epoch[0]:
            g.fp8_epoch = E._fp8_epoch[0]
            self._drop(g)
        g.seen += 1
        if g.seen <= WARM_STEPS:
            return None
        if eng.fp8:
            if g.eager_left > 0:
                g.eager_left -= 1
                return None
            if g.replays >= FP8_EAGER_EVERY:
                g.replays = 0
                g.eager_left = FP8_EAGER_STEPS - 1
                self._age_fp8_weights(FP8_EAGER_EVERY)
                return None
        if self._weights_moved(eng):
            return None
        s = g.sets[g.next]
        if self.pending is s:
            return None
        g.next ^= 1
        return ('replay' if s.F is not None and s.B is not None else 'record'), s

    def _weights_moved(self, eng) -> bool:
        moved = False
        for w in self._conv_weights(eng):
            if '_w2l_ready_ev' not in w.__dict__:
                continue
            pk = (getattr(w, '_w2l_pack', None) or {}).get(False)
            if pk is None or pk.src_ptr != w.data_ptr():
                self.groups.clear()
                self.pending = None
                return True
            if pk.version != w._version:
                moved = True
        return moved

    def _conv_weights(self, eng):
        ws = self._fused_ws
        if ws is None or ws[0] is not eng.units:
            ws = self._fused_ws = (eng.units, [c.weight for u in eng.units for c in (u.main, u.res) if c is not None] +
                                   ([eng.head.weight] if eng.head is not None else []))
        return ws[1]

    def _age_fp8_weights(self, n):
        eng = self.engine()
        for u in eng.units:
            for c in (u.main, u.res):
                st = c.weight.__dict__.get('_w2l_fp8') if c is not None else None
                if st is not None:
                    st['age'] += n

    def _drop(self, g):
        for s in g.sets:
            if self.pending is s:
                continue
            s.reset()

    def fail(self, s: RecordSet, why: str):
        g = s.group()
        s.reset()
        if g is None:
            return
        STATS['poisoned'].append(why)
        _say(f'recording dropped: {why}')
        if any(t in why for t in TRANSIENT):
            g.seen = 0
            return
        g.failures += 1
        if g.failures >= MAX_FAILURES:
            g.disabled = why
            for t in g.sets:
                if self.pending is not t:
                    t.reset()

    def before_eager(self):
        if self.after_replayed_O and self.opt_stream is not None:
            _lib.stream_wait_stream(_lib.raw_stream(), self.opt_stream)
        self.after_replayed_O = False

    def flush_pending(self):
        eng = self.engine()
        s = self.pending
        if s is None or not eng._deferred:
            self.pending = None
            return
        opt = eng.deferred
        if opt is None or not all(eng._stepped(r) for r in eng._deferred) or s.B is None:
            self.pending = None
            return
        hp = opt._deferred_state()['hp']
        sig = tuple(hp[id(r.conv.weight)][2] for r in eng._deferred) + (opt.__dict__.get('_w2l_state_epoch', 0),)
        if s.X is not None and s.X_sig != sig:
            s.X = None
        if s.X is not None:
            s.X.replay()
            from . import engine as E
            for r in eng._deferred:
                w = r.conv.weight
                for pk in (getattr(w, '_w2l_pack', None) or {}).values():
                    pk.ready, pk.version = E.weight_event(w), w._version
            eng._deferred = []
            eng._side_used = True
            STATS['replayed_X'] += 1
            self.pending = None
            return
        s.lease_X = _Lease()
        s.pool_X = new_pool(s.lease_X)
        with torch.cuda.use_mem_pool(s.pool_X), _lib.Recorder() as rec:
            eng.flush_deferred(pos=0)
        ph = rec.finish()
        self.pending = None
        if ph is None or eng._deferred:
# ... 343 lines not shown
```

Baseline: 2.556 million.

## Store per-element activation gate bits in forward to skip recomputation in BN backward

The BN+activation forward kernels now write a per-8-channel byte mask that combines dropout keep bits, activation pass and length masking. The backward reduce and apply kernels read this byte instead of recomputing z from scale and shift, so they skip the shift load and the lens and dropout checks. The inner math is also rewritten with packed float2 vectors so the compiler can emit packed FP32 ops. In exchange the forward pass writes an extra uint8 tensor per gated layer and uses more memory.

New measurement: 2.568 million, median of 6. No clear change (+0.5%).

```diff
diff --git a/include/w2l_hip.h b/include/w2l_hip.h
--- a/include/w2l_hip.h
+++ b/include/w2l_hip.h
@@ -139,6 +139,7 @@
     const int32_t* lens;
     const uint64_t* offset_dev;
     uint64_t* q_clipped;
+    uint8_t* gate;
 } w2l_bnact_t;
 
 int w2l_bn_act_fwd(const w2l_bnact_t* d, void* out_hi, void* out_lo, int out_rows, int pad_l, int pad_r,
diff --git a/wav2letter_pytorch_amd/_lib.py b/wav2letter_pytorch_amd/_lib.py
--- a/wav2letter_pytorch_amd/_lib.py
+++ b/wav2letter_pytorch_amd/_lib.py
@@ -24,7 +24,7 @@
         ('scale', c_p), ('shift', c_p), ('mean', c_p), ('invstd', c_p),
         ('y2', c_p), ('scale2', c_p), ('shift2', c_p), ('mean2', c_p), ('invstd2', c_p),
         ('act', C.c_int32), ('drop_p', c_f), ('seed', c_u64), ('offset', c_u64),
-        ('mask', c_p), ('lens', c_p), ('offset_dev', c_p), ('q_clipped', c_p),
+        ('mask', c_p), ('lens', c_p), ('offset_dev', c_p), ('q_clipped', c_p), ('gate', c_p),
     ]
 
 
diff --git a/wav2letter_pytorch_amd/csrc/bn_act.hip b/wav2letter_pytorch_amd/csrc/bn_act.hip
--- a/wav2letter_pytorch_amd/csrc/bn_act.hip
+++ b/wav2letter_pytorch_amd/csrc/bn_act.hip
@@ -125,6 +125,32 @@
     if (act == 1) return z >= 0.f && z <= 20.f;
     if (act == 2) return z > 0.f;
     return true;
+}
+
+template <int ACT>
+__device__ __forceinline__ uint32_t gate_bits(const float z[8], const float a[8], uint32_t keep) {
+    if (ACT != 1 && ACT != 2) return keep;
+    uint32_t open = 0;
+#pragma unroll
+    for (int j = 7; j >= 0; --j) open = open + open + ((ACT == 1 ? a[j] == z[j] : z[j] > 0.f) ? 1u : 0u);
+    return open & keep;
+}
+
+typedef __attribute__((ext_vector_type(2))) float f32x2;
+__device__ __forceinline__ void unpack8(const u16x8& v, f32x2 o[4]) {
+    const u32x4 w = __builtin_bit_cast(u32x4, v);
+#pragma unroll
+    for (int p = 0; p < 4; ++p) o[p] = f32x2{__uint_as_float(w[p] << 16), __uint_as_float(w[p] & 0xFFFF0000u)};
+}
+__device__ __forceinline__ void loadp8(const float* p, int c, f32x2 v[4]) {
+    const f32x4 a = *reinterpret_cast<const f32x4*>(p + c), b = *reinterpret_cast<const f32x4*>(p + c + 4);
+    v[0] = f32x2{a[0], a[1]}; v[1] = f32x2{a[2], a[3]}; v[2] = f32x2{b[0], b[1]}; v[3] = f32x2{b[2], b[3]};
+}
+__device__ __forceinline__ void store8_pairs(bf16_raw* hi, int64_t off, const f32x2 v[4]) {
+    float f[8];
+#pragma unroll
+    for (int p = 0; p < 4; ++p) { f[2 * p] = v[p][0]; f[2 * p + 1] = v[p][1]; }
+    store8_split(hi, nullptr, off, f);
 }
 
 constexpr int AMAX_SLOTS = W2L_AMAX_SLOTS;
@@ -165,16 +191,19 @@
         float a[8];
 #pragma unroll
         for (int j = 0; j < 8; ++j) a[j] = 0.f;
+        uint32_t gate = 0;
         if (t >= 0 && (!d.lens || t < d.lens[n])) {
             float z[8], y1[8], y2v[8];
             Chan c1, c2;
             load_chan(c1, d.scale, d.shift, nullptr, nullptr, cg * 8);
             if (HAS2) load_chan(c2, d.scale2, d.shift2, nullptr, nullptr, cg * 8);
-            preact8<F32, HAS2>(d, c1, c2, (int64_t)n * d.T + t, cg, G, z, y1, y2v, thresh, inv_keep, true,
-                         r - pad_l == t);
+            const uint32_t keep = preact8<F32, HAS2>(d, c1, c2, (int64_t)n * d.T + t, cg, G, z, y1, y2v, thresh, inv_keep,
+                                                     true, r - pad_l == t);
 #pragma unroll
             for (int j = 0; j < 8; ++j) a[j] = activate_t<ACT>(z[j]);
-        }
+            if (d.gate) gate = gate_bits<ACT>(z, a, keep);
+        }
+        if (d.gate && t >= 0 && r - pad_l == t) d.gate[((int64_t)n * d.T + t) * G + cg] = (uint8_t)gate;
         store8_split(out_hi, out_lo, (int64_t)orow * d.C + cg * 8, a);
         if (out_q) {
             *reinterpret_cast<uint2*>(out_q + (int64_t)orow * d.C + cg * 8) = quant8_e4m3(a, q_scale);
@@ -329,6 +358,7 @@
         float a[8];
 #pragma unroll
         for (int j = 0; j < 8; ++j) a[j] = 0.f;
+        uint32_t gate = 0;
         if (ok[u]) {
             float z[8];
 #pragma unroll
@@ -336,16 +366,19 @@
                 z[j] = bf16_bits_to_f32(ya[u][j]) * sc1[j] + sh1[j];
                 if (HAS2) z[j] += bf16_bits_to_f32(yb[u][j]) * sc2[j] + sh2[j];
             }
+            uint32_t bits = 0xFFu;
             if (drop) {
                 const int64_t gidx = ((int64_t)nn[u] * T + tt[u]) * G + cg;
-                const uint32_t bits = dropout_bits(d.seed, off, (uint64_t)gidx, thresh);
+                bits = dropout_bits(d.seed, off, (uint64_t)gidx, thresh);
                 if (rw[u] - pad_l == tt[u]) d.mask[gidx] = (uint8_t)bits;
 #pragma unroll
                 for (int j = 0; j < 8; ++j) z[j] = (bits >> j) & 1u ? z[j] * inv_keep : 0.f;
             }
 #pragma unroll
             for (int j = 0; j < 8; ++j) a[j] = activate_t<ACT>(z[j]);
-        }
+            if (d.gate) gate = gate_bits<ACT>(z, a, bits);
+        }
+        if (d.gate && tt[u] >= 0 && rw[u] - pad_l == tt[u]) d.gate[((int64_t)nn[u] * T + tt[u]) * G + cg] = (uint8_t)gate;
         store8_split(out_hi, nullptr, q * d.C + c, a);
         if (out_q) {
             *reinterpret_cast<uint2*>(out_q + q * d.C + c) = quant8_e4m3(a, q_scale);
@@ -752,6 +785,7 @@
     int n, t;
 };
 
+template <bool GATE>
 __device__ __forceinline__ void fast_row_load(const w2l_bnact_t& d, const w2l_gradsrc_t& s, int64_t row, int64_t rows, int c,
                                               int cg, int G, FastRow& o) {
     o.live = row < rows;
@@ -763,8 +797,11 @@
     const int n = (int)(row / T), t = (int)(row - (int64_t)n * T);
     o.n = n; o.t = t;
     o.y = *reinterpret_cast<const u16x8*>(reinterpret_cast<const bf16_raw*>(d.y) + row * d.C + c);
-    if (d.drop_p > 0.f) o.bits = d.mask[row * G + cg];
-    o.masked = d.lens && t >= d.lens[n];
+    if (GATE) o.bits = d.gate[row * G + cg];
+    else {
+        if (d.drop_p > 0.f) o.bits = d.mask[row * G + cg];
+        o.masked = d.lens && t >= d.lens[n];
+    }
     const bf16_raw* gp = reinterpret_cast<const bf16_raw*>(s.dxp);
     const int64_t base = (int64_t)n * s.rows;
     o.g = *reinterpret_cast<const u16x8*>(gp + (base + t + s.pad_l) * d.C + c);
@@ -776,38 +813,76 @@
     }
 }
 
-template <int ACT, bool DROP>
-__device__ __forceinline__ void fast_row_eval(const FastRow& r, const Chan& ch, float inv_keep, float g[8], float xh[8]) {
-    float gv[8];
-#pragma unroll
-    for (int j = 0; j < 8; ++j) gv[j] = bf16_bits_to_f32(r.g[j]);
+struct Chan2 {
+    f32x2 sc[4], sh[4], m[4], is[4];
+};
+template <bool GATE, bool NEED_SC>
+__device__ __forceinline__ void load_chan2(Chan2& ch, const w2l_bnact_t& d, int c) {
+#pragma unroll
+    for (int p = 0; p < 4; ++p) { ch.sc[p] = f32x2{1.f, 1.f}; ch.sh[p] = f32x2{0.f, 0.f}; ch.m[p] = f32x2{0.f, 0.f}; ch.is[p] = f32x2{0.f, 0.f}; }
+    if (!GATE || NEED_SC) loadp8(d.scale, c, ch.sc);
+    if (!GATE) loadp8(d.shift, c, ch.sh);
+    if (d.mean) { loadp8(d.mean, c, ch.m); loadp8(d.invstd, c, ch.is); }
+}
+
+template <int ACT, bool DROP, bool GATE>
+__device__ __forceinline__ void fast_row_eval(const FastRow& r, const Chan2& ch, float inv_keep, f32x2 g[4], f32x2 xh[4]) {
+    f32x2 gv[4], y[4];
+    unpack8(r.g, gv);
+    unpack8(r.y, y);
     if (r.fa) {
-#pragma unroll
-        for (int j = 0; j < 8; ++j) gv[j] += bf16_bits_to_f32(r.ga[j]);
+        f32x2 v[4];
+        unpack8(r.ga, v);
+#pragma unroll
+        for (int p = 0; p < 4; ++p) gv[p] += v[p];
     }
     if (r.fb) {
-#pragma unroll
-        for (int j = 0; j < 8; ++j) gv[j] += bf16_bits_to_f32(r.gb[j]);
-    }
-    const float gk = DROP ? inv_keep : 1.f;
-    const bool row_ok = !r.masked;
-#pragma unroll
-    for (int j = 0; j < 8; ++j) {
-        const float y = bf16_bits_to_f32(r.y[j]);
-        float z = y * ch.sc[j] + ch.sh[j];
-        bool pass = row_ok;
-        if (DROP) {
-            pass = pass && ((r.bits >> j) & 1u);
-            z *= inv_keep;
-        }
-        if (ACT == 1) pass = pass && z >= 0.f && z <= 20.f;
-        else if (ACT == 2) pass = pass && z > 0.f;
-        g[j] = pass ? gv[j] * gk : 0.f;
-        xh[j] = (y - ch.m[j]) * ch.is[j];
-    }
-}
-
-template <int U, int ACT, bool DROP>
+        f32x2 v[4];
+        unpack8(r.gb, v);
+#pragma unroll
+        for (int p = 0; p < 4; ++p) gv[p] += v[p];
+    }
+    if (DROP) {
+#pragma unroll
+        for (int p = 0; p < 4; ++p) gv[p] *= inv_keep;
+    }
+    if (GATE) {
+#pragma unroll
+        for (int p = 0; p < 4; ++p) {
+            g[p][0] = (r.bits >> (2 * p)) & 1u ? gv[p][0] : 0.f;
+            g[p][1] = (r.bits >> (2 * p + 1)) & 1u ? gv[p][1] : 0.f;
+        }
+    } else {
+        const bool row_ok = !r.masked;
+#pragma unroll
+        for (int p = 0; p < 4; ++p) {
+            f32x2 z = y[p] * ch.sc[p] + ch.sh[p];
+            if (DROP) z *= inv_keep;
+#pragma unroll
+            for (int e = 0; e < 2; ++e) {
+                bool pass = row_ok;
+                if (DROP) pass = pass && ((r.bits >> (2 * p + e)) & 1u);
+                if (ACT == 1) pass = pass && z[e] >= 0.f && z[e] <= 20.f;
+                else if (ACT == 2) pass = pass && z[e] > 0.f;
+                g[p][e] = pass ? gv[p][e] : 0.f;
+            }
+        }
+    }
+#pragma unroll
+    for (int p = 0; p < 4; ++p) xh[p] = (y[p] - ch.m[p]) * ch.is[p];
+}
+
+__device__ __forceinline__ void fast_sum_rows(f32x2 s0[4], f32x2 s1[4]) {
+#pragma unroll
+    for (int m = 8; m < 64; m <<= 1)
+#pragma unroll
+        for (int p = 0; p < 4; ++p) {
+            s0[p] += f32x2{__shfl_xor(s0[p][0], m, 64), __shfl_xor(s0[p][1], m, 64)};
+            s1[p] += f32x2{__shfl_xor(s1[p][0], m, 64), __shfl_xor(s1[p][1], m, 64)};
+        }
+}
+
+template <int U, int ACT, bool DROP, bool GATE>
 __global__ __launch_bounds__(256) void bn_bwd_reduce_fast_kernel(w2l_bnact_t d, w2l_gradsrc_t g1, float* partial, float inv_keep,
                                                                   int slots) {
     __shared__ float red[4][2][BWD_SLAB];
@@ -820,30 +895,24 @@
     const int64_t q0 = ((int64_t)chunk * 4 + wave) * (U * 8) + rr;
     FastRow r[U];
 #pragma unroll
-    for (int u = 0; u < U; ++u) fast_row_load(d, g1, q0 + 8 * u, rows, c, cg, G, r[u]);
-    Chan ch;
-    load_chan(ch, d.scale, d.shift, d.mean, d.invstd, c);
-    float s0[8], s1[8];
-#pragma unroll
-    for (int j = 0; j < 8; ++j) { s0[j] = 0.f; s1[j] = 0.f; }
+    for (int u = 0; u < U; ++u) fast_row_load<GATE>(d, g1, q0 + 8 * u, rows, c, cg, G, r[u]);
+    Chan2 ch;
+    load_chan2<GATE, false>(ch, d, c);
+    f32x2 s0[4], s1[4];
+#pragma unroll
+    for (int p = 0; p < 4; ++p) { s0[p] = f32x2{0.f, 0.f}; s1[p] = f32x2{0.f, 0.f}; }
 #pragma unroll
     for (int u = 0; u < U; ++u) {
         if (!r[u].live) continue;
-        float g[8], xh[8];
-        fast_row_eval<ACT, DROP>(r[u], ch, inv_keep, g, xh);
-#pragma unroll
-        for (int j = 0; j < 8; ++j) { s0[j] += g[j]; s1[j] += g[j] * xh[j]; }
-    }
-#pragma unroll
-    for (int m = 8; m < 64; m <<= 1)
-#pragma unroll
-        for (int j = 0; j < 8; ++j) {
-            s0[j] += __shfl_xor(s0[j], m, 64);
-            s1[j] += __shfl_xor(s1[j], m, 64);
-        }
+        f32x2 g[4], xh[4];
+        fast_row_eval<ACT, DROP, GATE>(r[u], ch, inv_keep, g, xh);
+#pragma unroll
+        for (int p = 0; p < 4; ++p) { s0[p] += g[p]; s1[p] += g[p] * xh[p]; }
+    }
+    fast_sum_rows(s0, s1);
     if (rr == 0) {
 #pragma unroll
-        for (int j = 0; j < 8; ++j) { red[wave][0][cgl * 8 + j] = s0[j]; red[wave][1][cgl * 8 + j] = s1[j]; }
+        for (int j = 0; j < 8; ++j) { red[wave][0][cgl * 8 + j] = s0[j >> 1][j & 1]; red[wave][1][cgl * 8 + j] = s1[j >> 1][j & 1]; }
     }
     __syncthreads();
     if (tid < 2 * BWD_SLAB) {
@@ -853,7 +922,7 @@
     }
 }
 
-template <int U, int ACT, bool DROP>
+template <int U, int ACT, bool DROP, bool GATE>
 __global__ __launch_bounds__(256) void bn_bwd_apply_fast_kernel(w2l_bnact_t d, w2l_gradsrc_t g1, const float* partial, int nb,
                                                                  float* sums_out, bf16_raw* dy_hi, int h1, float inv_keep,
                                                                  float* amax) {
@@ -869,7 +938,7 @@
     const int64_t q0 = ((int64_t)chunk * 4 + wave) * (U * 8) + rr;
     FastRow r[U];
 #pragma unroll
-    for (int u = 0; u < U; ++u) fast_row_load(d, g1, q0 + 8 * u, rows, c, cg, G, r[u]);
+    for (int u = 0; u < U; ++u) fast_row_load<GATE>(d, g1, q0 + 8 * u, rows, c, cg, G, r[u]);
     if (tid < 2 * BWD_SLAB) {
         const int k = tid >> 6, cc = tid & 63;
         float a = 0.f;
@@ -886,29 +955,32 @@
         if (chunk == 0) sums_out[(int64_t)k * d.C + slab * BWD_SLAB + cc] = a;
     }
     __syncthreads();
-    Chan ch;
-    load_chan(ch, d.scale, d.shift, d.mean, d.invstd, c);
-    float sg[8], sgx[8];
-#pragma unroll
-    for (int j = 0; j < 8; ++j) { sg[j] = ssum[0][cgl * 8 + j]; sgx[j] = ssum[1][cgl * 8 + j]; }
+    Chan2 ch;
+    load_chan2<GATE, true>(ch, d, c);
+    f32x2 sg[4], sgx[4];
+#pragma unroll
+    for (int p = 0; p < 4; ++p) {
+        sg[p] = f32x2{ssum[0][cgl * 8 + 2 * p], ssum[0][cgl * 8 + 2 * p + 1]};
+        sgx[p] = f32x2{ssum[1][cgl * 8 + 2 * p], ssum[1][cgl * 8 + 2 * p + 1]};
+    }
     const float invM = 1.f / ((float)N * (float)T);
     float mx = 0.f;
 #pragma unroll
     for (int u = 0; u < U; ++u) {
         if (!r[u].live) continue;
-        float g[8], xh[8], o[8];
-        fast_row_eval<ACT, DROP>(r[u], ch, inv_keep, g, xh);
+        f32x2 g[4], xh[4], o[4];
+        fast_row_eval<ACT, DROP, GATE>(r[u], ch, inv_keep, g, xh);
         if (d.mean) {
 #pragma unroll
-            for (int j = 0; j < 8; ++j) o[j] = ch.sc[j] * (g[j] - sg[j] * invM - xh[j] * sgx[j] * invM);
+            for (int p = 0; p < 4; ++p) o[p] = ch.sc[p] * (g[p] - sg[p] * invM - xh[p] * sgx[p] * invM);
         } else {
 #pragma unroll
-            for (int j = 0; j < 8; ++j) o[j] = g[j] * ch.sc[j];
-        }
-        store8_split(dy_hi, nullptr, ((int64_t)h1 + (int64_t)r[u].n * (T + h1) + r[u].t) * d.C + c, o);
+            for (int p = 0; p < 4; ++p) o[p] = g[p] * ch.sc[p];
+        }
+        store8_pairs(dy_hi, ((int64_t)h1 + (int64_t)r[u].n * (T + h1) + r[u].t) * d.C + c, o);
         if (amax) {
 #pragma unroll
-            for (int j = 0; j < 8; ++j) mx = fmaxf(mx, fabsf(o[j]));
+            for (int p = 0; p < 4; ++p) mx = fmaxf(mx, fmaxf(fabsf(o[p][0]), fabsf(o[p][1])));
         }
     }
     if (h1 > 0) {
@@ -941,13 +1013,15 @@
     const bf16_raw* pg;
     const uint8_t* pm;
 };
+template <bool GATE>
 __device__ __forceinline__ void rowcur_init(RowCur& q, const w2l_bnact_t& d, const w2l_gradsrc_t& s, int64_t row, int c, int cg, int G) {
     q.row = row;
     q.n = (int)(row / d.T);
     q.t = (int)(row - (int64_t)q.n * d.T);
     q.py = reinterpret_cast<const bf16_raw*>(d.y) + row * d.C + c;
     q.pg = reinterpret_cast<const bf16_raw*>(s.dxp) + ((int64_t)q.n * s.rows + q.t + s.pad_l) * d.C + c;
-    q.pm = d.mask ? d.mask + row * G + cg : nullptr;
+    const uint8_t* bits = GATE ? d.gate : d.mask;
+    q.pm = bits ? bits + row * G + cg : nullptr;
 }
 __device__ __forceinline__ void rowcur_step(RowCur& q, const w2l_bnact_t& d, const w2l_gradsrc_t& s, int G) {
     q.row += 8;
@@ -961,6 +1035,7 @@
         q.pg += (int64_t)(s.rows - d.T) * d.C;
     }
 }
+template <bool GATE>
 __device__ __forceinline__ void fast_row_load_cur(const w2l_bnact_t& d, const w2l_gradsrc_t& s, const RowCur& q, bool live, FastRow& o) {
     o.live = live;
     o.fa = o.fb = o.masked = false;
@@ -969,8 +1044,11 @@
     if (!live) return;
     const int T = d.T, t = q.t;
     o.y = *reinterpret_cast<const u16x8*>(q.py);
-    if (d.drop_p > 0.f) o.bits = *q.pm;
-    o.masked = d.lens && t >= d.lens[q.n];
+    if (GATE) o.bits = *q.pm;
+    else {
+        if (d.drop_p > 0.f) o.bits = *q.pm;
+        o.masked = d.lens && t >= d.lens[q.n];
+    }
     o.g = *reinterpret_cast<const u16x8*>(q.pg);
     if (s.pad_mode == 1) {
         o.fa = t >= 1 && t <= s.pad_l;
@@ -980,7 +1058,7 @@
     }
 }
 
-template <int ACT, bool DROP>
+template <int ACT, bool DROP, bool GATE>
 __global__ __launch_bounds__(256) void bn_bwd_reduce_loop_kernel(w2l_bnact_t d, w2l_gradsrc_t g1, float* partial, float inv_keep,
                                                                   int slots, int iters) {
     __shared__ float red[4][2][BWD_SLAB];
@@ -991,35 +1069,29 @@
     const int cg = slab * (BWD_SLAB / 8) + cgl, c = cg * 8;
     const int64_t rows = (int64_t)d.N * d.T;
     RowCur q;
-    rowcur_init(q, d, g1, ((int64_t)chunk * 4 + wave) * ((int64_t)iters * 8) + rr, c, cg, G);
+    rowcur_init<GATE>(q, d, g1, ((int64_t)chunk * 4 + wave) * ((int64_t)iters * 8) + rr, c, cg, G);
     FastRow cur, nxt;
-    fast_row_load_cur(d, g1, q, q.row < rows, cur);
-    Chan ch;
-    load_chan(ch, d.scale, d.shift, d.mean, d.invstd, c);
-    float s0[8], s1[8];
-#pragma unroll
-    for (int j = 0; j < 8; ++j) { s0[j] = 0.f; s1[j] = 0.f; }
+    fast_row_load_cur<GATE>(d, g1, q, q.row < rows, cur);
+    Chan2 ch;
+    load_chan2<GATE, false>(ch, d, c);
+    f32x2 s0[4], s1[4];
+#pragma unroll
+    for (int p = 0; p < 4; ++p) { s0[p] = f32x2{0.f, 0.f}; s1[p] = f32x2{0.f, 0.f}; }
     for (int it = 0; it < iters; ++it) {
         rowcur_step(q, d, g1, G);
-        fast_row_load_cur(d, g1, q, it + 1 < iters && q.row < rows, nxt);
+        fast_row_load_cur<GATE>(d, g1, q, it + 1 < iters && q.row < rows, nxt);
         if (cur.live) {
-            float g[8], xh[8];
-            fast_row_eval<ACT, DROP>(cur, ch, inv_keep, g, xh);
-#pragma unroll
-            for (int j = 0; j < 8; ++j) { s0[j] += g[j]; s1[j] += g[j] * xh[j]; }
+            f32x2 g[4], xh[4];
+            fast_row_eval<ACT, DROP, GATE>(cur, ch, inv_keep, g, xh);
+#pragma unroll
+            for (int p = 0; p < 4; ++p) { s0[p] += g[p]; s1[p] += g[p] * xh[p]; }
         }
         cur = nxt;
     }
-#pragma unroll
-    for (int m = 8; m < 64; m <<= 1)
-#pragma unroll
-        for (int j = 0; j < 8; ++j) {
-            s0[j] += __shfl_xor(s0[j], m, 64);
-            s1[j] += __shfl_xor(s1[j], m, 64);
-        }
+    fast_sum_rows(s0, s1);
     if (rr == 0) {
 #pragma unroll
-        for (int j = 0; j < 8; ++j) { red[wave][0][cgl * 8 + j] = s0[j]; red[wave][1][cgl * 8 + j] = s1[j]; }
+        for (int j = 0; j < 8; ++j) { red[wave][0][cgl * 8 + j] = s0[j >> 1][j & 1]; red[wave][1][cgl * 8 + j] = s1[j >> 1][j & 1]; }
     }
     __syncthreads();
     if (tid < 2 * BWD_SLAB) {
@@ -1029,7 +1101,7 @@
     }
 }
 
-template <int ACT, bool DROP>
+template <int ACT, bool DROP, bool GATE>
 __global__ __launch_bounds__(256) void bn_bwd_apply_loop_kernel(w2l_bnact_t d, w2l_gradsrc_t g1, const float* partial, int nb,
                                                                  float* sums_out, bf16_raw* dy_hi, int h1, float inv_keep,
                                                                  float* amax, int iters) {
@@ -1043,10 +1115,10 @@
     const int T = d.T, N = d.N;
     const int64_t rows = (int64_t)N * T;
     RowCur q;
-    rowcur_init(q, d, g1, ((int64_t)chunk * 4 + wave) * ((int64_t)iters * 8) + rr, c, cg, G);
+    rowcur_init<GATE>(q, d, g1, ((int64_t)chunk * 4 + wave) * ((int64_t)iters * 8) + rr, c, cg, G);
     bf16_raw* pdy = dy_hi + ((int64_t)h1 + (int64_t)q.n * (T + h1) + q.t) * d.C + c;
     FastRow cur, nxt;
-    fast_row_load_cur(d, g1, q, q.row < rows, cur);
+    fast_row_load_cur<GATE>(d, g1, q, q.row < rows, cur);
     if (tid < 2 * BWD_SLAB) {
         const int k = tid >> 6, cc = tid & 63;
         float a = 0.f;
@@ -1063,32 +1135,35 @@
         if (chunk == 0) sums_out[(int64_t)k * d.C + slab * BWD_SLAB + cc] = a;
     }
     __syncthreads();
-    Chan ch;
-    load_chan(ch, d.scale, d.shift, d.mean, d.invstd, c);
+    Chan2 ch;
+    load_chan2<GATE, true>(ch, d, c);
     const float invM = 1.f / ((float)N * (float)T);
-    float sg[8], sgx[8];
-#pragma unroll
-    for (int j = 0; j < 8; ++j) { sg[j] = ssum[0][cgl * 8 + j] * invM; sgx[j] = ssum[1][cgl * 8 + j] * invM; }
+    f32x2 sg[4], sgx[4];
+#pragma unroll
+    for (int p = 0; p < 4; ++p) {
+        sg[p] = f32x2{ssum[0][cgl * 8 + 2 * p], ssum[0][cgl * 8 + 2 * p + 1]} * invM;
+        sgx[p] = f32x2{ssum[1][cgl * 8 + 2 * p], ssum[1][cgl * 8 + 2 * p + 1]} * invM;
+    }
     float mx = 0.f;
     for (int it = 0; it < iters; ++it) {
         bf16_raw* const pdy_cur = pdy;
         pdy += (int64_t)(q.t + 8 >= T ? 8 + h1 : 8) * d.C;
         rowcur_step(q, d, g1, G);
-        fast_row_load_cur(d, g1, q, it + 1 < iters && q.row < rows, nxt);
+        fast_row_load_cur<GATE>(d, g1, q, it + 1 < iters && q.row < rows, nxt);
         if (cur.live) {
-            float g[8], xh[8], o[8];
-            fast_row_eval<ACT, DROP>(cur, ch, inv_keep, g, xh);
+            f32x2 g[4], xh[4], o[4];
+            fast_row_eval<ACT, DROP, GATE>(cur, ch, inv_keep, g, xh);
             if (d.mean) {
 #pragma unroll
-                for (int j = 0; j < 8; ++j) o[j] = ch.sc[j] * (g[j] - sg[j] - xh[j] * sgx[j]);
+                for (int p = 0; p < 4; ++p) o[p] = ch.sc[p] * (g[p] - sg[p] - xh[p] * sgx[p]);
             } else {
 #pragma unroll
-                for (int j = 0; j < 8; ++j) o[j] = g[j] * ch.sc[j];
-            }
-            store8_split(pdy_cur, nullptr, 0, o);
+                for (int p = 0; p < 4; ++p) o[p] = g[p] * ch.sc[p];
+            }
+            store8_pairs(pdy_cur, 0, o);
             if (amax) {
 #pragma unroll
-                for (int j = 0; j < 8; ++j) mx = fmaxf(mx, fabsf(o[j]));
+                for (int p = 0; p < 4; ++p) mx = fmaxf(mx, fmaxf(fabsf(o[p][0]), fabsf(o[p][1])));
             }
         }
         cur = nxt;
@@ -1360,26 +1435,30 @@
     if (iters > 0) {
         const int nch = (int)((rows + 4LL * iters * 8 - 1) / (4LL * iters * 8));
         const dim3 lgrid((unsigned)(nch * (d->C / BWD_SLAB)));
-#define W2L_REDL(A, D) hipLaunchKernelGGL((bn_bwd_reduce_loop_kernel<A, D>), lgrid, dim3(256), 0, (hipStream_t)stream, *d, *g1, partial, inv_keep, slots, iters)
+#define W2L_REDL_G(A, D, GT) hipLaunchKernelGGL((bn_bwd_reduce_loop_kernel<A, D, GT>), lgrid, dim3(256), 0, (hipStream_t)stream, *d, *g1, partial, inv_keep, slots, iters)
+#define W2L_REDL(A, D) do { if (d->gate) W2L_REDL_G(A, D, true); else W2L_REDL_G(A, D, false); } while (0)
         switch (d->act) {
             case 1: if (drop) W2L_REDL(1, true); else W2L_REDL(1, false); break;
             case 2: if (drop) W2L_REDL(2, true); else W2L_REDL(2, false); break;
             default: if (drop) W2L_REDL(0, true); else W2L_REDL(0, false); break;
         }
 #undef W2L_REDL
+#undef W2L_REDL_G
         W2L_CHECK_LAUNCH();
         return 0;
     }
     constexpr int U = 2;
     const int nchunks = (int)((rows + 4 * U * 8 - 1) / (4 * U * 8));
     const dim3 grid((unsigned)(nchunks * (d->C / BWD_SLAB)));
-#define W2L_RED(A, D) hipLaunchKernelGGL((bn_bwd_reduce_fast_kernel<U, A, D>), grid, dim3(256), 0, (hipStream_t)stream, *d, *g1, partial, inv_keep, slots)
+#define W2L_RED_G(A, D, GT) hipLaunchKernelGGL((bn_bwd_reduce_fast_kernel<U, A, D, GT>), grid, dim3(256), 0, (hipStream_t)stream, *d, *g1, partial, inv_keep, slots)
+#define W2L_RED(A, D) do { if (d->gate) W2L_RED_G(A, D, true); else W2L_RED_G(A, D, false); } while (0)
     switch (d->act) {
         case 1: if (drop) W2L_RED(1, true); else W2L_RED(1, false); break;
         case 2: if (drop) W2L_RED(2, true); else W2L_RED(2, false); break;
         default: if (drop) W2L_RED(0, true); else W2L_RED(0, false); break;
     }
 #undef W2L_RED
+#undef W2L_RED_G
     W2L_CHECK_LAUNCH();
     return 0;
 }
@@ -1398,20 +1477,23 @@
         const int nch = (int)((rows + 4LL * iters * 8 - 1) / (4LL * iters * 8));
         const dim3 lgrid((unsigned)(nch * (d->C / BWD_SLAB)));
         const bool dropl = d->drop_p > 0.f;
-#define W2L_APPL(A, D) hipLaunchKernelGGL((bn_bwd_apply_loop_kernel<A, D>), lgrid, dim3(256), 0, (hipStream_t)stream, *d, *g1, partial, nrows, sums, (bf16_raw*)dy_hi, halo, inv_keep, amax, iters)
+#define W2L_APPL_G(A, D, GT) hipLaunchKernelGGL((bn_bwd_apply_loop_kernel<A, D, GT>), lgrid, dim3(256), 0, (hipStream_t)stream, *d, *g1, partial, nrows, sums, (bf16_raw*)dy_hi, halo, inv_keep, amax, iters)
+#define W2L_APPL(A, D) do { if (d->gate) W2L_APPL_G(A, D, true); else W2L_APPL_G(A, D, false); } while (0)
         switch (d->act) {
             case 1: if (dropl) W2L_APPL(1, true); else W2L_APPL(1, false); break;
             case 2: if (dropl) W2L_APPL(2, true); else W2L_APPL(2, false); break;
             default: if (dropl) W2L_APPL(0, true); else W2L_APPL(0, false); break;
         }
 #undef W2L_APPL
+#undef W2L_APPL_G
         W2L_CHECK_LAUNCH();
         return 0;
     }
     const int U = amax ? 4 : (d->C <= 384 ? 2 : 1);
     const int nchunks = (int)((rows + 4 * U * 8 - 1) / (4 * U * 8));
     const dim3 grid((unsigned)(nchunks * (d->C / BWD_SLAB)));
-#define W2L_APP(UU, A, D) hipLaunchKernelGGL((bn_bwd_apply_fast_kernel<UU, A, D>), grid, dim3(256), 0, (hipStream_t)stream, *d, *g1, partial, nrows, sums, (bf16_raw*)dy_hi, halo, inv_keep, amax)
+#define W2L_APP_G(UU, A, D, GT) hipLaunchKernelGGL((bn_bwd_apply_fast_kernel<UU, A, D, GT>), grid, dim3(256), 0, (hipStream_t)stream, *d, *g1, partial, nrows, sums, (bf16_raw*)dy_hi, halo, inv_keep, amax)
+#define W2L_APP(UU, A, D) do { if (d->gate) W2L_APP_G(UU, A, D, true); else W2L_APP_G(UU, A, D, false); } while (0)
 #define W2L_APP_U(A, D) do { if (U == 4) W2L_APP(4, A, D); else if (U == 2) W2L_APP(2, A, D); else W2L_APP(1, A, D); } while (0)
     const bool drop = d->drop_p > 0.f;
     switch (d->act) {
@@ -1421,6 +1503,7 @@
     }
 #undef W2L_APP_U
 #undef W2L_APP
+#undef W2L_APP_G
     W2L_CHECK_LAUNCH();
     return 0;
 }
diff --git a/wav2letter_pytorch_amd/engine.py b/wav2letter_pytorch_amd/engine.py
--- a/wav2letter_pytorch_amd/engine.py
+++ b/wav2letter_pytorch_amd/engine.py
@@ -174,6 +174,7 @@
     mean2: Optional[torch.Tensor] = None
     invstd2: Optional[torch.Tensor] = None
     mask: Optional[torch.Tensor] = None
+    gate: Optional[torch.Tensor] = None
     seed: int = 0
     offset: int = 0
     out_index: int = 0
@@ -499,6 +500,7 @@
 FOLD_BN_FWD_MAX_ROWS = 12288
 FAST_BN_BWD = os.environ.get('W2L_FAST_BN_BWD', '1') == '1'
 STAT_SLOTS = int(os.environ.get('W2L_STAT_SLOTS', '8'))
+BN_GATE = os.environ.get('W2L_BN_GATE', '1') == '1'
 
 
 def _wgrad_workspace(dev, cin, cout, kw):
@@ -772,6 +774,9 @@
                 else:
                     _dropout_calls += 1
                     uc.offset = _dropout_calls
+            if (BN_GATE and FAST_BN_BWD and not DETERMINISTIC_WGRAD and training and not precise and u.res is None
+                    and conv.has_bn and coutp % 64 == 0):
+                uc.gate = torch.empty(N * Tout * (coutp // 8), dtype=torch.uint8, device=dev)
             d = self._desc(uc, N, Tout, coutp, p, uc.lens_out)
             out_q, q_scale = None, 1.0
             if self.fp8 and coutp % 128 == 0 and self._fp8_consumers(ui + 1):
@@ -1287,6 +1292,7 @@
         d.drop_p = float(p)
         d.seed, d.offset = uc.seed, uc.offset
         d.mask = uc.mask.data_ptr() if uc.mask is not None else None
+        d.gate = uc.gate.data_ptr() if (uc.gate is not None and BN_GATE) else None
         d.lens = lens.data_ptr() if lens is not None else None
         d.offset_dev = self.dropout_counter.data_ptr() if (self.dropout_counter is not None and p > 0.0) else None
         uc.keep.append(lens)
diff --git a/wav2letter_pytorch_amd/replay.py b/wav2letter_pytorch_amd/replay.py
--- a/wav2letter_pytorch_amd/replay.py
+++ b/wav2letter_pytorch_amd/replay.py
@@ -118,7 +118,7 @@
     def _mode_flags(self):
         from . import engine as E
         return (E.DETERMINISTIC_WGRAD, E.DEALT_WGRAD, E.DEFER_SPREAD, E.WGRAD_AFTER_DGRAD, E.FUSED_BN_REDUCE, E.FOLD_BN_FINALIZE,
-                E.FOLD_BN_FWD, E.FAST_BN_BWD, E.STAT_SLOTS, E.FP8_DGRAD, E.FP8_WGRAD, E.WGROUP_MAX, E.AUTOTUNE,
+                E.FOLD_BN_FWD, E.FAST_BN_BWD, E.BN_GATE, E.STAT_SLOTS, E.FP8_DGRAD, E.FP8_WGRAD, E.WGROUP_MAX, E.AUTOTUNE,
                 os.environ.get('W2L_WGRAD_GROUPS', 'auto'))
 
     def plan_forward(self, x, lens, training, softmax_mode, keep_ctx):
```
